# MarioPasc/MU-Diff

Hardware: AMD Instinct MI355X
Metric: 256x256 slices/sec (4-step dual-gen reverse) (higher is better)
Workload: dtype f32 (convs/attention: fp16 hi+lo split MFMA x3; 3x3 convs that fill the chip: fp16 hi.hi + e4m3 cross terms; fp32 accumulate); 1 GPU; BASELINE config 3 (BraTS-shaped test-split batches of 32; model and slice shapes of config 2): 4-step dual-generator sampling, 256x256, nf=64, ch_mult 1-2-4, 32 slices per GPU per step, batch-sharded over 1 GPU(s), weights replicated; batch=32, hipgraph=True

## Files before the change

include/mudiff_hip.h:

```cpp
#ifndef MUDIFF_HIP_H
#define MUDIFF_HIP_H

#include <stdint.h>

#ifdef __cplusplus
extern "C" {
#endif

#define MUD_OK 0
#define MUD_ERR_ARG 1
#define MUD_ERR_LAUNCH 2
#define MUD_ERR_UNSUPPORTED 3

#define MUD_ACT_NONE 0
#define MUD_ACT_SIGMOID 1
#define MUD_ACT_TANH 2
#define MUD_ACT_SILU 3
#define MUD_ACT_LRELU 4

#define MUD_PRO_NONE 0
#define MUD_PRO_AFFINE 1
#define MUD_PRO_AFFINE_SILU 2
#define MUD_PRO_LRELU 3
#define MUD_PRO_UP2_AFFINE_SILU 4

#define MUD_PREC_16X3 0
#define MUD_PREC_FP8X 1
#define MUD_PREC_16X1 2

int mud_version(void);
const char* mud_last_error(void);
const char* mud_build_flags(void);

int mud_posterior_sample(const float* x01, const float* x02, const float* xt, const float* noise,
                         const int64_t* t, const float* coef1, const float* coef2, const float* std_tab,
                         int ntab, float* out, int B, int64_t per_sample, void* stream);
int mud_q_sample(const float* x, const float* noise, const int64_t* t, int toff, const float* a_tab,
                 const float* s_tab, int ntab, float* out, int B, int64_t per_sample, void* stream);

int mud_timestep_embedding(const int64_t* t, float* out, int B, int dim, float max_positions, void* stream);
int mud_pixel_norm(const float* z, float* out, int B, int K, void* stream);
int mud_dense(const float* in, int ldi, const float* W, const float* bias, float* out, int ldo,
              int B, int K, int N, int act_in, int act_out, void* stream);

#define MUD_MLP_MAX_LAYERS 6
typedef struct mud_mlp_args {
  const float* x; int ldx; int B;
  int nlayers; int dims[MUD_MLP_MAX_LAYERS + 1];
  const float* W[MUD_MLP_MAX_LAYERS]; const float* b[MUD_MLP_MAX_LAYERS];
  int pixel_norm; int act; int act_last;
  float* out; int ldo;
  int maxdim;
} mud_mlp_args;
int mud_mlp_chain(const mud_mlp_args* a, void* stream);
int mud_mlp_chains(const mud_mlp_args* a, int n, void* stream);

int64_t mud_gn_ws_bytes(int B, int64_t HW, int C, int G);
int mud_gn_scale_shift(const float* x, int B, int64_t HW, int C, int ld, int G, float eps,
                       const float* gamma, const float* beta, int64_t g_bstride,
                       float* scale, float* shift, int ld_ss, float* mean_rstd ,
                       void* ws, void* stream);
int mud_gn_scale_shift_from_sums(const double* sums, int sums_ld, int B, int C, int G, double count, float eps,
                                 const float* gamma, const float* beta, int64_t g_bstride,
                                 float* scale, float* shift, int ld_ss, void* stream);
int mud_channel_mean(const float* x, int B, int64_t HW, int C, int ld, float* out, int ldo, void* ws, void* stream);

typedef struct mud_conv_args {
  const float* x;  int B, H, W, Cin, ldx;
  const void* w;   int64_t w_bstride;
  int ks, stride, pad;
  const float* pro_scale; const float* pro_shift; int pro_ld; int pro_mode;
  const float* bias;
  const float* bias2; int bias2_ld;
  const float* res; int ldr;
  float out_scale; int act;
  const float* emul; int ld_emul;
  const float* egate; int ld_egate;
  const float* eother; int ld_eother;
  float* out; int Cout, ldo;
  int sub2;
  double* stats; int stats_ld;
  int emul_cout;
  const double* gn_sums; int gn_sums_ld;
  int gn_G; float gn_eps; double gn_count;
  const float* gn_gamma; const float* gn_beta;
  int64_t gn_bstride;
  void* splitk_ws; int64_t splitk_ws_bytes;
  unsigned* splitk_counters; int splitk_ncounters;
  const void* skip_w; const float* skip_bias; float* skip_out; int skip_ldo;
  int prec; int w_exp;
  int res_up2; float res_k[4];
  int in_up2; float in_k[4];
} mud_conv_args;

int mud_conv2d_direct(const mud_conv_args* a, void* stream);

int64_t mud_packed_weight_bytes(int ks, int Cin, int Cout);
int mud_pack_weights(const float* src, int64_t s_tap, int64_t s_ci, int64_t s_co, int64_t src_bstride,
                     int ks, int Cin, int Cout, int nbatch, void* dst, void* stream);
int mud_pack_weights_prec(const float* src, int64_t s_tap, int64_t s_ci, int64_t s_co, int64_t src_bstride,
                          int ks, int Cin, int Cout, int nbatch, int prec, int w_exp, void* dst, void* stream);
int64_t mud_packed_weight_bytes_prec(int ks, int Cin, int Cout, int prec);
int mud_conv2d_mfma(const mud_conv_args* a, void* stream);
int mud_conv2d_mfma_prec_supported(const mud_conv_args* a, int prec);
int64_t mud_conv2d_mfma_splitk_bytes(const mud_conv_args* a);
int mud_conv2d_mfma_res_up2_supported(const mud_conv_args* a);
int mud_conv2d_mfma_in_up2_supported(const mud_conv_args* a);

typedef struct mud_census_args {
  const float* x; int B, H, W, C, ldx;
  const float* pro_scale; const float* pro_shift; int pro_ld; int pro_mode;
} mud_census_args;
typedef struct mud_census_out {
  uint64_t n, n_over, n_under, n_fp16_over, amax_bits;
} mud_census_out;
int mud_e4m3_census(const mud_census_args* a, mud_census_out* out, void* stream);

int mud_upfirdn2d(const float* in, int64_t planes, int H, int W, const float* kernel, int kh, int kw,
                  int up_x, int up_y, int down_x, int down_y, int pad_x0, int pad_x1, int pad_y0, int pad_y1,
                  float* out, void* stream);
int mud_fir_nhwc(const float* x, int B, int H, int W, int C, int ldx, const float* kernel_host, int kh, int kw,
                 int up, int down, int pad0, int pad1,
                 const float* pro_scale, const float* pro_shift, int pro_ld, int pro_mode,
                 float* out_h, int ldh, float* out_x, int ldxo, void* stream);

int mud_minibatch_stddev(const float* x, int B, int64_t hw, int C, int ld, int group, float* out, void* stream);

int mud_attention_supported(int C);
int64_t mud_attention_ws_bytes(int B, int N, int C);
int mud_attention(const float* qkv, int B, int N, int C, int ld, float scale, float* out, int ldo, void* ws, void* stream);

int mud_softmax_rows(float* s, int64_t rows, int n, int ld, void* stream);
int mud_mul(const float* a, int lda, const float* b, int ldb, float* out, int ldo, int64_t npix, int C, void* stream);
int mud_gate_mix(const float* g, int ldg, const float* att, int lda, const float* other, int ldb,
                 float* out, int ldo, int B, int64_t hw, int C, double* stats, int stats_ld, void* stream);

int mud_fourier_embedding(const float* t, const float* W, float* out, int B, int n, void* stream);
int mud_resize_bilinear(const float* in, int64_t planes, int H, int W, int Ho, int Wo, float* out, void* stream);
int mud_affine_clamp(const float* x, int64_t n, float scale, float shift, float lo, float hi, float* out, void* stream);

int64_t mud_value_range_ws_bytes(void);
int mud_value_range(const float* a, int64_t na, const float* b, int64_t nb, float* out, void* ws, void* stream);
int mud_quantize_u8(const float* x, int64_t n, float lo, float range, uint8_t* out, void* stream);
int64_t mud_slice_metrics_ws_bytes(int n, int H, int W);
int mud_slice_metrics_u8(const uint8_t* pred, const uint8_t* gt, int n, int H, int W, int64_t* sse, int64_t* sae, double* ssim_sum,
                         void* ws, int64_t ws_bytes, void* stream);

#define MUD_VM_MAX_REGIONS 8
#define MUD_VM_NQ 8
#define MUD_VM_N 0
#define MUD_VM_SSE 1
#define MUD_VM_SAE 2
#define MUD_VM_N_INT 3
#define MUD_VM_SSIM 4
#define MUD_VM_SS 5
#define MUD_VM_SS2 6
#define MUD_VM_SSE_STD 7
int64_t mud_volume_metrics_ws_bytes(int Z, int X, int Y, int nreg);
int mud_volume_metrics(const float* pred, const float* gt, const uint8_t* region, const float* std, int Z, int X, int Y, int nreg,
                       double* sums, void* ws, int64_t ws_bytes, void* stream);

int64_t mud_lpips_packed_bytes(void);
int mud_lpips_pack(const float* table, void* const* conv_w, void* const* conv_b, void* const* lin_w, void* packed, void* stream);
int64_t mud_lpips_ws_bytes(int n, int H, int W);
int mud_lpips_u8(const uint8_t* pred, const uint8_t* gt, int n, int H, int W, const void* packed, double* out, void* ws,
                 int64_t ws_bytes, void* stream);

int mud_randn_keyed(float* out, int rows, int64_t row_len, const int64_t* keys, uint64_t seed, int step, int kind, void* stream);
int mud_ensemble_stats(const float* samples, int n, int N, int64_t hw, float scale, float shift, float lo, float hi, float* mean,
                       float* std, void* stream);

#define MUD_ENSEMBLE_MAX_QUANTILES 8
#define MUD_ENSEMBLE_QUANTILES_MAX_N 64
int mud_ensemble_quantiles(const float* samples, int n, int N, int64_t hw, float scale, float shift, float lo, float hi, const double* q,
                           int K, float* out, void* stream);

#define MUD_VC_NC 5
#define MUD_VC_NS 2
#define MUD_VC_PARTS 16
#define MUD_VC_N 0
#define MUD_VC_BELOW 1
#define MUD_VC_ABOVE 2
#define MUD_VC_INSIDE 3
#define MUD_VC_NONFINITE 4
#define MUD_VC_WIDTH 0
#define MUD_VC_WIDTH_INSIDE 1
int mud_volume_interval_coverage(const float* lo, const float* hi, const float* gt, const uint8_t* region, int Z, int X, int Y, int nreg,
                                 int z0, int z1, int64_t* counts, double* sums, void* ws, int64_t ws_bytes, void* stream);

#define MUD_COUPLING_MAX_RADIUS 32
int mud_randn_keyed_coupled(float* out, int rows, int64_t row_len, const int64_t* keys, uint64_t seed, int step, int kind,
                            const double* half_taps, int radius, void* stream);

int mud_known_constrain(const float* x_new, const float* known, const uint8_t* mask, const float* noise, const int64_t* keys, uint64_t seed,
                        int step, int kind, const int64_t* t, int toff, const float* a_tab, const float* s_tab, int ntab, int clean,
                        float* out, int rows, int64_t row_len, void* stream);
int mud_known_coverage(const double* m, int SX, int SY, int SZ, int X, int Y, int Z, uint8_t* out, void* stream);

int mud_fft2_c2c(const float* in, float* out, int rows, int S, int inverse, void* stream);
int mud_fft2_r2c(const float* in, float* out, int rows, int S, int inverse, void* stream);
int mud_kspace_constrain(const float* x_new, const float* y, const uint8_t* mask, int mask_rows, const float* noise, const int64_t* keys,
                         uint64_t seed, int step, int kind, const int64_t* t, int toff, const float* a_tab, const float* s_tab, int ntab,
                         int clean, float* out, float* work, int rows, int S, void* stream);

#define MUD_SLAB_MAX_MEMBERS 16
int mud_slab_constrain(const float* x_new, const float* y, const int32_t* members, const float* weights, const float* gains, int groups, int L,
                       const float* noise, const int64_t* keys, uint64_t seed, int step, int kind, const int64_t* t, int toff,
                       const float* a_tab, const float* s_tab, int ntab, int clean, float* out, int rows, int64_t row_len, void* stream);
int mud_slab_average(const float* x, const int32_t* members, const float* weights, int groups, int L, float* avg, int rows, int64_t row_len,
                     void* stream);

int mud_slab_kspace_constrain(const float* x_new, const float* y, const uint8_t* mask, int mask_rows, const int32_t* members,
                              const float* weights, const float* gains, int groups, int L, const float* noise, const int64_t* keys,
                              uint64_t seed, int step, int kind, const int64_t* t, int toff, const float* a_tab, const float* s_tab,
                              int ntab, int clean, float* out, float* work, int rows, int S, void* stream);

#define MUD_BAND_MAX_MEMBERS 32
#define MUD_BAND_MAX_BW 8
#define MUD_BAND_MAX_M 256
#define MUD_BAND_MAX_N 512
typedef struct mud_band_tables {
  int m, n, bw, nnz;
  const int32_t* start;
  const int32_t* member;
  const float* w;
  const int32_t* tstart;
  const int32_t* tmember;
  const float* tw;
  const float* lc;
} mud_band_tables;
int mud_band_constrain(const float* x, const float* y, const mud_band_tables* tab, const float* noise, const int64_t* keys, uint64_t seed, int step,
                       int kind, const int64_t* t, int toff, const float* a_tab, const float* s_tab, int ntab, int clean, float* out, float* work,
                       int sets, int64_t row_len, void* stream);
int mud_band_measure(const float* x, const mud_band_tables* tab, float* ax, int sets, int64_t row_len, void* stream);

#define MUD_TP_NQ 8
#define MUD_TP_PARTS 16
#define MUD_TP_N_DZ 0
#define MUD_TP_S_DZ 1
#define MUD_TP_N_DZZ 2
#define MUD_TP_S_DZZ 3
#define MUD_TP_N_DX 4
#define MUD_TP_S_DX 5
#define MUD_TP_N_DY 6
#define MUD_TP_S_DY 7
int mud_volume_through_plane(const float* vol, const uint8_t* mask, int Z, int X, int Y, int z0, int z1, double* sums, void* ws,
                             int64_t ws_bytes, void* stream);

#define MUD_NIFTI_U1 2
#define MUD_NIFTI_I2 4
#define MUD_NIFTI_I4 8
#define MUD_NIFTI_F4 16
#define MUD_NIFTI_U2 512
#define MUD_VI_MAX_RANKS 4
#define MUD_VI_WINDOW 16
typedef struct mud_volume_census_record {
  uint64_t n, n_nonfinite;
  float min, max;
  int32_t count[MUD_VI_MAX_RANKS];
  int64_t first_rank[MUD_VI_MAX_RANKS];
  float window[MUD_VI_MAX_RANKS][MUD_VI_WINDOW];
} mud_volume_census_record;
int64_t mud_volume_census_ws_bytes(void);
int mud_volume_census(const void* vol, int datatype, int X, int Y, int Z, float slope, float inter, const double* q, int nq,
                      mud_volume_census_record* record, void* ws, int64_t ws_bytes, void* stream);
int mud_volume_slab_normalise(const void* vol, int datatype, int X, int Y, int Z, float slope, float inter, float lo, float den,
                              int degenerate, int s0, int s1, float* out, void* stream);
int mud_volume_slab_zscore(const void* vol, int datatype, int X, int Y, int Z, float slope, float inter, float mean, float std, int s0,
                           int s1, float* out, void* stream);
int mud_volume_assemble(const float* planes, const float* planes2, int X, int Y, int Z, int s0, int s1, float* vol, float* vol2,
                        void* stream);
int mud_volume_regrid(const void* src, int datatype, int SX, int SY, int SZ, float slope, float inter, const double* m, int mode, int X,
                      int Y, int Z, float* out, void* stream);
int mud_volume_bspline_coeffs(const void* vol, int datatype, int SX, int SY, int SZ, float slope, float inter, double* coeffs,
                              uint32_t* nonfinite, void* stream);
int mud_volume_regrid_cubic(const double* coeffs, int SX, int SY, int SZ, const void* src, int datatype, float slope, float inter,
                            const double* m, double lo, double hi, int X, int Y, int Z, float* out, void* stream);
int mud_volume_joint_hist(const void* fix, int fix_dt, int X, int Y, int Z, float fix_slope, float fix_inter, const void* mov, int mov_dt,
                          int SX, int SY, int SZ, float mov_slope, float mov_inter, const double* m, int stride, double fix_lo,
                          double fix_scale, double mov_lo, double mov_scale, int bins, uint32_t* hist, void* stream);
int mud_volume_mirror_moments(const void* vol, int datatype, int X, int Y, int Z, float slope, float inter, const double* mats, int K,
                              int stride, double lo, double scale, int bins, uint64_t* sums, void* stream);
int mud_volume_bias_log(const void* vol, int datatype, int X, int Y, int Z, float slope, float inter, int shrink, float* u, void* stream);
int mud_volume_bias_corrected(const float* u, const float* c_old, float* c_new, const double* lattices, int levels, int X, int Y, int Z,
                              int shrink, uint64_t* stats, void* stream);
int mud_volume_bias_hist(const float* c, int64_t n, double lo, double scale, int bins, uint32_t* hist, void* stream);
int mud_volume_bias_fit(const float* c, const double* table, int bins, double lo, double scale, int level, int X, int Y, int Z, int shrink,
                        int k, int64_t* sums, void* stream);
int mud_volume_bias_apply(const void* vol, int datatype, int X, int Y, int Z, float slope, float inter, const double* lattices, int levels,
                          int field, float* out, void* stream);
int mud_volume_denoise_residual(const void* vol, int datatype, int X, int Y, int Z, float slope, float inter, uint32_t* keys, void* stream);
int mud_volume_denoise_select_hist(const uint32_t* keys, int64_t n, uint32_t prefix, int pass, uint32_t* hist, void* stream);
int mud_volume_denoise_nlm(const void* vol, int datatype, int X, int Y, int Z, float slope, float inter, int search, int patch, double sigma,
                           double beta, int rician, float* out, uint32_t* zeroed, void* stream);
int mud_volume_fg_range(const void* vol, int datatype, int X, int Y, int Z, float slope, float inter, uint32_t* range, void* stream);
int mud_volume_fg_hist(const void* vol, int datatype, int X, int Y, int Z, float slope, float inter, double lo, double scale, int bins,
                       uint32_t* hist, void* stream);
int mud_volume_fg_mask(const void* vol, int datatype, int X, int Y, int Z, float slope, float inter, double lo, double scale, int bins, int k,
                       uint8_t* mask, void* stream);
int mud_volume_fg_morph(const uint8_t* in, int X, int Y, int Z, int dilate, uint8_t* out, void* stream);
int mud_volume_fg_label(const uint8_t* mask, int X, int Y, int Z, int value, int32_t* labels, void* stream);
int mud_volume_fg_census(const int32_t* labels, int X, int Y, int Z, uint32_t* census, uint64_t* summary, void* stream);
int mud_volume_fg_select(const int32_t* labels, const uint32_t* census, int64_t n, int root, int holes, uint8_t* mask, uint32_t* count,
                         void* stream);
int mud_volume_fg_apply(const void* vol, int datatype, int X, int Y, int Z, float slope, float inter, const uint8_t* mask, float* out,
                        uint32_t* removed, void* stream);
int mud_volume_edt(const uint8_t* mask, int X, int Y, int Z, int value, double sx, double sy, double sz, double* d2, void* stream);
int mud_volume_edt_select(const double* d2, int64_t n, double r2, int above, const uint8_t* within, uint8_t* out, uint32_t* count,
                          void* stream);
int mud_volume_reorient(const void* src, int elem_bytes, int SX, int SY, int SZ, int p0, int p1, int p2, int flip_mask, void* dst,
                        void* stream);
int mud_volume_lowpass(const void* vol, int datatype, int X, int Y, int Z, float slope, float inter, const double* wx, int rx,
                       const double* wy, int ry, const double* wz, int rz, float* out, float* scratch, uint32_t* nonfinite, void* stream);

#ifdef __cplusplus
}
#endif
#endif
```

mu-diff_amd/backbones/up_or_down_sampling.py:

```python
import numpy as np
import torch
import torch.nn as nn

from mudiff_hip import ops
from mudiff_hip.ops import View
from utils.op import upfirdn2d


def _setup_kernel(k):
    k = np.asarray(k, dtype=np.float32)
    if k.ndim == 1:
        k = np.outer(k, k)
    k /= np.sum(k)
    assert k.ndim == 2 and k.shape[0] == k.shape[1]
    return k


def fir_params(mode, k=None, factor=2, gain=1, conv_k=3):
    if k is None:
        k = [1] * factor
    if mode == 'up':
        kk = _setup_kernel(k) * (gain * (factor ** 2))
        p = kk.shape[0] - factor
        return kk, factor, 1, ((p + 1) // 2 + factor - 1, p // 2)
    if mode == 'naive_up':
        return np.ones((factor, factor), np.float32), factor, 1, (factor - 1, 0)
    if mode == 'naive_down':
        return np.full((factor, factor), 1.0 / (factor * factor), np.float32), 1, factor, (0, 0)
    kk = _setup_kernel(k) * gain
    if mode == 'down':
        p = kk.shape[0] - factor
        return kk, 1, factor, ((p + 1) // 2, p // 2)
    if mode == 'conv_down':
        p = (kk.shape[0] - factor) + (conv_k - 1)
        return kk, 1, 1, ((p + 1) // 2, p // 2)
    raise ValueError(mode)


_DEV_KERNELS = {}


def _device_kernel(kk, device):
    key = (kk.tobytes(), kk.shape, str(device))
    t = _DEV_KERNELS.get(key)
    if t is None:
        t = torch.tensor(kk, device=device, dtype=torch.float32)
        _DEV_KERNELS[key] = t
    return t


def upsample_2d(x, k=None, factor=2, gain=1):
    kk, up, down, pad = fir_params('up', k, factor, gain)
    return upfirdn2d(x, torch.tensor(kk, device=x.device, dtype=x.dtype), up=up, pad=pad)


def downsample_2d(x, k=None, factor=2, gain=1):
    kk, up, down, pad = fir_params('down', k, factor, gain)
    return upfirdn2d(x, torch.tensor(kk, device=x.device, dtype=x.dtype), down=down, pad=pad)


def conv_downsample_2d(x, w, k=None, factor=2, gain=1):
    kk, _, _, pad = fir_params('conv_down', k, factor, gain, conv_k=w.shape[-1])
    xf = upfirdn2d(x, torch.tensor(kk, device=x.device, dtype=x.dtype), pad=pad)
    out = ops.conv(View.from_nchw(xf), ops.direct_weight(w), w.shape[-1], w.shape[0], mfma=False, stride=factor, pad=0)
    return out.to_nchw()


def naive_upsample_2d(x, factor=2):
    kk, up, down, pad = fir_params('naive_up', factor=factor)
    return upfirdn2d(x, _device_kernel(kk, x.device), up=up, pad=pad)


def naive_downsample_2d(x, factor=2):
    kk, up, down, pad = fir_params('naive_down', factor=factor)
    return upfirdn2d(x, _device_kernel(kk, x.device), down=down, pad=pad)


def resample_view(x: View, direction, fir, fir_kernel):
    kk, up, down, pad = fir_params(direction if fir else 'naive_' + direction, fir_kernel)
    if x.C % 4 == 0:
        return ops.fir_nhwc(x, kk, up, down, pad)[0]
    assert x.ld == x.C, 'planes path needs a dense view'
    t = x.base.reshape(x.B, x.H, x.W, x.C)
    planes = t.reshape(x.B, 1, x.H, x.W) if x.C == 1 else t.permute(0, 3, 1, 2).contiguous()
    r = upfirdn2d(planes, _device_kernel(kk, x.device), up=up, down=down, pad=pad)
    return View.from_nchw(r)


def padded_strided_conv(x: View, kk, pad, weights, ks, cout, bias, res, out_scale, out, layer=None):
    if x.C % 4 == 0 and x.C >= 8 and ks == 3 and x.H % 2 == 0 and x.W % 2 == 0:
        xf, _ = ops.fir_nhwc(x, kk, 1, 1, pad)
        prec = ops.choose_prec(xf, cout, ops.PRO_NONE, sub2=True)
        return ops.conv(xf, weights(True, prec), 3, cout, mfma=True, bias=bias, res=res, out_scale=out_scale, out=out, sub2=True, prec=prec,
                        layer=layer)
    if x.C % 4 == 0:
        xf, _ = ops.fir_nhwc(x, kk, 1, 1, pad)
    else:
        assert x.ld == x.C
        t = x.base.reshape(x.B, x.H, x.W, x.C)
        planes = t.reshape(x.B, 1, x.H, x.W) if x.C == 1 else t.permute(0, 3, 1, 2).contiguous()
        xf = View.from_nchw(upfirdn2d(planes, _device_kernel(np.ascontiguousarray(kk, np.float32), x.device), pad=pad))
    return ops.conv(xf, weights(False), ks, cout, mfma=False, stride=2, pad=0, bias=bias, res=res, out_scale=out_scale, out=out)


class Conv2d(nn.Module):

    def __init__(self, in_ch, out_ch, kernel, up=False, down=False, resample_kernel=(1, 3, 3, 1), use_bias=True, kernel_init=None):
        super().__init__()
        assert not (up and down)
        assert kernel >= 1 and kernel % 2 == 1
        self.weight = nn.Parameter(torch.zeros(out_ch, in_ch, kernel, kernel))
        if kernel_init is not None:
            self.weight.data = kernel_init(self.weight.data.shape)
        if use_bias:
            self.bias = nn.Parameter(torch.zeros(out_ch))
        self.up, self.down, self.resample_kernel, self.kernel, self.use_bias = up, down, resample_kernel, kernel, use_bias
        self._prep = None

    def _weights(self, mfma=False, prec=ops.PREC_16X3):
        key = (self.weight._version, self.weight.data_ptr(), mfma, prec)
        if self._prep is None or self._prep[0] != key:
            with torch.no_grad():
                self._prep = (key, ops.pack_conv_weight(self.weight, prec=prec) if mfma else ops.direct_weight(self.weight))
        return self._prep[1]

    def run(self, x: View, res: View = None, out_scale=1.0, out: View = None):
        if self.up:
            raise NotImplementedError('Conv2d(up=True) is unreachable in the reference (upsample_conv_2d raises)')
        bias = self.bias.detach() if self.use_bias else None
        if not self.down:
            return ops.conv(x, self._weights(), self.kernel, self.weight.shape[0], mfma=False, bias=bias, res=res, out_scale=out_scale, out=out)
        kk, up, down, pad = fir_params('conv_down', self.resample_kernel, conv_k=self.kernel)
        return padded_strided_conv(x, kk, pad, self._weights, self.kernel, self.weight.shape[0], bias, res, out_scale, out,
                                   layer=self.__dict__.get('_layer_name', 'Conv2d_0'))

    def forward(self, x):
        return self.run(View.from_nchw(x)).to_nchw()
```

mu-diff_amd/csrc/conv_direct.hip:

```cpp
#include "mud_common.h"
#include <stdlib.h>

template <int VO, int VI>
__global__ __launch_bounds__(256) void k_conv_direct(mud_conv_args a, int Ho, int Wo, int co_groups) {
  extern __shared__ __attribute__((aligned(16))) char smem_raw[];
  float* st_lds = (float*)smem_raw;
  const int b = blockIdx.y;
  if (a.stats) {
    for (int i = threadIdx.x; i < 2 * a.Cout; i += 256) st_lds[i] = 0.f;
    __syncthreads();
  }
  const unsigned total = (unsigned)Ho * (unsigned)Wo * (unsigned)co_groups;
  const unsigned nthreads = gridDim.x * blockDim.x;
  const unsigned stride = (nthreads / (unsigned)co_groups) * (unsigned)co_groups;
  const unsigned first = blockIdx.x * blockDim.x + threadIdx.x;
  const int cg = (int)(first % (unsigned)co_groups);
  float ssum[VO], ssq[VO];
#pragma unroll
  for (int j = 0; j < VO; ++j) ssum[j] = ssq[j] = 0.f;
  for (uint64_t idx64 = first; first < stride && idx64 < total; idx64 += stride) {
    const unsigned p = (unsigned)idx64 / (unsigned)co_groups;
    const int oy = (int)(p / (unsigned)Wo);
    const int ox = (int)(p - (unsigned)oy * (unsigned)Wo);
    const int co = cg * VO;
    float acc[VO];
#pragma unroll
    for (int j = 0; j < VO; ++j) acc[j] = 0.f;
    const float* wb = (const float*)((const char*)a.w + (int64_t)b * a.w_bstride);
    for (int ky = 0; ky < a.ks; ++ky) {
      const int iy = oy * a.stride - a.pad + ky;
      if (iy < 0 || iy >= a.H) continue;
      for (int kx = 0; kx < a.ks; ++kx) {
        const int ix = ox * a.stride - a.pad + kx;
        if (ix < 0 || ix >= a.W) continue;
        const float* xp = a.x + (((int64_t)b * a.H + iy) * a.W + ix) * a.ldx;
        const float* wp = wb + ((int64_t)(ky * a.ks + kx) * a.Cin) * a.Cout + co;
        for (int ci = 0; ci < a.Cin; ci += VI) {
          float xv[VI];
          if (VI == 4) *(f32x4*)xv = *(const f32x4*)(xp + ci);
          else xv[0] = xp[ci];
#pragma unroll
          for (int u = 0; u < VI; ++u) {
            float v = xv[u];
            if (a.pro_mode == MUD_PRO_LRELU)
              v = v > 0.f ? v : 0.2f * v;
            else if (a.pro_mode != MUD_PRO_NONE)
              v = mud_prologue(v, a.pro_scale[(int64_t)b * a.pro_ld + ci + u], a.pro_shift[(int64_t)b * a.pro_ld + ci + u], a.pro_mode);
            const float* w = wp + (int64_t)(ci + u) * a.Cout;
            if (VO == 4) {
              const f32x4 wv = *(const f32x4*)w;
#pragma unroll
              for (int j = 0; j < 4; ++j) acc[j] = fmaf(v, wv[j], acc[j]);
            } else {
              acc[0] = fmaf(v, w[0], acc[0]);
            }
          }
        }
      }
    }
    const int64_t opix = ((int64_t)b * Ho + oy) * Wo + ox;
#pragma unroll
    for (int j = 0; j < VO; ++j) {
      float v = acc[j];
      if (a.bias) v += a.bias[co + j];
      if (a.bias2) v += a.bias2[(int64_t)b * a.bias2_ld + co + j];
      if (a.res) v += a.res[opix * a.ldr + co + j];
      v = mud_act(v * a.out_scale, a.act);
      if (a.emul && (a.emul_cout <= 0 || co + j < a.emul_cout)) v *= a.emul[opix * a.ld_emul + co + j];
      if (a.egate) {
        const float gt = a.egate[opix * a.ld_egate + co + j];
        v = gt * v + (1.0f - gt) * a.eother[opix * a.ld_eother + co + j];
      }
      acc[j] = v;
    }
    float* op = a.out + opix * a.ldo + co;
    if (VO == 4) *(f32x4*)op = *(f32x4*)acc;
    else op[0] = acc[0];
#pragma unroll
    for (int j = 0; j < VO; ++j) {
      ssum[j] += acc[j];
      ssq[j] += acc[j] * acc[j];
    }
  }
  if (a.stats) {
    if (first < stride && first < total) {
      const int co = (int)(first % co_groups) * VO;
#pragma unroll
      for (int j = 0; j < VO; ++j) {
        atomicAdd(&st_lds[(co + j) * 2], ssum[j]);
        atomicAdd(&st_lds[(co + j) * 2 + 1], ssq[j]);
      }
    }
    __syncthreads();
    for (int i = threadIdx.x; i < 2 * a.Cout; i += 256)
      atomicAdd(a.stats + ((int64_t)b * a.stats_ld + (i >> 1)) * 2 + (i & 1), (double)st_lds[i]);
  }
}

#define HEAD_PIX 8
template <int S>
__global__ __launch_bounds__(256) void k_conv_head3x3(mud_conv_args a, int co_groups, int strips_per_row, int Ho, int Wo) {
  extern __shared__ __attribute__((aligned(16))) char smem_raw[];
  float* st_lds = (float*)smem_raw;
  const int b = blockIdx.y;
  if (a.stats) {
    for (int i = threadIdx.x; i < 2 * a.Cout; i += 256) st_lds[i] = 0.f;
    __syncthreads();
  }
  const int cg = threadIdx.x % co_groups, co = cg * 4;
  const int spb = 256 / co_groups;
  const int ls = threadIdx.x / co_groups;
  f32x4 w[9];
#pragma unroll
  for (int t = 0; t < 9; ++t) w[t] = *(const f32x4*)((const float*)a.w + (int64_t)t * a.Cout + co);
  f32x4 bias = {0.f, 0.f, 0.f, 0.f};
  if (a.bias) bias = *(const f32x4*)(a.bias + co);
  if (a.bias2) bias += *(const f32x4*)(a.bias2 + (int64_t)b * a.bias2_ld + co);
  const int64_t HW = (int64_t)a.H * a.W;
  const float* xb = a.x + (int64_t)b * HW * a.ldx;
  f32x4 s4 = {0.f, 0.f, 0.f, 0.f}, q4 = {0.f, 0.f, 0.f, 0.f};
  const int64_t nstrips = (int64_t)Ho * strips_per_row;
  constexpr int WIN = S * (HEAD_PIX - 1) + 3;
  const bool active = ls < spb;
  for (int64_t st = (int64_t)blockIdx.x * spb + ls; active && st < nstrips; st += (int64_t)gridDim.x * spb) {
    const int y = (int)(st / strips_per_row), x0 = (int)(st - (int64_t)y * strips_per_row) * HEAD_PIX;
    float win[3][WIN];
#pragma unroll
    for (int dy = 0; dy < 3; ++dy) {
      const int iy = y * S + dy - a.pad;
      const bool yok = iy >= 0 && iy < a.H;
      const int64_t rowoff = (int64_t)(yok ? iy : 0) * a.W;
#pragma unroll
      for (int j = 0; j < WIN; ++j) {
        const int ix = x0 * S + j - a.pad;
        const bool ok = yok && ix >= 0 && ix < a.W;
        const float v = xb[(rowoff + (ok ? ix : 0)) * a.ldx];
        win[dy][j] = ok ? v : 0.f;
      }
    }
#pragma unroll
    for (int k = 0; k < HEAD_PIX; ++k) {
      if (x0 + k >= Wo) break;
      f32x4 acc = bias;
#pragma unroll
      for (int dy = 0; dy < 3; ++dy)
#pragma unroll
        for (int dx = 0; dx < 3; ++dx) acc += win[dy][k * S + dx] * w[dy * 3 + dx];
      const int64_t opix = ((int64_t)b * Ho + y) * Wo + x0 + k;
      if (a.res) acc += *(const f32x4*)(a.res + opix * a.ldr + co);
      acc *= a.out_scale;
      if (a.act != MUD_ACT_NONE) {
#pragma unroll
        for (int e = 0; e < 4; ++e) acc[e] = mud_act(acc[e], a.act);
      }
      *(f32x4*)(a.out + opix * a.ldo + co) = acc;
      s4 += acc;
      q4 += acc * acc;
    }
  }
  if (a.stats) {
    if (active) {
#pragma unroll
      for (int e = 0; e < 4; ++e) {
        atomicAdd(&st_lds[(co + e) * 2], s4[e]);
        atomicAdd(&st_lds[(co + e) * 2 + 1], q4[e]);
      }
    }
    __syncthreads();
    for (int i = threadIdx.x; i < 2 * a.Cout; i += 256)
      atomicAdd(a.stats + ((int64_t)b * a.stats_ld + (i >> 1)) * 2 + (i & 1), (double)st_lds[i]);
  }
}

#define TAIL_ROWS 8
#define TAIL_REC 20
template <int COUT>
__global__ __launch_bounds__(256) void k_conv_tail3x3(mud_conv_args a, int tiles_x, int tiles_y) {
  __shared__ __attribute__((aligned(16))) float tile[(TAIL_ROWS + 2) * 34 * TAIL_REC];
  const int b = blockIdx.y;
  const int ty0 = (blockIdx.x / tiles_x) * TAIL_ROWS, tx0 = (blockIdx.x % tiles_x) * 32;
  const int tid = threadIdx.x, py = tid >> 5, px = tid & 31;
  const float* xb = a.x + (int64_t)b * a.H * a.W * a.ldx;
  const float* wb = (const float*)((const char*)a.w + (int64_t)b * a.w_bstride);
  float acc[COUT];
#pragma unroll
  for (int j = 0; j < COUT; ++j) acc[j] = 0.f;
  constexpr int NPIX = (TAIL_ROWS + 2) * 34, ITEMS = NPIX * 4;
  for (int c0 = 0; c0 < a.Cin; c0 += 16) {
    for (int it = tid; it < ITEMS; it += 256) {
      const int p = it >> 2, q = it & 3;
      const int gy = ty0 + p / 34 - 1, gx = tx0 + p % 34 - 1;
      const bool ok = gy >= 0 && gy < a.H && gx >= 0 && gx < a.W;
      f32x4 v = {0.f, 0.f, 0.f, 0.f};
      if (ok) {
        v = *(const f32x4*)(xb + ((int64_t)gy * a.W + gx) * a.ldx + c0 + q * 4);
        if (a.pro_mode == MUD_PRO_LRELU) {
#pragma unroll
          for (int e = 0; e < 4; ++e) v[e] = v[e] > 0.f ? v[e] : 0.2f * v[e];
        } else if (a.pro_mode != MUD_PRO_NONE) {
          const f32x4 sc = *(const f32x4*)(a.pro_scale + (int64_t)b * a.pro_ld + c0 + q * 4);
          const f32x4 sh = *(const f32x4*)(a.pro_shift + (int64_t)b * a.pro_ld + c0 + q * 4);
#pragma unroll
          for (int e = 0; e < 4; ++e) v[e] = mud_prologue(v[e], sc[e], sh[e], a.pro_mode);
        }
      }
      *(f32x4*)(tile + p * TAIL_REC + q * 4) = v;
    }
    __syncthreads();
#pragma unroll
    for (int t = 0; t < 9; ++t) {
      const float* rec = tile + ((py + t / 3) * 34 + px + t % 3) * TAIL_REC;
      const float* wt = wb + ((int64_t)t * a.Cin + c0) * a.Cout;
#pragma unroll
      for (int q = 0; q < 4; ++q) {
        const f32x4 v = *(const f32x4*)(rec + q * 4);
#pragma unroll
        for (int e = 0; e < 4; ++e)
#pragma unroll
          for (int j = 0; j < COUT; ++j) acc[j] = fmaf(v[e], wt[(q * 4 + e) * COUT + j], acc[j]);
      }
    }
    __syncthreads();
  }
  const int gy = ty0 + py, gx = tx0 + px;
  if (gy < a.H && gx < a.W) {
    const int64_t opix = ((int64_t)b * a.H + gy) * a.W + gx;
#pragma unroll
    for (int j = 0; j < COUT; ++j) {
      float v = acc[j];
      if (a.bias) v += a.bias[j];
      if (a.res) v += a.res[opix * a.ldr + j];
      a.out[opix * a.ldo + j] = mud_act(v * a.out_scale, a.act);
    }
  }
}

extern "C" int mud_conv2d_direct(const mud_conv_args* ap, void* stream) {
  MUD_REQUIRE(ap, "mud_conv2d_direct: null args");
  const mud_conv_args a = *ap;
  MUD_REQUIRE(a.x && a.w && a.out, "mud_conv2d_direct: null pointer");
  MUD_REQUIRE(a.B >= 0 && a.H > 0 && a.W > 0 && a.Cin > 0 && a.Cout > 0 && a.ks >= 1 && a.stride >= 1 && a.pad >= 0,
              "mud_conv2d_direct: bad sizes");
  MUD_REQUIRE(a.ldx >= a.Cin && a.ldo >= a.Cout, "mud_conv2d_direct: ld smaller than C");
  MUD_REQUIRE(a.pro_mode == MUD_PRO_NONE || a.pro_mode == MUD_PRO_LRELU || (a.pro_scale && a.pro_shift && a.pro_ld >= a.Cin), "mud_conv2d_direct: prologue arrays missing");
  MUD_REQUIRE(!a.res || a.ldr >= a.Cout, "mud_conv2d_direct: bad residual view");
  MUD_REQUIRE(!a.res_up2, "mud_conv2d_direct: res_up2 (a residual up-sampled on load) is built for mud_conv2d_mfma's 3x3 kernel only");
  MUD_REQUIRE(!a.in_up2, "mud_conv2d_direct: in_up2 (an input up-sampled while it is staged) is built for mud_conv2d_mfma's 3x3 kernel only");
  const int Ho = (a.H + 2 * a.pad - a.ks) / a.stride + 1, Wo = (a.W + 2 * a.pad - a.ks) / a.stride + 1;
  MUD_REQUIRE(Ho > 0 && Wo > 0, "mud_conv2d_direct: empty output");
  if (a.B == 0) return MUD_OK;
  const bool vo4 = a.Cout % 4 == 0 && a.ldo % 4 == 0 && mud_aligned16(a.out) && mud_aligned16(a.w) && (a.w_bstride % 16 == 0);
  const bool vi4 = a.Cin % 4 == 0 && a.ldx % 4 == 0 && mud_aligned16(a.x);
  const int co_groups = vo4 ? a.Cout / 4 : a.Cout;
  if (a.Cin == 1 && a.ks == 3 && ((a.stride == 1 && a.pad == 1) || (a.stride == 2 && a.pad == 0)) && vo4 && !a.emul && !a.egate && co_groups <= 256 && a.pro_mode == MUD_PRO_NONE && a.w_bstride == 0 &&
      (!a.res || (a.ldr % 4 == 0 && mud_aligned16(a.res))) && (!a.bias || mud_aligned16(a.bias)) &&
      (!a.bias2 || (a.bias2_ld % 4 == 0 && mud_aligned16(a.bias2)))) {
    MUD_REQUIRE(a.B <= 65535 && (!a.stats || a.stats_ld >= a.Cout), "mud_conv2d_direct: bad batch / stats view");
    const int spb = 256 / co_groups, strips_per_row = (int)mud_cdiv(Wo, HEAD_PIX);
    int64_t blocks = mud_cdiv((int64_t)Ho * strips_per_row, spb);
    if (blocks > 256 * 16) blocks = 256 * 16;
    if (a.stats) {
      static const int cap = getenv("MUD_HEAD_CAP") ? atoi(getenv("MUD_HEAD_CAP")) : 0;
      int64_t per_image = 2048 / a.B > 16 ? 2048 / a.B : 16;
      const int64_t lim = cap > 0 ? cap : (a.B == 1 ? 256 : 128);
      if (per_image > lim) per_image = lim;
      if (blocks > per_image) blocks = per_image;
    }
    if (a.stride == 1)
      hipLaunchKernelGGL(k_conv_head3x3<1>, dim3((int)blocks, a.B), dim3(256), a.stats ? 2 * a.Cout * sizeof(float) : 0, (hipStream_t)stream, a, co_groups,
                         strips_per_row, Ho, Wo);
    else
      hipLaunchKernelGGL(k_conv_head3x3<2>, dim3((int)blocks, a.B), dim3(256), a.stats ? 2 * a.Cout * sizeof(float) : 0, (hipStream_t)stream, a, co_groups,
                         strips_per_row, Ho, Wo);
    MUD_CHECK_LAUNCH("mud_conv2d_direct(head)");
    return MUD_OK;
  }
  if (a.ks == 3 && a.stride == 1 && a.pad == 1 && a.Cout <= 4 && a.Cin % 16 == 0 && vi4 && !a.emul && !a.egate && !a.stats && !a.bias2 && !a.sub2 &&
      (a.pro_mode == MUD_PRO_NONE || a.pro_mode == MUD_PRO_LRELU || (a.pro_ld % 4 == 0 && mud_aligned16(a.pro_scale) && mud_aligned16(a.pro_shift)))) {
    MUD_REQUIRE(a.B <= 65535, "mud_conv2d_direct: B too large");
    const int tiles_x = (int)mud_cdiv(a.W, 32), tiles_y = (int)mud_cdiv(a.H, TAIL_ROWS);
    dim3 grid(tiles_x * tiles_y, a.B), block(256);
    hipStream_t s = (hipStream_t)stream;
    switch (a.Cout) {
      case 1: hipLaunchKernelGGL((k_conv_tail3x3<1>), grid, block, 0, s, a, tiles_x, tiles_y); break;
      case 2: hipLaunchKernelGGL((k_conv_tail3x3<2>), grid, block, 0, s, a, tiles_x, tiles_y); break;
      case 3: hipLaunchKernelGGL((k_conv_tail3x3<3>), grid, block, 0, s, a, tiles_x, tiles_y); break;
      default: hipLaunchKernelGGL((k_conv_tail3x3<4>), grid, block, 0, s, a, tiles_x, tiles_y); break;
    }
    MUD_CHECK_LAUNCH("mud_conv2d_direct(tail)");
    return MUD_OK;
  }
  const int64_t total = (int64_t)Ho * Wo * co_groups;
  int64_t blocks = mud_cdiv(total, 256 * (a.stats ? 8 : 1));
  if (blocks > 256 * 32) blocks = 256 * 32;
  while (blocks * 256 < co_groups) ++blocks;
  MUD_REQUIRE(a.B <= 65535 && total < (1ll << 31) - (1ll << 24), "mud_conv2d_direct: B or image too large");
  MUD_REQUIRE(!a.stats || (a.stats_ld >= a.Cout && a.Cout <= 8192), "mud_conv2d_direct: bad stats view");
  hipStream_t s = (hipStream_t)stream;
  dim3 grid((int)blocks, a.B), block(256);
  const size_t lds = a.stats ? 2 * a.Cout * sizeof(float) : 0;
  if (vo4 && vi4) hipLaunchKernelGGL((k_conv_direct<4, 4>), grid, block, lds, s, a, Ho, Wo, co_groups);
  else if (vo4) hipLaunchKernelGGL((k_conv_direct<4, 1>), grid, block, lds, s, a, Ho, Wo, co_groups);
  else if (vi4) hipLaunchKernelGGL((k_conv_direct<1, 4>), grid, block, lds, s, a, Ho, Wo, co_groups);
  else hipLaunchKernelGGL((k_conv_direct<1, 1>), grid, block, lds, s, a, Ho, Wo, co_groups);
  MUD_CHECK_LAUNCH("mud_conv2d_direct");
  return MUD_OK;
}
```

mu-diff_amd/csrc/conv_mfma.hip:

```cpp
#include "mud_common.h"
#include <stdlib.h>
#include <type_traits>
#include <utility>

typedef int i32x4 __attribute__((ext_vector_type(4)));
typedef int i32x8 __attribute__((ext_vector_type(8)));
typedef _Float16 f16x4 __attribute__((ext_vector_type(4)));
typedef _Float16 f16x8 __attribute__((ext_vector_type(8)));

typedef mud_h16x4 h16x4;
typedef mud_h16x8 h16x8;
__device__ __forceinline__ int cm_e4m3x4(f32x4 v, float scale) {
  v = v * scale;
#pragma unroll
  for (int e = 0; e < 4; ++e) v[e] = __builtin_amdgcn_fmed3f(v[e], -448.0f, 448.0f);
  int p = __builtin_amdgcn_cvt_pk_fp8_f32(v[0], v[1], 0, false);
  return __builtin_amdgcn_cvt_pk_fp8_f32(v[2], v[3], p, true);
}
#define CM_BN 64
#define CM_BPLANE (CM_BN * 32)
#define CM_BSTEP (2 * CM_BPLANE)
#define CM_PIX 80
#define CM_GN_MAXC 1024
#define CM_GN_BYTES (2 * CM_GN_MAXC * 4)

template <int KS, int MT, int WM, int WN, bool DUAL = false, int PREC = MUD_PREC_16X3>
struct CmGeo {
  static constexpr int NT = 64 * WM * WN;
  static constexpr int TAPS = KS * KS;
  static constexpr int CH = (KS == 3) ? 1 : 2;
  static constexpr int KCH = 16 * CH;
  static constexpr int ROWS = WM * MT;
  static constexpr int PW = 32 + KS - 1;
  static constexpr int P = (KS == 3) ? (ROWS + 2) * PW : 32 * WM * MT;
  static constexpr bool H1 = PREC == MUD_PREC_16X1;
  static constexpr int PIX = H1 ? 48 : CM_PIX;
  static constexpr int BSTEP = H1 ? CM_BPLANE : CM_BSTEP;
  static constexpr int PLANE = P * PIX;
  static constexpr int BUF = CH * PLANE;
  static constexpr int Q = 4 * CH;
  static constexpr int ITEMS = P * Q;
  static constexpr int NLOAD = (ITEMS + NT - 1) / NT;
  static constexpr int STEPS = TAPS * CH;
  static constexpr int GS = (KS == 3) ? 3 : 2;
  static constexpr int NG = STEPS / GS;
  static constexpr int GB1 = GS * BSTEP;
  static constexpr int GB = WN * GB1;
  static constexpr int N4 = GB / (1024 * WM * WN), REM = GB / 1024 - N4 * WM * WN;
  static_assert(GB % 1024 == 0 && GB1 % 1024 == 0, "whole 1 KiB pieces, none straddling two tiles");
  static constexpr int A_BYTES = 2 * BUF;
  static constexpr int B_OFF = A_BYTES;
  static constexpr int EP_BYTES = WM * WN * (32 * 36 * 4 + 64 * 2 * 4);
  static constexpr int GN_MAXC = DUAL ? 512 : CM_GN_MAXC;
  static constexpr int A2_OFF = A_BYTES + 2 * GB;
  static_assert(!DUAL || A2_OFF % 64 == 0, "the raw image's hi / lo halves are addressed by flipping bit 5 of the offset");
  static constexpr int A2_BYTES = DUAL ? ROWS * 32 * 64 : 0;
  static constexpr int B2_OFF = A2_OFF + A2_BYTES;
  static constexpr int B2_BYTES = DUAL ? WN * CM_BSTEP : 0;
  static constexpr int GN_OFF = B2_OFF + B2_BYTES;
  static constexpr int LDS_MAX = (GN_OFF + 2 * GN_MAXC * 4) > EP_BYTES ? (GN_OFF + 2 * GN_MAXC * 4) : EP_BYTES;
  static constexpr int lds_bytes(int gn_channels) {
    const int m = GN_OFF + 8 * ((gn_channels + 3) & ~3);
    return m > EP_BYTES ? m : EP_BYTES;
  }
  static_assert(LDS_MAX <= 160 * 1024, "LDS budget");
  static_assert(NT % Q == 0, "staging split");
  static constexpr int UP_ROWS = ROWS / 2 + 2, UP_COLS = 32 / 2 + 2;
  static constexpr int UP_ITEMS = UP_ROWS * UP_COLS * 4;
  static constexpr int UP_NLOAD = (UP_ITEMS + NT - 1) / NT;
  static constexpr int UP_BYTES = UP_ROWS * UP_COLS * 64;
};



template <class F, int... I>
__device__ __forceinline__ void cm_static_for_impl(F&& f, std::integer_sequence<int, I...>) { (f(std::integral_constant<int, I>{}), ...); }
template <int N, class F>
__device__ __forceinline__ void cm_static_for(F&& f) { cm_static_for_impl(f, std::make_integer_sequence<int, N>{}); }

__device__ __forceinline__ bool mud_dev_aligned16(const void* p) { return (((uintptr_t)p) & 15u) == 0; }


__device__ __forceinline__ void cm_gn_to_lds(const mud_conv_args& a, int b, int tid, int nthreads, float* sc_lds, int maxc) {
  float* sh_lds = sc_lds + maxc;
  const int cpg = a.Cin / a.gn_G;
  for (int c = tid; c < a.Cin; c += nthreads) {
    const int g0 = (c / cpg) * cpg;
    double s = 0.0, q = 0.0;
    for (int i = 0; i < cpg; ++i) {
      const double* p = a.gn_sums + ((int64_t)b * a.gn_sums_ld + g0 + i) * 2;
      s += p[0];
      q += p[1];
    }
    const double n = a.gn_count * cpg, mean = s / n;
    double var = q / n - mean * mean;
    if (var < 0.0) var = 0.0;
    const float rstd = (float)(1.0 / sqrt(var + (double)a.gn_eps)), meanf = (float)mean;
    const float ga = a.gn_gamma ? a.gn_gamma[(int64_t)b * a.gn_bstride + c] : 1.0f;
    const float be = a.gn_beta ? a.gn_beta[(int64_t)b * a.gn_bstride + c] : 0.0f;
    const float sc = ga * rstd;
    sc_lds[c] = sc;
    sh_lds[c] = be - meanf * sc;
  }
}

__device__ __forceinline__ void cm_saturating_converters() { asm volatile("s_setreg_imm32_b32 hwreg(HW_REG_MODE, 23, 1), 1"); }

template <int PRO, bool X8, bool H1 = false>
__device__ __forceinline__ void cm_stage4(const f32x4& rw, const f32x4& sc, const f32x4& sh, float keep, h16x4& hi, h16x4& lo, int& a8, int& al8) {
  f32x4 v, l;
#pragma unroll
  for (int e = 0; e < 4; ++e) {
    float x = rw[e];
    if (PRO == MUD_PRO_AFFINE || PRO == MUD_PRO_AFFINE_SILU) {
      x = __builtin_fmaf(x, sc[e], sh[e]);
      if (PRO == MUD_PRO_AFFINE_SILU) x = cm_fast_silu(x);
    } else if (PRO == MUD_PRO_LRELU) {
      x = x > 0.f ? x : 0.2f * x;
    }
    v[e] = x * keep;
  }
  hi = __builtin_convertvector(v, h16x4);
  if constexpr (H1) return;
#pragma unroll
  for (int e = 0; e < 4; ++e) l[e] = v[e] - (float)hi[e];
  if constexpr (X8) {
    typedef short s16x2 __attribute__((ext_vector_type(2)));
    constexpr float ia = 1.0f / (float)(1 << CM_X_SA), ial = 1.0f / (float)(1 << CM_X_SAL);
    const s16x2 z = {0, 0};
    const s16x2 av = __builtin_amdgcn_cvt_scalef32_pk_fp8_f32(__builtin_amdgcn_cvt_scalef32_pk_fp8_f32(z, v[0], v[1], ia, false), v[2], v[3], ia, true);
    const s16x2 lv = __builtin_amdgcn_cvt_scalef32_pk_fp8_f32(__builtin_amdgcn_cvt_scalef32_pk_fp8_f32(z, l[0], l[1], ial, false), l[2], l[3], ial, true);
    a8 = __builtin_bit_cast(int, av);
    al8 = __builtin_bit_cast(int, lv);
  } else {
    lo = __builtin_convertvector(l, h16x4);
  }
}
__device__ __forceinline__ void cm_split4s(const f32x4& rw, float keep, h16x4& hi, h16x4& lo) {
  f32x4 v, l;
#pragma unroll
  for (int e = 0; e < 4; ++e) v[e] = rw[e] * keep;
  hi = __builtin_convertvector(v, h16x4);
#pragma unroll
  for (int e = 0; e < 4; ++e) l[e] = v[e] - (float)hi[e];
  lo = __builtin_convertvector(l, h16x4);
}

struct CmFin {
  float* ws;
  unsigned* counters;
};

template <int KS, int MT, int WM, int WN, int PRO, bool DUAL = false, int PREC = MUD_PREC_16X3>
__global__ __launch_bounds__(64 * WM * WN, (MT == 1 && WM * WN == 8) ? 4 : 2) void k_conv_mfma(mud_conv_args a, int tiles_x, int tiles_per_img, int ntiles, int k16s,
                                                                unsigned nblocks, int nsplit, int64_t split_stride, CmFin fin) {
  using G = CmGeo<KS, MT, WM, WN, DUAL, PREC>;
  constexpr bool X8 = PREC == MUD_PREC_FP8X;
  constexpr bool H1 = G::H1;
  static_assert(!X8 || KS == 3, "the fp8 cross-term plan is built for the 3x3 kernel");
  static_assert(!H1 || KS == 3, "the single-pass fp16 plan is built for the 3x3 kernel");
  constexpr bool IUP = PRO == MUD_PRO_UP2_AFFINE_SILU;
  constexpr bool AFF = PRO == MUD_PRO_AFFINE || PRO == MUD_PRO_AFFINE_SILU || IUP;
  static_assert(!IUP || (KS == 3 && !DUAL && G::ROWS % 2 == 0 && G::LDS_MAX + G::UP_BYTES <= 160 * 1024), "in_up2: 3x3, no fused skip conv, even tile rows, LDS budget");
  constexpr int GN_OFF = G::GN_OFF + (IUP ? G::UP_BYTES : 0);
  constexpr int NRAW = IUP ? G::UP_NLOAD : G::NLOAD;
  using HV4 = h16x4;
  using HV8 = h16x8;
  extern __shared__ __attribute__((aligned(16))) char smem[];
  cm_saturating_converters();
  const int tid = threadIdx.x, lane = tid & 63, wave = tid >> 6, r = lane & 31, hh = lane >> 5;
  const int wm = wave % WM, wn = wave / WM;

  unsigned lid;
  {
    const unsigned orig = blockIdx.x, xcd = orig & 7u, q = nblocks >> 3, rem = nblocks & 7u;
    lid = (xcd < rem ? xcd * (q + 1) : rem * (q + 1) + (xcd - rem) * q) + (orig >> 3);
  }
  const int nt = lid % ntiles;
  const unsigned rest = lid / ntiles;
  const int tile = rest % tiles_per_img;
  const unsigned rest2 = rest / tiles_per_img;
  const int b = rest2 % (unsigned)a.B;
  const int ksi = rest2 / (unsigned)a.B;

  const int64_t HW = (int64_t)a.H * a.W;
  int ty0 = 0, tx0 = 0;
  int64_t flat0 = 0;
  if (KS == 3) {
    ty0 = (tile / tiles_x) * G::ROWS;
    tx0 = (tile % tiles_x) * 32;
  } else {
    flat0 = (int64_t)tile * G::P;
  }
  const float* xb = a.x + (int64_t)b * (IUP ? (int64_t)(a.H >> 1) * (a.W >> 1) : HW) * a.ldx;
  const int64_t tile_bytes = (int64_t)k16s * (G::TAPS * G::BSTEP);
  const char* wb = (const char*)a.w + (int64_t)b * a.w_bstride + (int64_t)nt * WN * tile_bytes;
  const float* psc = a.pro_scale + (int64_t)b * a.pro_ld;
  const float* psh = a.pro_shift + (int64_t)b * a.pro_ld;
  const int nchunks_all = (k16s + G::CH - 1) / G::CH;
  const int per_split = (nchunks_all + nsplit - 1) / nsplit;
  const int kc0 = ksi * per_split;
  const int nchunks = (kc0 + per_split < nchunks_all) ? kc0 + per_split : nchunks_all;
  a.out += (int64_t)ksi * split_stride;

  const int q = tid % G::Q;
  int goff[NRAW], loff[G::NLOAD];
  int loff2[DUAL ? G::NLOAD : 1];
  unsigned vmask = 0;
  int slo[IUP ? G::UP_NLOAD : 1], soff[IUP ? G::NLOAD : 1];
  unsigned lmask = 0, ymask = 0, xmask = 0;
  if constexpr (IUP) {
    const int Hl = a.H >> 1, Wl = a.W >> 1;
#pragma unroll
    for (int j = 0; j < G::UP_NLOAD; ++j) {
      const int item = (tid + j * G::NT) % G::UP_ITEMS;
      const int p = item >> 2, py = p / G::UP_COLS, px = p - py * G::UP_COLS;
      const int ly = (ty0 >> 1) - 1 + py, lx = (tx0 >> 1) - 1 + px;
      const bool valid = ly >= 0 && ly < Hl && lx >= 0 && lx < Wl;
      goff[j] = valid ? (ly * Wl + lx) * a.ldx : 0;
      lmask |= (valid ? 1u : 0u) << j;
      slo[j] = p * 64 + q * 16;
    }
  }
#pragma unroll
  for (int j = 0; j < G::NLOAD; ++j) {
    const int item = (tid + j * G::NT) % G::ITEMS;
    const int p = item / G::Q;
    bool valid;
    int64_t g;
    if (KS == 3) {
      const int py = p / G::PW, px = p - py * G::PW;
      const int gy = ty0 + py - 1, gx = tx0 + px - 1;
      valid = gy >= 0 && gy < a.H && gx >= 0 && gx < a.W;
      g = ((int64_t)gy * a.W + gx) * a.ldx;
      if (DUAL) {
        const bool centre = py >= 1 && py <= G::ROWS && px >= 1 && px <= 32 && tid + j * G::NT < G::ITEMS;
        const int col = px - 1, sw = (col >> 2) & 3;
        loff2[j] = centre ? ((py - 1) * 32 + col) * 64 + ((((q & 3) >> 1) ^ sw) << 4) + (q & 1) * 8 : -1;
      }
    } else {
      const int64_t fp = flat0 + p;
      valid = fp < HW;
      g = fp * a.ldx;
    }
    if constexpr (IUP) {
      const int py = p / G::PW, px = p - py * G::PW;
      const int gy = ty0 + py - 1, gx = tx0 + px - 1, ay = gy & 1, ax = gx & 1;
      soff[j] = ((((gy >> 1) + ay - (ty0 >> 1)) * G::UP_COLS + (gx >> 1) + ax - (tx0 >> 1)) * 16 + q * 4) * 4;
      ymask |= (unsigned)ay << j;
      xmask |= (unsigned)ax << j;
    } else
      goff[j] = valid ? (int)g : 0;
    vmask |= (valid ? 1u : 0u) << j;
    loff[j] = (q >> 2) * G::PLANE + p * G::PIX + (q & 3) * 8;
  }

  f32x4 raw[NRAW];
  constexpr bool CNT = KS == 3 && !DUAL;
#define CM_RAW_WAIT(N)                                                          \
  do {                                                                          \
    if constexpr (CNT) {                                                        \
      asm volatile("s_waitcnt vmcnt(%0)" ::"n"(N) : "memory");                 \
      _Pragma("unroll") for (int j_ = 0; j_ < NRAW; ++j_) asm volatile("" : "+v"(raw[j_])); \
    }                                                                           \
  } while (0)
  f32x4 psc_r = {1.f, 1.f, 1.f, 1.f}, psh_r = {0.f, 0.f, 0.f, 0.f};
  const bool gn_fold = AFF && a.gn_sums != nullptr;
  const float* const gn_sc = (const float*)(smem + GN_OFF);
  const int gn_c = (a.Cin + 3) & ~3;
  auto fetch_raw = [&](int chunk) {
    int c = chunk * G::KCH + q * 4;
    c = c < a.Cin ? c : 0;
#pragma unroll
    for (int j = 0; j < NRAW; ++j) {
      if constexpr (CNT) asm volatile("global_load_dwordx4 %0, %1, off" : "=v"(raw[j]) : "v"(xb + goff[j] + c) : "memory");
      else raw[j] = *(const f32x4*)(xb + goff[j] + c);
    }
  };
  auto fetch_ss = [&](int chunk) {
    if (AFF) {
      int c = chunk * G::KCH + q * 4;
      c = c < a.Cin ? c : 0;
      psc_r = *(const f32x4*)(gn_sc + c);
      psh_r = *(const f32x4*)(gn_sc + gn_c + c);
    }
  };
  auto fetch_a = [&](int chunk) {
    fetch_ss(chunk);
    fetch_raw(chunk);
  };
  auto store_a_slots = [&](int chunk, char* buf, int j0, int j1) {
    const bool cvalid = chunk * G::KCH + q * 4 < a.Cin;
#pragma unroll
    for (int j = 0; j < G::NLOAD; ++j) {
      if (j < j0 || j >= j1) continue;
      const float keep = (cvalid && ((vmask >> j) & 1u)) ? 1.0f : 0.0f;
      HV4 hi, lo;
      int a8 = 0, al8 = 0;
      cm_stage4<PRO, X8, H1>(raw[j], psc_r, psh_r, keep, hi, lo, a8, al8);
      *(HV4*)(buf + loff[j]) = hi;
      if constexpr (X8) {
        *(int*)(buf + loff[j] + 32 - q * 4) = a8;
        *(int*)(buf + loff[j] + 48 - q * 4) = al8;
      } else if constexpr (!H1) {
        *(HV4*)(buf + loff[j] + 32) = lo;
      }
      if (DUAL) {
        if (loff2[j] >= 0) {
          h16x4 rhi, rlo;
          cm_split4s(raw[j], cvalid ? 1.0f : 0.0f, rhi, rlo);
          char* a2 = smem + G::A2_OFF;
          *(h16x4*)(a2 + loff2[j]) = rhi;
          *(h16x4*)(a2 + (loff2[j] ^ 32)) = rlo;
        }
      }
    }
  };
  auto store_a = [&](int chunk, char* buf) { store_a_slots(chunk, buf, 0, G::NLOAD); };
  char* const scr = smem + G::GN_OFF;
  auto up_pass1 = [&](int chunk) {
    if constexpr (IUP) {
      const bool cvalid = chunk * G::KCH + q * 4 < a.Cin;
#pragma unroll
      for (int j = 0; j < G::UP_NLOAD; ++j) {
        const float keep = (cvalid && ((lmask >> j) & 1u)) ? 1.0f : 0.0f;
        f32x4 v;
#pragma unroll
        for (int e = 0; e < 4; ++e) v[e] = cm_fast_silu(__builtin_fmaf(raw[j][e], psc_r[e], psh_r[e])) * keep;
        *(f32x4*)(scr + slo[j]) = v;
      }
    }
  };
  auto up_pass2 = [&](char* buf, int j0, int j1) {
    if constexpr (IUP) {
#pragma unroll
      for (int j = 0; j < G::NLOAD; ++j) {
        if (j < j0 || j >= j1) continue;
        const bool ay = (ymask >> j) & 1u, ax = (xmask >> j) & 1u;
        const float ky0 = ay ? a.in_k[2] : a.in_k[3], ky1 = ay ? a.in_k[0] : a.in_k[1];
        const float kx0 = ax ? a.in_k[2] : a.in_k[3], kx1 = ax ? a.in_k[0] : a.in_k[1];
        const float w00 = ky0 * kx0, w01 = ky0 * kx1, w10 = ky1 * kx0, w11 = ky1 * kx1;
        const char* sp = scr + soff[j];
        const f32x4 v00 = *(const f32x4*)sp, v01 = *(const f32x4*)(sp + 64);
        const f32x4 v10 = *(const f32x4*)(sp + G::UP_COLS * 64), v11 = *(const f32x4*)(sp + G::UP_COLS * 64 + 64);
        f32x4 t;
#pragma unroll
        for (int e = 0; e < 4; ++e) {
          float u = w00 * v00[e];
          u = __builtin_fmaf(w01, v01[e], u);
          u = __builtin_fmaf(w10, v10[e], u);
          t[e] = __builtin_fmaf(w11, v11[e], u);
        }
        HV4 hi, lo;
        int a8 = 0, al8 = 0;
        cm_stage4<MUD_PRO_NONE, X8, H1>(t, psc_r, psh_r, ((vmask >> j) & 1u) ? 1.0f : 0.0f, hi, lo, a8, al8);
        *(HV4*)(buf + loff[j]) = hi;
        if constexpr (X8) {
          *(int*)(buf + loff[j] + 32 - q * 4) = a8;
          *(int*)(buf + loff[j] + 48 - q * 4) = al8;
        } else if constexpr (!H1) {
          *(HV4*)(buf + loff[j] + 32) = lo;
        }
      }
    }
  };

  const int total_groups_all = (k16s * G::TAPS + G::GS - 1) / G::GS;
  const int total_groups = (nchunks * G::NG < total_groups_all) ? nchunks * G::NG : total_groups_all;
  char* const bring = smem + G::B_OFF;
  auto dma_b = [&](int gg) {
    char* dst = bring + (gg & 1) * G::GB;
    gg = gg < total_groups ? gg : total_groups - 1;
#pragma unroll
    for (int j = 0; j < G::N4; ++j) {
      const int byte = (wave + WM * WN * j) * 1024;
      const char* src = wb + (byte / G::GB1) * tile_bytes + (int64_t)gg * G::GB1 + byte % G::GB1 + lane * 16;
      __builtin_amdgcn_global_load_lds((const __attribute__((address_space(1))) void*)src, (__attribute__((address_space(3))) void*)(dst + byte), 16, 0, 0);
    }
    if constexpr (G::REM > 0) {
      const int byte = (wave + WM * WN * G::N4) * 1024;
      if (__builtin_amdgcn_readfirstlane(wave) < G::REM) {
        const char* src = wb + (byte / G::GB1) * tile_bytes + (int64_t)gg * G::GB1 + byte % G::GB1 + lane * 16;
        __builtin_amdgcn_global_load_lds((const __attribute__((address_space(1))) void*)src, (__attribute__((address_space(3))) void*)(dst + byte), 16, 0, 0);
      }
    }
  };
  const int lane_b = r * 32 + ((hh ^ ((r >> 3) & 1)) << 4);
  auto dma_b2 = [&](int chunk) {
    if (DUAL) {
      if (wave < 4 * WN && chunk < nchunks) {
        const int t64 = wave >> 2, within = wave & 3;
        const char* src = (const char*)a.skip_w + ((int64_t)(nt * WN + t64) * k16s + chunk) * CM_BSTEP + within * 1024 + lane * 16;
        __builtin_amdgcn_global_load_lds((const __attribute__((address_space(1))) void*)src,
                                         (__attribute__((address_space(3))) void*)(smem + G::B2_OFF + wave * 1024), 16, 0, 0);
      }
    }
  };

  const int lane_a = ((KS == 3) ? (wm * MT * G::PW + r) : (wm * MT * 32 + r)) * G::PIX + hh * 16;
  const int xa_lane0 = lane_a - hh * 16 + hh * (2 * CM_PIX);
  const int xa_lane1_t0 = lane_a - hh * 16 + (hh ? 2 * CM_PIX + 64 : CM_PIX + 48);
  const int xb_lane = r * 16 + hh * (2 * CM_BSTEP);
  const int s_a = (127 - CM_X_SA) * 0x01010101, s_al = (127 - CM_X_SAL) * 0x01010101;
  const int s_w = (127 - a.w_exp) * 0x01010101, s_wl = (127 - a.w_exp - 11) * 0x01010101;

  f32x16 acc[MT][2];
  f32x16 acc2[DUAL ? MT : 1][2];
#pragma unroll
  for (int m = 0; m < MT; ++m)
#pragma unroll
    for (int n = 0; n < 2; ++n)
#pragma unroll
      for (int i = 0; i < 16; ++i) {
        acc[m][n][i] = 0.f;
        if (DUAL) acc2[m][n][i] = 0.f;
      }
  const int lane_a2 = ((wm * MT) * 32 + r) * 64 + ((hh ^ ((r >> 2) & 3)) << 4);

  if constexpr (X8) {
    if (q == 0) {
#pragma unroll
      for (int j = 0; j < G::NLOAD; ++j) {
        *(i32x4*)(smem + loff[j] + 64) = i32x4{0, 0, 0, 0};
        *(i32x4*)(smem + G::BUF + loff[j] + 64) = i32x4{0, 0, 0, 0};
      }
    }
  }
  dma_b(kc0 * G::NG);
  dma_b2(kc0);
  fetch_raw(kc0);

  const int emul_lim = a.emul_cout > 0 ? a.emul_cout : a.Cout;
  const bool vec = ((a.Cout | a.ldo | emul_lim | (a.res ? a.ldr : 0) | (a.emul ? a.ld_emul : 0) | (a.egate ? (a.ld_egate | a.ld_eother) : 0)) & 3) == 0 &&
                   mud_dev_aligned16(a.out) && (!a.res || mud_dev_aligned16(a.res)) && (!a.emul || mud_dev_aligned16(a.emul)) &&
                   (!a.egate || (mud_dev_aligned16(a.egate) && mud_dev_aligned16(a.eother)));
  const bool slab_mode = KS == 3 && nsplit > 1 && fin.counters != nullptr;
  const bool res_in_acc = !DUAL && KS == 3 && a.res != nullptr && !a.sub2 && nsplit == 1;
  constexpr bool UP2 = KS == 3 && !DUAL && PRO == MUD_PRO_AFFINE_SILU;
  bool res_up2 = false;
  if constexpr (UP2) res_up2 = res_in_acc && a.res_up2 != 0;
  if (res_up2) {
    if constexpr (UP2) {
      const int Hl = a.H >> 1, Wl = a.W >> 1;
      const float* rb = a.res + (int64_t)b * Hl * Wl * a.ldr;
      const int jq = ((tx0 + 4 * hh) >> 1) - 1;
      unsigned cmask = 0;
#pragma unroll
      for (int i = 0; i < 16; ++i) cmask |= (jq + i >= 0 && jq + i < Wl ? 1u : 0u) << i;
      const int co0 = (nt * WN + wn) * CM_BN + r;
      const float* rc = rb + (co0 < a.Cout ? co0 : 0);
      const int dn = co0 + 32 < a.Cout ? 32 : 0;
      unsigned cm[2] = {co0 < a.Cout ? cmask : 0u, co0 + 32 < a.Cout ? cmask : 0u};
      asm volatile("" : "+v"(cm[0]), "+v"(cm[1]));
#pragma unroll
      for (int m = 0; m < MT; ++m) {
        const int gy = ty0 + __builtin_amdgcn_readfirstlane(wm) * MT + m;
        const int ay = gy & 1, y0 = (gy >> 1) - 1 + ay;
        const float ky[2] = {(y0 >= 0 && y0 < Hl) ? (ay ? a.res_k[2] : a.res_k[3]) : 0.f, (y0 + 1 < Hl) ? (ay ? a.res_k[0] : a.res_k[1]) : 0.f};
        const int yo[2] = {min(max(y0, 0), Hl - 1) * Wl, min(y0 + 1, Hl - 1) * Wl};
#pragma unroll
        for (int g4 = 0; g4 < 4; ++g4) {
          float v[2][2][4];
#pragma unroll
          for (int ry = 0; ry < 2; ++ry)
#pragma unroll
            for (int cx = 0; cx < 4; ++cx) {
              const float* pp = rc + (yo[ry] + min(max(jq + 4 * g4 + cx, 0), Wl - 1)) * a.ldr;
              v[0][ry][cx] = pp[0];
              v[1][ry][cx] = pp[dn];
            }
#pragma unroll
          for (int n = 0; n < 2; ++n) {
#pragma unroll
            for (int ry = 0; ry < 2; ++ry)
#pragma unroll
              for (int cx = 0; cx < 4; ++cx) v[n][ry][cx] = (cm[n] & (1u << (4 * g4 + cx))) ? v[n][ry][cx] : 0.f;
#pragma unroll
            for (int e = 0; e < 4; ++e) {
              const int ca = (e + 1) >> 1;
              const float kx0 = (e & 1) ? a.res_k[2] : a.res_k[3], kx1 = (e & 1) ? a.res_k[0] : a.res_k[1];
              float t = (ky[0] * kx0) * v[n][0][ca];
              t = __builtin_fmaf(ky[0] * kx1, v[n][0][ca + 1], t);
              t = __builtin_fmaf(ky[1] * kx0, v[n][1][ca], t);
              t = __builtin_fmaf(ky[1] * kx1, v[n][1][ca + 1], t);
              acc[m][n][g4 * 4 + e] = t;
            }
          }
        }
      }
    }
  } else if (res_in_acc) {
#pragma unroll
    for (int n = 0; n < 2; ++n) {
      const int co = (nt * WN + wn) * CM_BN + n * 32 + r;
#pragma unroll
      for (int m = 0; m < MT; ++m) {
        const int gy = ty0 + wm * MT + m;
#pragma unroll
        for (int reg = 0; reg < 16; ++reg) {
          const int gx = tx0 + (reg & 3) + 8 * (reg >> 2) + 4 * hh;
          const bool ok = gy < a.H && gx < a.W && co < a.Cout;
          acc[m][n][reg] = ok ? a.res[(((int64_t)b * a.H + gy) * a.W + gx) * a.ldr + co] : 0.f;
        }
      }
    }
  }

  if (gn_fold) {
    cm_gn_to_lds(a, b, tid, G::NT, (float*)(smem + GN_OFF), gn_c);
    __syncthreads();
  } else if (AFF) {
    float* sc_lds = (float*)(smem + GN_OFF);
    for (int c = tid; c < a.Cin; c += G::NT) {
      sc_lds[c] = psc[c];
      sc_lds[gn_c + c] = psh[c];
    }
    __syncthreads();
  }
  fetch_ss(kc0);
  CM_RAW_WAIT(0);
  if constexpr (IUP) {
    up_pass1(kc0);
    __syncthreads();
    up_pass2(smem + (kc0 & 1) * G::BUF, 0, G::NLOAD);
  } else
    store_a(kc0, smem + (kc0 & 1) * G::BUF);
  __syncthreads();

  auto chunk_body = [&](const int kc, auto more_t) {
    constexpr bool more = decltype(more_t)::value;
    char* cur = smem + (kc & 1) * G::BUF;
    char* nxt = smem + ((kc + 1) & 1) * G::BUF;
    cm_static_for<G::NG>([&](auto g_t) {
      constexpr int g = decltype(g_t)::value;
      const int gg = kc * G::NG + g;
      dma_b(gg + 1);
      if (g == 0 && more) fetch_a(kc + 1);
      const char* bcur = bring + (gg & 1) * G::GB + wn * G::GB1;
      if (DUAL && g == 0) {
        const char* b2 = smem + G::B2_OFF + wn * CM_BSTEP;
        h16x8 bh[2], bl[2];
#pragma unroll
        for (int n = 0; n < 2; ++n) {
          bh[n] = *(const h16x8*)(b2 + n * 1024 + lane_b);
          bl[n] = *(const h16x8*)(b2 + CM_BPLANE + n * 1024 + lane_b);
        }
#pragma unroll
        for (int m = 0; m < MT; ++m) {
          const int o2 = lane_a2 + m * (32 * 64);
          const h16x8 ah = *(const h16x8*)(smem + G::A2_OFF + o2);
          const h16x8 al = *(const h16x8*)(smem + G::A2_OFF + (o2 ^ 32));
#pragma unroll
          for (int n = 0; n < 2; ++n) {
            acc2[m][n] = mud_mfma16(al, bh[n], acc2[m][n]);
            acc2[m][n] = mud_mfma16(ah, bl[n], acc2[m][n]);
            acc2[m][n] = mud_mfma16(ah, bh[n], acc2[m][n]);
          }
        }
      }
      if (DUAL && g == 1 && more) dma_b2(kc + 1);
#pragma unroll
      for (int sg = 0; sg < G::GS; ++sg) {
        const int st = g * G::GS + sg;
        const int s = (KS == 3) ? 0 : st;
        const int tap = (KS == 3) ? st : 0;
        const int dy = tap / KS, dx = tap % KS;
        if (KS == 3 || kc * G::CH + s < k16s) {
          HV8 bh[2], bl[2];
#pragma unroll
          for (int n = 0; n < 2; ++n) {
            bh[n] = *(const HV8*)(bcur + sg * G::BSTEP + n * 1024 + lane_b);
            if constexpr (!X8 && !H1) bl[n] = *(const HV8*)(bcur + sg * G::BSTEP + CM_BPLANE + n * 1024 + lane_b);
          }
#pragma unroll
          for (int m = 0; m < MT; ++m) {
            const int off = s * G::PLANE + ((KS == 3) ? ((m + dy) * G::PW + dx) : (m * 32)) * G::PIX;
            const HV8 ah = *(const HV8*)(cur + lane_a + off);
            if constexpr (X8 || H1) {
              acc[m][0] = mud_mfma16(ah, bh[0], acc[m][0]);
              acc[m][1] = mud_mfma16(ah, bh[1], acc[m][1]);
            } else {
              const HV8 al = *(const HV8*)(cur + lane_a + off + 32);
              acc[m][0] = mud_mfma16(al, bh[0], acc[m][0]);
              acc[m][1] = mud_mfma16(al, bh[1], acc[m][1]);
              acc[m][0] = mud_mfma16(ah, bl[0], acc[m][0]);
              acc[m][1] = mud_mfma16(ah, bl[1], acc[m][1]);
              acc[m][0] = mud_mfma16(ah, bh[0], acc[m][0]);
              acc[m][1] = mud_mfma16(ah, bh[1], acc[m][1]);
            }
          }
          if constexpr (X8) {
            if (sg == G::GS - 1) {
              const char* brow = bcur + xb_lane;
              const char* brow1 = bcur + CM_BSTEP + r * 16;
              const int o0 = ((g * G::GS) / KS * G::PW + (g * G::GS) % KS) * CM_PIX;
              const int d1 = hh ? 0 : 16;
              auto cross = [&](int term) {
                const int wplane = CM_BPLANE + term * 1024, aoff = 48 - 16 * term;
                const char* pa0 = cur + xa_lane0 + o0 + aoff;
                const char* pa1 = cur + xa_lane1_t0 + o0 - d1 * term;
                const int sa = term ? s_a : s_al, sb = term ? s_wl : s_w;
                i32x8 wq[2];
#pragma unroll
                for (int n = 0; n < 2; ++n) {
                  const i32x4 q0 = *(const i32x4*)(brow + wplane + n * 512);
                  const i32x4 q1 = *(const i32x4*)(brow1 + wplane + n * 512);
                  wq[n] = i32x8{q0[0], q0[1], q0[2], q0[3], q1[0], q1[1], q1[2], q1[3]};
                }
#pragma unroll
                for (int m = 0; m < MT; ++m) {
                  const i32x4 p0 = *(const i32x4*)(pa0 + m * G::PW * CM_PIX);
                  const i32x4 p1 = *(const i32x4*)(pa1 + m * G::PW * CM_PIX);
                  const i32x8 aq = i32x8{p0[0], p0[1], p0[2], p0[3], p1[0], p1[1], p1[2], p1[3]};
#pragma unroll
                  for (int n = 0; n < 2; ++n) acc[m][n] = __builtin_amdgcn_mfma_scale_f32_32x32x64_f8f6f4(aq, wq[n], acc[m][n], 0, 0, 0, sa, 0, sb);
                }
              };
              if constexpr (DUAL || MT == 1) {
#pragma clang loop unroll(disable)
                for (int term = 0; term < 2; ++term) cross(term);
              } else {
                cross(0);
                cross(1);
              }
            }
          }
        }
        if (more && G::NG > 1 && st >= G::GS) {
          static_assert(G::N4 * WM * WN + G::REM == G::GB / 1024 && G::REM < WM * WN, "DMA pieces per wave and group");
          if (st == G::GS) {
            if constexpr (G::REM > 0) {
              if (__builtin_amdgcn_readfirstlane(wave) < G::REM) CM_RAW_WAIT(G::N4 + 1);
              else CM_RAW_WAIT(G::N4);
            } else CM_RAW_WAIT(G::N4);
          }
          constexpr int SPAN = G::STEPS - G::GS;
          auto jb = [](int i) {
            if (PRO != MUD_PRO_NONE) return (i * G::NLOAD) / SPAN;
            return i >= SPAN ? G::NLOAD : ((i > 0 ? i - 1 : 0) * G::NLOAD + G::NLOAD - 1) / SPAN;
          };
          const int j0 = jb(st - G::GS), j1 = jb(st - G::GS + 1);
          if constexpr (IUP) {
            static_assert(G::NG == 3 && G::GS == 3, "in_up2: the scratch in group 1, the staging in group 2");
            if (st == G::GS) up_pass1(kc + 1);
            if (st >= 2 * G::GS) up_pass2(nxt, ((st - 2 * G::GS) * G::NLOAD) / G::GS, ((st - 2 * G::GS + 1) * G::NLOAD) / G::GS);
          } else
            store_a_slots(kc + 1, nxt, j0, j1);
        }
      }
      if (G::NG == 1 && more) store_a(kc + 1, nxt);
      if constexpr (g == 0 && more && CNT) {
        asm volatile("s_waitcnt vmcnt(%0) lgkmcnt(0)\n\ts_barrier" ::"n"(NRAW) : "memory");
      } else
        __syncthreads();
    });
  };
  for (int kc = kc0; kc + 1 < nchunks; ++kc) chunk_body(kc, std::true_type{});
  if (kc0 < nchunks) chunk_body(nchunks - 1, std::false_type{});

  if constexpr (KS == 3) {
    if (slab_mode) {
      constexpr int NT = 64 * WM * WN;
      const unsigned nslots = nblocks / (unsigned)nsplit;
      const unsigned slot = ((unsigned)b * (unsigned)tiles_per_img + (unsigned)tile) * (unsigned)ntiles + (unsigned)nt;
      constexpr int ACC_WORDS = 32 * MT;
      const int64_t tile_words = (int64_t)NT * ACC_WORDS * (DUAL ? 2 : 1);
      float* mine = fin.ws + ((int64_t)ksi * nslots + slot) * tile_words + tid;
#pragma unroll
      for (int m = 0; m < MT; ++m)
#pragma unroll
        for (int n = 0; n < 2; ++n)
#pragma unroll
          for (int reg = 0; reg < 16; ++reg)
            __hip_atomic_store(mine + ((m * 2 + n) * 16 + reg) * NT, acc[m][n][reg], __ATOMIC_RELAXED, __HIP_MEMORY_SCOPE_AGENT);
      if (DUAL) {
#pragma unroll
        for (int m = 0; m < MT; ++m)
#pragma unroll
          for (int n = 0; n < 2; ++n)
#pragma unroll
            for (int reg = 0; reg < 16; ++reg)
              __hip_atomic_store(mine + (ACC_WORDS + (m * 2 + n) * 16 + reg) * NT, acc2[m][n][reg], __ATOMIC_RELAXED, __HIP_MEMORY_SCOPE_AGENT);
      }
      __builtin_amdgcn_fence(__ATOMIC_RELEASE, "workgroup");
      asm volatile("s_waitcnt vmcnt(0)" ::: "memory");
      __syncthreads();
      int* flag = (int*)smem;
      if (tid == 0) {
        unsigned* cnt = fin.counters + slot;
        const int last = __hip_atomic_fetch_add(cnt, 1u, __ATOMIC_RELAXED, __HIP_MEMORY_SCOPE_AGENT) == (unsigned)nsplit - 1u;
        if (last) __hip_atomic_store(cnt, 0u, __ATOMIC_RELAXED, __HIP_MEMORY_SCOPE_AGENT);
        *flag = last;
      }
      __syncthreads();
      if (!*flag) return;
      __syncthreads();
      const float* slab0 = fin.ws + (int64_t)slot * tile_words + tid;
      for (int k = 0; k < nsplit; ++k) {
        const float* src = slab0 + (int64_t)k * nslots * tile_words;
#pragma unroll
        for (int m = 0; m < MT; ++m)
#pragma unroll
          for (int n = 0; n < 2; ++n)
#pragma unroll
            for (int reg = 0; reg < 16; ++reg) {
              const float pv = __hip_atomic_load(src + ((m * 2 + n) * 16 + reg) * NT, __ATOMIC_RELAXED, __HIP_MEMORY_SCOPE_AGENT);
              acc[m][n][reg] = k == 0 ? pv : acc[m][n][reg] + pv;
            }
        if (DUAL) {
#pragma unroll
          for (int m = 0; m < MT; ++m)
#pragma unroll
            for (int n = 0; n < 2; ++n)
#pragma unroll
              for (int reg = 0; reg < 16; ++reg) {
                const float pv = __hip_atomic_load(src + (ACC_WORDS + (m * 2 + n) * 16 + reg) * NT, __ATOMIC_RELAXED, __HIP_MEMORY_SCOPE_AGENT);
                acc2[m][n][reg] = k == 0 ? pv : acc2[m][n][reg] + pv;
              }
        }
      }
    }
  }

  constexpr int EP_LD = 36;
  float* ep = (float*)smem + wave * (32 * EP_LD);
  float* st_lds = (float*)smem + WM * WN * (32 * EP_LD);
#pragma unroll
  for (int n = 0; n < 2; ++n) {
    const int co = (nt * WN + wn) * CM_BN + n * 32 + r;
    const bool cok = co < a.Cout;
    float badd = (a.bias && cok) ? a.bias[co] : 0.f;
    if (a.bias2 && cok) badd += a.bias2[(int64_t)b * a.bias2_ld + co];
    if (vec) {
      const int col = (lane & 7) * 4, co4 = (nt * WN + wn) * CM_BN + n * 32 + col;
      f32x4 s4 = {0.f, 0.f, 0.f, 0.f}, q4 = {0.f, 0.f, 0.f, 0.f};
#pragma unroll
      for (int m = 0; m < MT; ++m) {
#pragma unroll
        for (int reg = 0; reg < 16; ++reg) ep[((reg & 3) + 8 * (reg >> 2) + 4 * hh) * EP_LD + r] = acc[m][n][reg] + badd;
#pragma unroll
        for (int pass = 0; pass < 4; ++pass) {
          const int prow = pass * 8 + (lane >> 3);
          int64_t opix;
          bool valid;
          if (KS == 3) {
            const int gy = ty0 + wm * MT + m, gx = tx0 + prow;
            valid = gy < a.H && gx < a.W;
            opix = ((int64_t)b * a.H + gy) * a.W + gx;
            if (a.sub2) {
              valid = valid && (gy & 1) && (gx & 1);
              opix = ((int64_t)b * (a.H >> 1) + (gy >> 1)) * (a.W >> 1) + (gx >> 1);
            }
          } else {
            const int64_t fp = flat0 + (wm * MT + m) * 32 + prow;
            valid = fp < HW;
            opix = (int64_t)b * HW + fp;
          }
          f32x4 v = *(const f32x4*)(ep + prow * EP_LD + col);
          if (valid && co4 < a.Cout) {
            if (a.res && !res_in_acc) v += *(const f32x4*)(a.res + opix * a.ldr + co4);
            v *= a.out_scale;
            if (a.act != MUD_ACT_NONE) {
#pragma unroll
              for (int e = 0; e < 4; ++e) v[e] = mud_act_fast(v[e], a.act);
            }
            if (a.emul && co4 < emul_lim) v *= *(const f32x4*)(a.emul + opix * a.ld_emul + co4);
            if (a.egate) {
              const f32x4 gt = *(const f32x4*)(a.egate + opix * a.ld_egate + co4);
              v = gt * v + (1.0f - gt) * *(const f32x4*)(a.eother + opix * a.ld_eother + co4);
            }
            *(f32x4*)(a.out + opix * a.ldo + co4) = v;
            s4 += v;
            q4 += v * v;
          }
        }
      }
      if (a.stats) {
#pragma unroll
        for (int e = 0; e < 4; ++e) {
          float ss = s4[e], qq = q4[e];
#pragma unroll
          for (int o = 8; o < 64; o <<= 1) { ss += __shfl_xor(ss, o, 64); qq += __shfl_xor(qq, o, 64); }
          if (lane < 8) {
            st_lds[(wave * 64 + n * 32 + col + e) * 2] = ss;
            st_lds[(wave * 64 + n * 32 + col + e) * 2 + 1] = qq;
          }
        }
      }
    } else {
      float ssum = 0.f, ssq = 0.f;
#pragma unroll
      for (int m = 0; m < MT; ++m) {
#pragma unroll
        for (int reg = 0; reg < 16; ++reg) {
          const int prow = (reg & 3) + 8 * (reg >> 2) + 4 * hh;
          int64_t opix;
          bool valid;
          if (KS == 3) {
            const int gy = ty0 + wm * MT + m, gx = tx0 + prow;
            valid = gy < a.H && gx < a.W;
            opix = ((int64_t)b * a.H + gy) * a.W + gx;
            if (a.sub2) {
              valid = valid && (gy & 1) && (gx & 1);
              opix = ((int64_t)b * (a.H >> 1) + (gy >> 1)) * (a.W >> 1) + (gx >> 1);
            }
          } else {
            const int64_t fp = flat0 + (wm * MT + m) * 32 + prow;
            valid = fp < HW;
            opix = (int64_t)b * HW + fp;
          }
          if (valid && cok) {
            float v = acc[m][n][reg] + badd;
            if (a.res && !res_in_acc) v += a.res[opix * a.ldr + co];
            v = mud_act_fast(v * a.out_scale, a.act);
            if (a.emul && co < emul_lim) v *= a.emul[opix * a.ld_emul + co];
            if (a.egate) {
              const float gt = a.egate[opix * a.ld_egate + co];
              v = gt * v + (1.0f - gt) * a.eother[opix * a.ld_eother + co];
            }
            a.out[opix * a.ldo + co] = v;
            ssum += v;
            ssq += v * v;
          }
        }
      }
      if (a.stats) {
        ssum += __shfl_xor(ssum, 32, 64);
        ssq += __shfl_xor(ssq, 32, 64);
        if (hh == 0) {
          st_lds[(wave * 64 + n * 32 + r) * 2] = ssum;
          st_lds[(wave * 64 + n * 32 + r) * 2 + 1] = ssq;
        }
      }
    }
  }
  if (DUAL) {
#pragma unroll
    for (int n = 0; n < 2; ++n) {
      const int co = (nt * WN + wn) * CM_BN + n * 32 + r;
      const float badd = (a.skip_bias && co < a.Cout) ? a.skip_bias[co] : 0.f;
      const int col = (lane & 7) * 4, co4 = (nt * WN + wn) * CM_BN + n * 32 + col;
#pragma unroll
      for (int m = 0; m < MT; ++m) {
#pragma unroll
        for (int reg = 0; reg < 16; ++reg) ep[((reg & 3) + 8 * (reg >> 2) + 4 * hh) * EP_LD + r] = acc2[m][n][reg] + badd;
#pragma unroll
        for (int pass = 0; pass < 4; ++pass) {
          const int prow = pass * 8 + (lane >> 3);
          const int gy = ty0 + wm * MT + m, gx = tx0 + prow;
          const f32x4 v = *(const f32x4*)(ep + prow * EP_LD + col);
          if (gy < a.H && gx < a.W && co4 < a.Cout) *(f32x4*)(a.skip_out + (((int64_t)b * a.H + gy) * a.W + gx) * a.skip_ldo + co4) = v;
        }
      }
    }
  }
  if (a.stats) {
    __syncthreads();
    if (tid < 128 * WN) {
      const int tn = tid >> 7, ch = (tid & 127) >> 1, k = tid & 1, co = (nt * WN + tn) * CM_BN + ch;
      if (co < a.Cout) {
        float t = 0.f;
#pragma unroll
        for (int w = 0; w < WM; ++w) t += st_lds[((tn * WM + w) * 64 + ch) * 2 + k];
        atomicAdd(a.stats + ((int64_t)b * a.stats_ld + co) * 2 + k, (double)t);
      }
    }
  }
}

template <int KS, int MT>
struct CmGeoRegB {
  static constexpr int TAPS = KS * KS;
  static constexpr int CH = (KS == 3) ? 1 : 2;
  static constexpr int KCH = 16 * CH;
  static constexpr int ROWS = 4 * MT;
  static constexpr int PW = 32 + KS - 1;
  static constexpr int P = (KS == 3) ? (ROWS + 2) * PW : 128 * MT;
  static constexpr int PLANE = P * CM_PIX;
  static constexpr int BUF = CH * PLANE;
  static constexpr int GN_OFF = 2 * BUF;
  static constexpr int GN_MAXC = CM_GN_MAXC;
  static constexpr int LDS_MAX = GN_OFF + CM_GN_BYTES;
  static constexpr int lds_bytes(int gn_channels) { return GN_OFF + 8 * ((gn_channels + 3) & ~3); }
  static constexpr int Q = 4 * CH;
  static constexpr int ITEMS = P * Q;
  static constexpr int NLOAD = (ITEMS + 255) / 256;
  static constexpr int STEPS = TAPS * CH;
  static constexpr int RING = (KS == 3) ? 3 : 2;
};
template <int KS, int MT, int PRO>
__global__ __launch_bounds__(256, (MT == 4 ? 1 : 2)) void k_conv_mfma_regb(mud_conv_args a, int tiles_x, int tiles_per_img, int ntiles, int k16s,
                                                       unsigned nblocks) {
  using G = CmGeoRegB<KS, MT>;
  extern __shared__ __attribute__((aligned(16))) char smem[];
  cm_saturating_converters();
  const int tid = threadIdx.x, lane = tid & 63, wave = tid >> 6, r = lane & 31, hh = lane >> 5;

  unsigned lid;
  {
    const unsigned orig = blockIdx.x, xcd = orig & 7u, q = nblocks >> 3, rem = nblocks & 7u;
    lid = (xcd < rem ? xcd * (q + 1) : rem * (q + 1) + (xcd - rem) * q) + (orig >> 3);
  }
  const int nt = lid % ntiles;
  const unsigned rest = lid / ntiles;
  const int tile = rest % tiles_per_img;
  const int b = rest / tiles_per_img;

  const int64_t HW = (int64_t)a.H * a.W;
  int ty0 = 0, tx0 = 0;
  int64_t flat0 = 0;
  if (KS == 3) {
    ty0 = (tile / tiles_x) * G::ROWS;
    tx0 = (tile % tiles_x) * 32;
  } else {
    flat0 = (int64_t)tile * G::P;
  }
  const float* xb = a.x + (int64_t)b * HW * a.ldx;
  const char* wb = (const char*)a.w + (int64_t)b * a.w_bstride + (int64_t)nt * k16s * (G::TAPS * CM_BSTEP) + r * 32 + ((hh ^ ((r >> 3) & 1)) << 4);
  const float* psc = a.pro_scale + (int64_t)b * a.pro_ld;
  const float* psh = a.pro_shift + (int64_t)b * a.pro_ld;
  const int nchunks = (k16s + G::CH - 1) / G::CH;

  const int q = tid % G::Q;
  int goff[G::NLOAD], loff[G::NLOAD];
  unsigned vmask = 0;
#pragma unroll
  for (int j = 0; j < G::NLOAD; ++j) {
    const int item = (tid + j * 256) % G::ITEMS;
    const int p = item / G::Q;
    bool valid;
    int64_t g;
    if (KS == 3) {
      const int py = p / G::PW, px = p - py * G::PW;
      const int gy = ty0 + py - 1, gx = tx0 + px - 1;
      valid = gy >= 0 && gy < a.H && gx >= 0 && gx < a.W;
      g = ((int64_t)gy * a.W + gx) * a.ldx;
    } else {
      const int64_t fp = flat0 + p;
      valid = fp < HW;
      g = fp * a.ldx;
    }
    goff[j] = valid ? (int)g : 0;
    vmask |= (valid ? 1u : 0u) << j;
    loff[j] = (q >> 2) * G::PLANE + p * CM_PIX + (q & 3) * 8;
  }

  f32x4 raw[G::NLOAD];
  f32x4 psc_r = {1.f, 1.f, 1.f, 1.f}, psh_r = {0.f, 0.f, 0.f, 0.f};
  const bool gn_fold = (PRO == MUD_PRO_AFFINE || PRO == MUD_PRO_AFFINE_SILU) && a.gn_sums != nullptr;
  const float* const gn_sc = (const float*)(smem + G::GN_OFF);
  const int gn_c = (a.Cin + 3) & ~3;
  auto fetch_raw = [&](int chunk) {
    int c = chunk * G::KCH + q * 4;
    c = c < a.Cin ? c : 0;
#pragma unroll
    for (int j = 0; j < G::NLOAD; ++j) raw[j] = *(const f32x4*)(xb + goff[j] + c);
  };
  auto fetch_ss = [&](int chunk) {
    if (PRO == MUD_PRO_AFFINE || PRO == MUD_PRO_AFFINE_SILU) {
      int c = chunk * G::KCH + q * 4;
      c = c < a.Cin ? c : 0;
// ... 118 lines not shown
            const int gy = ty0 + wave * MT + m, gx = tx0 + prow;
            valid = gy < a.H && gx < a.W;
            opix = ((int64_t)b * a.H + gy) * a.W + gx;
            if (a.sub2) {
              valid = valid && (gy & 1) && (gx & 1);
              opix = ((int64_t)b * (a.H >> 1) + (gy >> 1)) * (a.W >> 1) + (gx >> 1);
            }
          } else {
            const int64_t fp = flat0 + (wave * MT + m) * 32 + prow;
            valid = fp < HW;
            opix = (int64_t)b * HW + fp;
          }
          f32x4 v = *(const f32x4*)(ep + prow * EP_LD + col);
          if (valid && co4 < a.Cout) {
            if (a.res) v += *(const f32x4*)(a.res + opix * a.ldr + co4);
            v *= a.out_scale;
            if (a.act != MUD_ACT_NONE) {
#pragma unroll
              for (int e = 0; e < 4; ++e) v[e] = mud_act_fast(v[e], a.act);
            }
            if (a.emul && co4 < emul_lim) v *= *(const f32x4*)(a.emul + opix * a.ld_emul + co4);
            if (a.egate) {
              const f32x4 gt = *(const f32x4*)(a.egate + opix * a.ld_egate + co4);
              v = gt * v + (1.0f - gt) * *(const f32x4*)(a.eother + opix * a.ld_eother + co4);
            }
            *(f32x4*)(a.out + opix * a.ldo + co4) = v;
            s4 += v;
            q4 += v * v;
          }
        }
      }
      if (a.stats) {
#pragma unroll
        for (int e = 0; e < 4; ++e) {
          float ss = s4[e], qq = q4[e];
#pragma unroll
          for (int o = 8; o < 64; o <<= 1) { ss += __shfl_xor(ss, o, 64); qq += __shfl_xor(qq, o, 64); }
          if (lane < 8) {
            st_lds[(wave * 64 + n * 32 + col + e) * 2] = ss;
            st_lds[(wave * 64 + n * 32 + col + e) * 2 + 1] = qq;
          }
        }
      }
    } else {
      float ssum = 0.f, ssq = 0.f;
#pragma unroll
      for (int m = 0; m < MT; ++m) {
#pragma unroll
        for (int reg = 0; reg < 16; ++reg) {
          const int prow = (reg & 3) + 8 * (reg >> 2) + 4 * hh;
          int64_t opix;
          bool valid;
          if (KS == 3) {
            const int gy = ty0 + wave * MT + m, gx = tx0 + prow;
            valid = gy < a.H && gx < a.W;
            opix = ((int64_t)b * a.H + gy) * a.W + gx;
            if (a.sub2) {
              valid = valid && (gy & 1) && (gx & 1);
              opix = ((int64_t)b * (a.H >> 1) + (gy >> 1)) * (a.W >> 1) + (gx >> 1);
            }
          } else {
            const int64_t fp = flat0 + (wave * MT + m) * 32 + prow;
            valid = fp < HW;
            opix = (int64_t)b * HW + fp;
          }
          if (valid && cok) {
            float v = acc[m][n][reg] + badd;
            if (a.res) v += a.res[opix * a.ldr + co];
            v = mud_act_fast(v * a.out_scale, a.act);
            if (a.emul && co < emul_lim) v *= a.emul[opix * a.ld_emul + co];
            if (a.egate) {
              const float gt = a.egate[opix * a.ld_egate + co];
              v = gt * v + (1.0f - gt) * a.eother[opix * a.ld_eother + co];
            }
            a.out[opix * a.ldo + co] = v;
            ssum += v;
            ssq += v * v;
          }
        }
      }
      if (a.stats) {
        ssum += __shfl_xor(ssum, 32, 64);
        ssq += __shfl_xor(ssq, 32, 64);
        if (hh == 0) {
          st_lds[(wave * 64 + n * 32 + r) * 2] = ssum;
          st_lds[(wave * 64 + n * 32 + r) * 2 + 1] = ssq;
        }
      }
    }
  }
  if (a.stats) {
    __syncthreads();
    if (tid < 128) {
      const int ch = tid >> 1, k = tid & 1, co = nt * CM_BN + ch;
      if (co < a.Cout) {
        const float t = (st_lds[(0 * 64 + ch) * 2 + k] + st_lds[(1 * 64 + ch) * 2 + k]) +
                        (st_lds[(2 * 64 + ch) * 2 + k] + st_lds[(3 * 64 + ch) * 2 + k]);
        atomicAdd(a.stats + ((int64_t)b * a.stats_ld + co) * 2 + k, (double)t);
      }
    }
  }
}

__global__ __launch_bounds__(256) void k_pack_weights(const float* __restrict__ src, int64_t s_tap, int64_t s_ci, int64_t s_co,
                                                      int64_t src_bstride, int taps, int Cin, int Cout, int k16s,
                                                      int64_t units, char* __restrict__ dst, int64_t dst_bstride, int prec, int w_exp) {
  const int b = blockIdx.y;
  for (int64_t u = (int64_t)blockIdx.x * blockDim.x + threadIdx.x; u < units; u += (int64_t)gridDim.x * blockDim.x) {
    const int h2 = (int)(u & 1), co_l = (int)((u >> 1) & 63);
    int64_t rest = u >> 7;
    const int tap = (int)(rest % taps);
    rest /= taps;
    const int kc = (int)(rest % k16s);
    const int nt = (int)(rest / k16s);
    const int co = nt * CM_BN + co_l, ci0 = kc * 16 + h2 * 8;
    f32x4 v0 = {0.f, 0.f, 0.f, 0.f}, v1 = {0.f, 0.f, 0.f, 0.f};
#pragma unroll
    for (int j = 0; j < 8; ++j) {
      float v = 0.f;
      if (co < Cout && ci0 + j < Cin) v = src[(int64_t)b * src_bstride + tap * s_tap + (int64_t)(ci0 + j) * s_ci + (int64_t)co * s_co];
      if (j < 4) v0[j] = v;
      else v1[j - 4] = v;
    }
    const int64_t bstep = prec == MUD_PREC_16X1 ? CM_BPLANE : CM_BSTEP;
    char* step = dst + (int64_t)b * dst_bstride + (((int64_t)nt * k16s + kc) * taps + tap) * bstep;
    char* base = step + co_l * 32 + ((h2 ^ ((co_l >> 3) & 1)) << 4);
    if (prec == MUD_PREC_16X1) {
      h16x4 h0, h1, l0, l1;
      mud_split4(v0, h0, l0);
      mud_split4(v1, h1, l1);
      *(h16x4*)base = h0;
      *(h16x4*)(base + 8) = h1;
    } else if (prec == MUD_PREC_FP8X) {
      h16x4 h0, h1, l0, l1;
      mud_split4(v0, h0, l0);
      mud_split4(v1, h1, l1);
      *(h16x4*)base = h0;
      *(h16x4*)(base + 8) = h1;
      const f32x4 lf0 = v0 - __builtin_convertvector(h0, f32x4), lf1 = v1 - __builtin_convertvector(h1, f32x4);
      const float sw = exp2f((float)w_exp), swl = exp2f((float)(w_exp + 11));
      char* row8 = step + CM_BPLANE + (co_l >> 5) * 512 + (co_l & 31) * 16 + h2 * 8;
      *(int*)(row8) = cm_e4m3x4(v0, sw);
      *(int*)(row8 + 4) = cm_e4m3x4(v1, sw);
      *(int*)(row8 + 1024) = cm_e4m3x4(lf0, swl);
      *(int*)(row8 + 1024 + 4) = cm_e4m3x4(lf1, swl);
    } else {
      h16x4 h0, h1, l0, l1;
      mud_split4(v0, h0, l0);
      mud_split4(v1, h1, l1);
      *(h16x4*)base = h0;
      *(h16x4*)(base + 8) = h1;
      *(h16x4*)(base + CM_BPLANE) = l0;
      *(h16x4*)(base + CM_BPLANE + 8) = l1;
    }
  }
}

extern "C" int64_t mud_packed_weight_bytes(int ks, int Cin, int Cout) {
  if ((ks != 1 && ks != 3) || Cin <= 0 || Cout <= 0) return -1;
  return mud_cdiv(Cout, CM_BN) * mud_cdiv(Cin, 16) * (int64_t)ks * ks * CM_BSTEP + 2 * CM_BSTEP;
}

extern "C" int64_t mud_packed_weight_bytes_prec(int ks, int Cin, int Cout, int prec) {
  if (prec == MUD_PREC_16X3 || (prec == MUD_PREC_FP8X && ks == 3)) return mud_packed_weight_bytes(ks, Cin, Cout);
  if (prec != MUD_PREC_16X1 || ks != 3 || Cin <= 0 || Cout <= 0) return -1;
  return mud_cdiv(Cout, CM_BN) * mud_cdiv(Cin, 16) * (int64_t)9 * CM_BPLANE + 2 * CM_BPLANE;
}

extern "C" int mud_pack_weights_prec(const float* src, int64_t s_tap, int64_t s_ci, int64_t s_co, int64_t src_bstride, int ks,
                                     int Cin, int Cout, int nbatch, int prec, int w_exp, void* dst, void* stream) {
  MUD_REQUIRE(src && dst, "mud_pack_weights: null pointer");
  MUD_REQUIRE((ks == 1 || ks == 3) && Cin > 0 && Cout > 0 && nbatch >= 1 && nbatch <= 65535, "mud_pack_weights: bad sizes");
  MUD_REQUIRE(mud_aligned16(dst), "mud_pack_weights: dst must be 16-byte aligned");
  MUD_REQUIRE(prec == MUD_PREC_16X3 || (prec == MUD_PREC_FP8X && ks == 3 && w_exp >= -100 && w_exp <= 100) || (prec == MUD_PREC_16X1 && ks == 3),
              "mud_pack_weights: prec must be MUD_PREC_16X3, MUD_PREC_FP8X with ks == 3 and |w_exp| <= 100, or MUD_PREC_16X1 with ks == 3 "
              "(got prec=%d ks=%d w_exp=%d)", prec, ks, w_exp);
  const int k16s = (int)mud_cdiv(Cin, 16), ntiles = (int)mud_cdiv(Cout, CM_BN), taps = ks * ks;
  const int64_t units = (int64_t)ntiles * k16s * taps * 128;
  int64_t blocks = mud_cdiv(units, 256);
  if (blocks > 256 * 16) blocks = 256 * 16;
  hipLaunchKernelGGL(k_pack_weights, dim3((int)blocks, nbatch), dim3(256), 0, (hipStream_t)stream, src, s_tap, s_ci, s_co,
                     src_bstride, taps, Cin, Cout, k16s, units, (char*)dst, mud_packed_weight_bytes_prec(ks, Cin, Cout, prec), prec, w_exp);
  MUD_CHECK_LAUNCH("mud_pack_weights");
  return MUD_OK;
}

extern "C" int mud_pack_weights(const float* src, int64_t s_tap, int64_t s_ci, int64_t s_co, int64_t src_bstride, int ks,
                                int Cin, int Cout, int nbatch, void* dst, void* stream) {
  return mud_pack_weights_prec(src, s_tap, s_ci, s_co, src_bstride, ks, Cin, Cout, nbatch, MUD_PREC_16X3, 0, dst, stream);
}

__global__ __launch_bounds__(256) void k_splitk_epilogue(mud_conv_args a, const float* __restrict__ part, int nsplit, int64_t split_stride,
                                                         int ldp, int64_t npix, int pix_per_block) {
  __shared__ float red[256 * 8];
  const int quads = a.Cout >> 2;
  const int rows = 256 / quads;
  const int tq = threadIdx.x % quads, tr = threadIdx.x / quads;
  const int64_t p0 = (int64_t)blockIdx.x * pix_per_block;
  const int64_t HW = (int64_t)a.H * a.W;
  const int b = (int)(p0 / HW);
  const int co = tq * 4;
  f32x4 badd = {0.f, 0.f, 0.f, 0.f};
  if (tr < rows) {
    if (a.bias) badd = *(const f32x4*)(a.bias + co);
    if (a.bias2) badd += *(const f32x4*)(a.bias2 + (int64_t)b * a.bias2_ld + co);
  }
  f32x4 s4 = {0.f, 0.f, 0.f, 0.f}, q4 = {0.f, 0.f, 0.f, 0.f};
  if (tr < rows) {
    for (int64_t p = p0 + tr; p < p0 + pix_per_block && p < npix; p += rows) {
      f32x4 v = *(const f32x4*)(part + p * ldp + co);
      for (int k = 1; k < nsplit; ++k) v += *(const f32x4*)(part + k * split_stride + p * ldp + co);
      v += badd;
      if (a.res) v += *(const f32x4*)(a.res + p * a.ldr + co);
      v *= a.out_scale;
      if (a.act != MUD_ACT_NONE) {
#pragma unroll
        for (int e = 0; e < 4; ++e) v[e] = mud_act_fast(v[e], a.act);
      }
      *(f32x4*)(a.out + p * a.ldo + co) = v;
      s4 += v;
      q4 += v * v;
    }
  }
  if (a.stats) {
#pragma unroll
    for (int e = 0; e < 4; ++e) {
      red[threadIdx.x * 8 + e] = s4[e];
      red[threadIdx.x * 8 + 4 + e] = q4[e];
    }
    __syncthreads();
    for (int i = threadIdx.x; i < quads * 8; i += 256) {
      const int qd = i >> 3, e = i & 7;
      float t = 0.f;
      for (int r = 0; r < rows; ++r) t += red[(r * quads + qd) * 8 + e];
      atomicAdd(a.stats + ((int64_t)b * a.stats_ld + qd * 4 + (e & 3)) * 2 + (e >> 2), (double)t);
    }
  }
}

static bool cm_split_eligible(const mud_conv_args& a) {
  return a.ks == 3 && !a.sub2 && !a.emul && !a.egate && a.Cout % 4 == 0 && a.Cout <= 1024 && a.ldo % 4 == 0 && (!a.res || a.ldr % 4 == 0) &&
         mud_aligned16(a.out) && (!a.res || mud_aligned16(a.res)) && (!a.bias || mud_aligned16(a.bias)) &&
         (!a.bias2 || (mud_aligned16(a.bias2) && a.bias2_ld % 4 == 0));
}

static int64_t cm_slab_bytes(int ns, int64_t blocks, int tile_words) { return (int64_t)ns * blocks * tile_words * 4; }

static int cm_splits(int64_t blocks, int nchunks) {
  static const int force = getenv("MUD_CONV_SPLITK") ? atoi(getenv("MUD_CONV_SPLITK")) : -1;
  static const int kMaxBlocks = getenv("MUD_SPLITK_MAXBLOCKS") ? atoi(getenv("MUD_SPLITK_MAXBLOCKS")) : 192;
  static const int kTarget = getenv("MUD_SPLITK_TARGET") ? atoi(getenv("MUD_SPLITK_TARGET")) : 512;
  static const int kMinChunks = getenv("MUD_SPLITK_MINCHUNKS") ? atoi(getenv("MUD_SPLITK_MINCHUNKS")) : 16;
  static const int kMinPer = getenv("MUD_SPLITK_MINPER") ? atoi(getenv("MUD_SPLITK_MINPER")) : 4;
  int ns = 1;
  if (force >= 0) ns = force < 1 ? 1 : force;
  else if (blocks <= kMaxBlocks && nchunks >= kMinChunks) {
    ns = (int)((kTarget + blocks - 1) / blocks);
    if (ns > 4) ns = 4;
  }
  if (ns > nchunks / kMinPer) ns = nchunks / kMinPer;
  if (ns < 1) ns = 1;
  while (ns > 1 && (nchunks + ns - 1) / ns * (ns - 1) >= nchunks) --ns;
  return ns;
}

template <int KS, int MT, int WM, int WN, int PRO, bool DUAL = false, int PREC = MUD_PREC_16X3>
static int cm_launch_pro(const mud_conv_args& a, hipStream_t s) {
  using G = typename std::conditional<KS == 3, CmGeo<KS, MT, WM, WN, DUAL, PREC>, CmGeoRegB<KS, MT>>::type;
  const void* kfn;
  if constexpr (KS == 3) kfn = (const void*)k_conv_mfma<KS, MT, WM, WN, PRO, DUAL, PREC>;
  else kfn = (const void*)k_conv_mfma_regb<KS, MT, PRO>;
  static mud_attr_once attr_once;
  int up_bytes = 0;
  if constexpr (PRO == MUD_PRO_UP2_AFFINE_SILU) up_bytes = G::UP_BYTES;
  if (attr_once.need()) {
    hipError_t e = hipFuncSetAttribute(kfn, hipFuncAttributeMaxDynamicSharedMemorySize, G::LDS_MAX + up_bytes);
    if (e != hipSuccess) {
      mud_set_error("mud_conv2d_mfma: cannot reserve %d B of LDS: %s", G::LDS_MAX + up_bytes, hipGetErrorString(e));
      return MUD_ERR_LAUNCH;
    }
    attr_once.ok();
  }
  const int k16s = (int)mud_cdiv(a.Cin, 16), ntiles = (int)mud_cdiv(a.Cout, CM_BN * WN);
  const int lds = G::lds_bytes((PRO == MUD_PRO_AFFINE || PRO == MUD_PRO_AFFINE_SILU || PRO == MUD_PRO_UP2_AFFINE_SILU) ? a.Cin : 0) + up_bytes;
  int tiles_x = 1;
  int64_t tiles;
  if (KS == 3) {
    tiles_x = (int)mud_cdiv(a.W, 32);
    tiles = (int64_t)tiles_x * mud_cdiv(a.H, WM * MT);
  } else {
    tiles = mud_cdiv((int64_t)a.H * a.W, G::P);
  }
  int64_t nblocks = tiles * ntiles * a.B;
  MUD_REQUIRE(nblocks <= 0x7fffffff, "mud_conv2d_mfma: grid too large");
  if constexpr (KS == 3) {
    const int64_t npix = (int64_t)a.B * a.H * a.W;
    int ns = 1;
    static const bool two_launches = getenv("MUD_CONV_SPLITK_2LAUNCH") != nullptr;
    const bool in_launch = !two_launches && a.splitk_counters && nblocks <= a.splitk_ncounters;
    if ((!DUAL || in_launch) && a.splitk_ws && mud_aligned16(a.splitk_ws) && cm_split_eligible(a)) ns = cm_splits(nblocks, k16s);
    if (ns > 1 && a.splitk_ws_bytes < cm_slab_bytes(ns, nblocks, 64 * WM * WN * 32 * MT * (DUAL ? 2 : 1))) ns = 1;
    MUD_REQUIRE(ns == 1 || !a.res_up2, "mud_conv2d_mfma: res_up2 is not built for a launch split over K (ask mud_conv2d_mfma_res_up2_supported first)");
    MUD_REQUIRE(ns == 1 || !a.in_up2, "mud_conv2d_mfma: in_up2 is not built for a launch split over K (ask mud_conv2d_mfma_in_up2_supported first)");
    if (ns > 1) {
      mud_conv_args p = a;
      p.out = (float*)a.splitk_ws;
      p.ldo = a.Cout;
      p.bias = p.bias2 = p.res = nullptr;
      p.out_scale = 1.0f;
      p.act = MUD_ACT_NONE;
      p.stats = nullptr;
      const int64_t stride = npix * a.Cout;
      if (in_launch) {
        hipLaunchKernelGGL((k_conv_mfma<KS, MT, WM, WN, PRO, DUAL, PREC>), dim3((unsigned)(nblocks * ns)), dim3(64 * WM * WN), lds, s, a, tiles_x,
                           (int)tiles, ntiles, k16s, (unsigned)(nblocks * ns), ns, (int64_t)0, CmFin{(float*)a.splitk_ws, a.splitk_counters});
        MUD_CHECK_LAUNCH("mud_conv2d_mfma(split-K, reduced in the launch)");
        return MUD_OK;
      }
      hipLaunchKernelGGL((k_conv_mfma<KS, MT, WM, WN, PRO, DUAL, PREC>), dim3((unsigned)(nblocks * ns)), dim3(64 * WM * WN), lds, s, p, tiles_x,
                         (int)tiles, ntiles, k16s, (unsigned)(nblocks * ns), ns, stride, CmFin{nullptr, nullptr});
      MUD_CHECK_LAUNCH("mud_conv2d_mfma(split-K)");
      const int64_t HW = (int64_t)a.H * a.W;
      int ppb = 32;
      while (ppb > 1 && HW % ppb) ppb >>= 1;
      hipLaunchKernelGGL(k_splitk_epilogue, dim3((unsigned)mud_cdiv(npix, ppb)), dim3(256), 0, s, a, (const float*)a.splitk_ws, ns, stride, a.Cout,
                         npix, ppb);
      MUD_CHECK_LAUNCH("mud_conv2d_mfma(split-K epilogue)");
      return MUD_OK;
    }
    hipLaunchKernelGGL((k_conv_mfma<KS, MT, WM, WN, PRO, DUAL, PREC>), dim3((unsigned)nblocks), dim3(64 * WM * WN), lds, s, a, tiles_x, (int)tiles,
                       ntiles, k16s, (unsigned)nblocks, 1, (int64_t)0, CmFin{nullptr, nullptr});
  } else
    hipLaunchKernelGGL((k_conv_mfma_regb<KS, MT, PRO>), dim3((unsigned)nblocks), dim3(256), lds, s, a, tiles_x, (int)tiles, ntiles, k16s,
                       (unsigned)nblocks);
  MUD_CHECK_LAUNCH("mud_conv2d_mfma");
  return MUD_OK;
}

template <int KS, int MT, int WM = 4, int WN = 1, int PREC = MUD_PREC_16X3>
static int cm_launch(const mud_conv_args& a, hipStream_t s) {
  switch (a.pro_mode) {
    case MUD_PRO_NONE: return cm_launch_pro<KS, MT, WM, WN, MUD_PRO_NONE, false, PREC>(a, s);
    case MUD_PRO_AFFINE: return cm_launch_pro<KS, MT, WM, WN, MUD_PRO_AFFINE, false, PREC>(a, s);
    case MUD_PRO_LRELU: return cm_launch_pro<KS, MT, WM, WN, MUD_PRO_LRELU, false, PREC>(a, s);
    default: return cm_launch_pro<KS, MT, WM, WN, MUD_PRO_AFFINE_SILU, false, PREC>(a, s);
  }
}

#ifdef MUD_EXPERIMENT_WS
#include "experiments/conv_ws.inc"
#endif

enum { CMV_8X2, CMV_16X1, CMV_MT2, CMV_MT1, CMV_8X1R };
static int cm_variant3(const mud_conv_args& a, int64_t* blocks) {
  const int64_t ntiles = mud_cdiv(a.Cout, CM_BN);
  int64_t nb;
  int v;
  const int64_t blocks8 = mud_cdiv(a.W, 32) * mud_cdiv(a.H, 8) * (ntiles / 2) * a.B;
  const int64_t blocks16 = mud_cdiv(a.W, 32) * mud_cdiv(a.H, 16) * ntiles * a.B;
  const int64_t blocks2 = mud_cdiv(a.W, 32) * mud_cdiv(a.H, 8) * ntiles * a.B;
  static const bool no16 = getenv("MUD_CONV_NO16") != nullptr;
  static const bool no8x1r = getenv("MUD_CONV_NO8X1R") != nullptr;
  if (!no8x1r && !a.skip_w && ntiles == 1 && a.Cin <= 64 && a.H >= 8 && blocks2 >= 512) v = CMV_8X1R, nb = blocks2;
  else if (ntiles % 2 == 0 && a.H >= 8 && blocks8 >= 256) v = CMV_8X2, nb = blocks8;
  else if (!no16 && a.H >= 16 && blocks16 >= 256) v = CMV_16X1, nb = blocks16;
  else if (blocks2 >= 512 && a.H >= 8) v = CMV_MT2, nb = blocks2;
  else v = CMV_MT1, nb = mud_cdiv(a.W, 32) * mud_cdiv(a.H, 4) * ntiles * a.B;
  if (blocks) *blocks = nb;
  return v;
}

extern "C" int64_t mud_conv2d_mfma_splitk_bytes(const mud_conv_args* ap) {
  if (!ap || ap->ks != 3 || ap->B <= 0 || ap->H <= 0 || ap->W <= 0 || ap->Cin <= 0 || ap->Cout <= 0 || !cm_split_eligible(*ap)) return 0;
  int64_t blocks = 0;
  int v = cm_variant3(*ap, &blocks);
  if (ap->skip_w) {
    if (!ap->splitk_counters) return 0;
    if (v != CMV_8X2 && v != CMV_16X1) {
      v = CMV_MT1;
      blocks = mud_cdiv(ap->W, 32) * mud_cdiv(ap->H, 4) * mud_cdiv(ap->Cout, CM_BN) * ap->B;
    }
  }
  const int ns = cm_splits(blocks, (int)mud_cdiv(ap->Cin, 16));
  const int tile_words = ((v == CMV_8X2 || v == CMV_16X1) ? 512 * 64 : v == CMV_MT2 ? 256 * 64 : v == CMV_8X1R ? 512 * 32 : 256 * 32) * (ap->skip_w ? 2 : 1);
  return ns > 1 ? cm_slab_bytes(ns, blocks, tile_words) : 0;
}

extern "C" int mud_conv2d_mfma_res_up2_supported(const mud_conv_args* ap) {
  if (!ap || ap->ks != 3 || ap->stride != 1 || ap->pad != 1 || ap->sub2 || ap->skip_w || ap->pro_mode != MUD_PRO_AFFINE_SILU) return 0;
  if (ap->B <= 0 || ap->H <= 0 || ap->W <= 0 || ap->Cin <= 0 || ap->Cout <= 0 || (ap->H & 1) || (ap->W & 1)) return 0;
  int64_t blocks = 0;
  cm_variant3(*ap, &blocks);
  return cm_splits(blocks, (int)mud_cdiv(ap->Cin, 16)) == 1;
}

static bool cm_in_up2_built(int variant, int prec) {
  if (variant == CMV_8X2) return prec == MUD_PREC_16X3 || prec == MUD_PREC_FP8X || prec == MUD_PREC_16X1;
  return variant == CMV_MT1 && (prec == MUD_PREC_16X3 || prec == MUD_PREC_16X1);
}
extern "C" int mud_conv2d_mfma_in_up2_supported(const mud_conv_args* ap) {
  if (!ap || ap->ks != 3 || ap->stride != 1 || ap->pad != 1 || ap->sub2 || ap->skip_w || ap->res_up2 || ap->pro_mode != MUD_PRO_AFFINE_SILU) return 0;
  if (ap->B <= 0 || ap->H <= 0 || ap->W <= 0 || ap->Cin <= 0 || ap->Cout <= 0 || (ap->H & 1) || (ap->W & 1)) return 0;
  static const bool forced_tile = getenv("MUD_CONV_MT") != nullptr;
  if (forced_tile) return 0;
  int64_t blocks = 0;
  const int v = cm_variant3(*ap, &blocks);
  return cm_in_up2_built(v, ap->prec) && cm_splits(blocks, (int)mud_cdiv(ap->Cin, 16)) == 1;
}

static bool cm_fp8x_built(const mud_conv_args& a) {
  if (a.ks != 3 || a.sub2 || (a.pro_mode != MUD_PRO_NONE && a.pro_mode != MUD_PRO_AFFINE_SILU)) return false;
  if (a.skip_w && a.pro_mode != MUD_PRO_AFFINE_SILU) return false;
  const int v = cm_variant3(a, nullptr);
  return v == CMV_8X2 || v == CMV_16X1 || v == CMV_8X1R;
}
extern "C" int mud_conv2d_mfma_prec_supported(const mud_conv_args* ap, int prec) {
  if (!ap || ap->B <= 0 || ap->H <= 0 || ap->W <= 0 || ap->Cin <= 0 || ap->Cout <= 0) return 0;
  if (prec == MUD_PREC_16X3) return ap->ks == 1 || ap->ks == 3;
  if (prec == MUD_PREC_16X1)
    return ap->ks == 3 && ap->pro_mode >= MUD_PRO_NONE && ap->pro_mode <= MUD_PRO_LRELU && (!ap->skip_w || ap->pro_mode == MUD_PRO_AFFINE_SILU);
  mud_conv_args a = *ap;
  a.prec = prec;
  return prec == MUD_PREC_FP8X && cm_fp8x_built(a);
}

extern "C" int mud_conv2d_mfma(const mud_conv_args* ap, void* stream) {
  MUD_REQUIRE(ap, "mud_conv2d_mfma: null args");
  mud_conv_args a = *ap;
  MUD_REQUIRE(a.x && a.w && a.out, "mud_conv2d_mfma: null pointer");
  MUD_REQUIRE((a.ks == 1 || a.ks == 3) && a.stride == 1 && a.pad == a.ks / 2, "mud_conv2d_mfma: only ks in {1,3}, stride 1, pad ks/2 (got ks=%d stride=%d pad=%d)", a.ks, a.stride, a.pad);
  MUD_REQUIRE(a.B >= 0 && a.H > 0 && a.W > 0 && a.Cin > 0 && a.Cout > 0, "mud_conv2d_mfma: bad sizes");
  MUD_REQUIRE(a.Cin % 4 == 0 && a.ldx % 4 == 0 && a.ldx >= a.Cin && mud_aligned16(a.x), "mud_conv2d_mfma: needs Cin%%4==0 (Cin=%d), ldx%%4==0 (ldx=%d), 16-byte aligned x", a.Cin, a.ldx);
  MUD_REQUIRE((int64_t)a.H * a.W * a.ldx < 0x7fffffffLL, "mud_conv2d_mfma: one image must stay below 2^31 elements");
  MUD_REQUIRE(mud_aligned16(a.w) && a.w_bstride % 16 == 0, "mud_conv2d_mfma: packed weights must be 16-byte aligned");
  MUD_REQUIRE(a.ldo >= a.Cout && (!a.res || a.ldr >= a.Cout), "mud_conv2d_mfma: bad output/residual view");
  MUD_REQUIRE(!a.stats || a.stats_ld >= a.Cout, "mud_conv2d_mfma: bad stats view");
  MUD_REQUIRE(!a.sub2 || (a.ks == 3 && (a.H & 1) && (a.W & 1)), "mud_conv2d_mfma: sub2 needs ks == 3 and odd H, W");
  MUD_REQUIRE(a.emul_cout >= 0 && a.emul_cout <= a.Cout, "mud_conv2d_mfma: emul_cout out of range");
  MUD_REQUIRE((!a.emul || a.ld_emul >= (a.emul_cout > 0 ? a.emul_cout : a.Cout)) && (!a.egate || (a.eother && a.ld_egate >= a.Cout && a.ld_eother >= a.Cout)), "mud_conv2d_mfma: bad emul / egate / eother view");
  MUD_REQUIRE(a.pro_mode >= MUD_PRO_NONE && a.pro_mode <= MUD_PRO_LRELU, "mud_conv2d_mfma: unknown prologue mode %d", a.pro_mode);
  if ((a.pro_mode == MUD_PRO_AFFINE || a.pro_mode == MUD_PRO_AFFINE_SILU) && a.gn_sums) {
    MUD_REQUIRE(a.Cin <= CM_GN_MAXC && a.gn_G > 0 && a.Cin % a.gn_G == 0 && a.gn_sums_ld >= a.Cin && a.gn_count > 0,
                "mud_conv2d_mfma: folded GroupNorm needs Cin <= %d, Cin %% gn_G == 0, gn_sums_ld >= Cin, gn_count > 0 (Cin=%d gn_G=%d)", CM_GN_MAXC, a.Cin, a.gn_G);
    MUD_REQUIRE((a.gn_gamma == nullptr) == (a.gn_beta == nullptr) && a.gn_bstride >= 0, "mud_conv2d_mfma: folded GroupNorm: gamma and beta come together");
    a.pro_scale = a.pro_shift = a.x;
    a.pro_ld = 0;
  } else if (a.pro_mode == MUD_PRO_AFFINE || a.pro_mode == MUD_PRO_AFFINE_SILU) {
    a.gn_sums = nullptr;
    MUD_REQUIRE(a.pro_scale && a.pro_shift && a.pro_ld >= a.Cin && a.pro_ld % 4 == 0 && mud_aligned16(a.pro_scale) && mud_aligned16(a.pro_shift),
                "mud_conv2d_mfma: prologue arrays missing or misaligned");
    MUD_REQUIRE(a.Cin <= CM_GN_MAXC, "mud_conv2d_mfma: a launch with prologue arrays takes Cin <= %d (the kernels keep them in LDS; Cin=%d)", CM_GN_MAXC, a.Cin);
  } else {
    a.pro_scale = a.pro_shift = a.x;
    a.pro_ld = 0;
    a.gn_sums = nullptr;
  }
  if (a.skip_w) {
    MUD_REQUIRE(a.ks == 3 && a.pro_mode == MUD_PRO_AFFINE_SILU && !a.res && !a.sub2 && !a.emul && !a.egate,
                "mud_conv2d_mfma: the fused skip conv needs ks == 3, the AFFINE_SILU prologue and a plain epilogue");
    MUD_REQUIRE(a.skip_out && a.Cin <= 512 && a.Cout % 4 == 0 && a.skip_ldo >= a.Cout && a.skip_ldo % 4 == 0 && a.ldo % 4 == 0 &&
                mud_aligned16(a.skip_w) && mud_aligned16(a.skip_out) && mud_aligned16(a.out),
                "mud_conv2d_mfma: fused skip conv needs Cin <= 512, Cout %% 4 == 0 and aligned float4 output rows (Cin=%d Cout=%d)", a.Cin, a.Cout);
  }
  if (a.res_up2) {
    MUD_REQUIRE(a.ks == 3 && a.res && !a.sub2 && !a.skip_w && (a.H & 1) == 0 && (a.W & 1) == 0 && a.pro_mode == MUD_PRO_AFFINE_SILU,
                "mud_conv2d_mfma: res_up2 needs ks == 3, the AFFINE_SILU prologue, a residual, no sub2 / fused skip conv and even H, W (ks=%d H=%d W=%d sub2=%d pro_mode=%d)",
                a.ks, a.H, a.W, a.sub2, a.pro_mode);
    MUD_REQUIRE((int64_t)(a.H / 2) * (a.W / 2) * a.ldr < 0x7fffffffLL, "mud_conv2d_mfma: res_up2: one low-resolution image must stay below 2^31 elements");
  }
  MUD_REQUIRE(a.prec == MUD_PREC_16X3 || a.prec == MUD_PREC_FP8X || a.prec == MUD_PREC_16X1, "mud_conv2d_mfma: unknown arithmetic plan prec=%d", a.prec);
  if (a.in_up2) {
    MUD_REQUIRE(a.ks == 3 && !a.sub2 && !a.skip_w && !a.res_up2 && (a.H & 1) == 0 && (a.W & 1) == 0 && a.pro_mode == MUD_PRO_AFFINE_SILU,
                "mud_conv2d_mfma: in_up2 needs ks == 3, the AFFINE_SILU prologue, no sub2 / fused skip conv / res_up2 and even H, W (ks=%d H=%d W=%d sub2=%d pro_mode=%d)",
                a.ks, a.H, a.W, a.sub2, a.pro_mode);
    MUD_REQUIRE(cm_in_up2_built(cm_variant3(a, nullptr), a.prec),
                "mud_conv2d_mfma: in_up2 is not built for the tile / arithmetic plan of this launch (prec=%d; ask mud_conv2d_mfma_in_up2_supported first)", a.prec);
  }
  MUD_REQUIRE(a.prec != MUD_PREC_16X1 || a.ks == 3, "mud_conv2d_mfma: MUD_PREC_16X1 is built for ks == 3 only (got ks=%d)", a.ks);
  MUD_REQUIRE(a.prec != MUD_PREC_FP8X || (cm_fp8x_built(a) && a.w_exp >= -100 && a.w_exp <= 100),
              "mud_conv2d_mfma: MUD_PREC_FP8X is not built for this launch (ask mud_conv2d_mfma_prec_supported first; the weights were packed for it and cannot be read by another plan)");
  if (a.B == 0) return MUD_OK;
  hipStream_t s = (hipStream_t)stream;
  if (a.in_up2) {
    constexpr int PU = MUD_PRO_UP2_AFFINE_SILU;
    if (cm_variant3(a, nullptr) == CMV_8X2)
      return a.prec == MUD_PREC_FP8X   ? cm_launch_pro<3, 2, 4, 2, PU, false, MUD_PREC_FP8X>(a, s)
             : a.prec == MUD_PREC_16X1 ? cm_launch_pro<3, 2, 4, 2, PU, false, MUD_PREC_16X1>(a, s)
                                       : cm_launch_pro<3, 2, 4, 2, PU>(a, s);
    return a.prec == MUD_PREC_16X1 ? cm_launch_pro<3, 1, 4, 1, PU, false, MUD_PREC_16X1>(a, s) : cm_launch_pro<3, 1, 4, 1, PU>(a, s);
  }
#ifdef MUD_EXPERIMENT_WS
  if (cm_ws_wanted(a)) return cm_ws_dispatch(a, s);
#endif
  if (a.prec == MUD_PREC_FP8X) {
    const int v8 = cm_variant3(a, nullptr);
    if (v8 == CMV_8X1R) return a.pro_mode == MUD_PRO_NONE ? cm_launch_pro<3, 1, 8, 1, MUD_PRO_NONE, false, MUD_PREC_FP8X>(a, s) : cm_launch_pro<3, 1, 8, 1, MUD_PRO_AFFINE_SILU, false, MUD_PREC_FP8X>(a, s);
    const bool x2 = v8 == CMV_8X2;
    if (a.skip_w) return x2 ? cm_launch_pro<3, 2, 4, 2, MUD_PRO_AFFINE_SILU, true, MUD_PREC_FP8X>(a, s) : cm_launch_pro<3, 2, 8, 1, MUD_PRO_AFFINE_SILU, true, MUD_PREC_FP8X>(a, s);
    if (a.pro_mode == MUD_PRO_NONE) return x2 ? cm_launch_pro<3, 2, 4, 2, MUD_PRO_NONE, false, MUD_PREC_FP8X>(a, s) : cm_launch_pro<3, 2, 8, 1, MUD_PRO_NONE, false, MUD_PREC_FP8X>(a, s);
    return x2 ? cm_launch_pro<3, 2, 4, 2, MUD_PRO_AFFINE_SILU, false, MUD_PREC_FP8X>(a, s) : cm_launch_pro<3, 2, 8, 1, MUD_PRO_AFFINE_SILU, false, MUD_PREC_FP8X>(a, s);
  }
  if (a.prec == MUD_PREC_16X1) {
    constexpr int P1 = MUD_PREC_16X1;
    if (a.skip_w) {
      switch (cm_variant3(a, nullptr)) {
        case CMV_8X2: return cm_launch_pro<3, 2, 4, 2, MUD_PRO_AFFINE_SILU, true, P1>(a, s);
        case CMV_16X1: return cm_launch_pro<3, 2, 8, 1, MUD_PRO_AFFINE_SILU, true, P1>(a, s);
        default: return cm_launch_pro<3, 1, 4, 1, MUD_PRO_AFFINE_SILU, true, P1>(a, s);
      }
    }
    switch (cm_variant3(a, nullptr)) {
      case CMV_8X2: return cm_launch<3, 2, 4, 2, P1>(a, s);
      case CMV_16X1: return cm_launch<3, 2, 8, 1, P1>(a, s);
      case CMV_MT2: return cm_launch<3, 2, 4, 1, P1>(a, s);
      case CMV_8X1R: return cm_launch<3, 1, 8, 1, P1>(a, s);
      default: return cm_launch<3, 1, 4, 1, P1>(a, s);
    }
  }
  const int64_t ntiles = mud_cdiv(a.Cout, CM_BN);
  static const int force_mt = getenv("MUD_CONV_MT") ? atoi(getenv("MUD_CONV_MT")) : 0;
  if (force_mt && !a.skip_w) {
    if (a.ks == 3) return (force_mt == 8 && ntiles % 2 == 0) ? cm_launch<3, 2, 4, 2>(a, s) : force_mt == 16 ? cm_launch<3, 2, 8, 1>(a, s) : force_mt == 1 ? cm_launch<3, 1>(a, s) : cm_launch<3, 2>(a, s);
    return cm_launch<1, 1>(a, s);
  }
  if (a.ks == 3 && a.skip_w) {
    switch (cm_variant3(a, nullptr)) {
      case CMV_8X2: return cm_launch_pro<3, 2, 4, 2, MUD_PRO_AFFINE_SILU, true>(a, s);
      case CMV_16X1: return cm_launch_pro<3, 2, 8, 1, MUD_PRO_AFFINE_SILU, true>(a, s);
      default: return cm_launch_pro<3, 1, 4, 1, MUD_PRO_AFFINE_SILU, true>(a, s);
    }
  }
  if (a.ks == 3) {
    switch (cm_variant3(a, nullptr)) {
      case CMV_8X2: return cm_launch<3, 2, 4, 2>(a, s);
      case CMV_16X1: return cm_launch<3, 2, 8, 1>(a, s);
      case CMV_MT2: return cm_launch<3, 2>(a, s);
      case CMV_8X1R: return cm_launch<3, 1, 8, 1>(a, s);
      default: return cm_launch<3, 1>(a, s);
    }
  }
  return cm_launch<1, 1>(a, s);
}
```

mu-diff_amd/mudiff_hip/__init__.py:

```python
from __future__ import annotations

import ctypes as C
import os

import torch

_HERE = os.path.dirname(os.path.abspath(__file__))
_SHIPPED = os.path.join(_HERE, 'libmudiff_hip.so')
_LIB_PATH = os.environ.get('MUDIFF_HIP_LIB', _SHIPPED)
_lib = None
PREC_16X3, PREC_FP8X, PREC_16X1 = 0, 1, 2

ACT_NONE, ACT_SIGMOID, ACT_TANH, ACT_SILU, ACT_LRELU = 0, 1, 2, 3, 4
PRO_NONE, PRO_AFFINE, PRO_AFFINE_SILU, PRO_LRELU = 0, 1, 2, 3


class MudiffHipError(RuntimeError):
    pass


class ConvArgs(C.Structure):
    _fields_ = [
        ('x', C.c_void_p), ('B', C.c_int), ('H', C.c_int), ('W', C.c_int), ('Cin', C.c_int), ('ldx', C.c_int),
        ('w', C.c_void_p), ('w_bstride', C.c_int64),
        ('ks', C.c_int), ('stride', C.c_int), ('pad', C.c_int),
        ('pro_scale', C.c_void_p), ('pro_shift', C.c_void_p), ('pro_ld', C.c_int), ('pro_mode', C.c_int),
        ('bias', C.c_void_p),
        ('bias2', C.c_void_p), ('bias2_ld', C.c_int),
        ('res', C.c_void_p), ('ldr', C.c_int),
        ('out_scale', C.c_float), ('act', C.c_int),
        ('emul', C.c_void_p), ('ld_emul', C.c_int), ('egate', C.c_void_p), ('ld_egate', C.c_int), ('eother', C.c_void_p), ('ld_eother', C.c_int),
        ('out', C.c_void_p), ('Cout', C.c_int), ('ldo', C.c_int),
        ('sub2', C.c_int),
        ('stats', C.c_void_p), ('stats_ld', C.c_int),
        ('emul_cout', C.c_int),
        ('gn_sums', C.c_void_p), ('gn_sums_ld', C.c_int), ('gn_G', C.c_int), ('gn_eps', C.c_float), ('gn_count', C.c_double),
        ('gn_gamma', C.c_void_p), ('gn_beta', C.c_void_p), ('gn_bstride', C.c_int64),
        ('splitk_ws', C.c_void_p), ('splitk_ws_bytes', C.c_int64),
        ('splitk_counters', C.c_void_p), ('splitk_ncounters', C.c_int),
        ('skip_w', C.c_void_p), ('skip_bias', C.c_void_p), ('skip_out', C.c_void_p), ('skip_ldo', C.c_int),
        ('prec', C.c_int), ('w_exp', C.c_int),
        ('res_up2', C.c_int), ('res_k', C.c_float * 4),
        ('in_up2', C.c_int), ('in_k', C.c_float * 4),
    ]


MLP_MAX_LAYERS = 6


class MlpArgs(C.Structure):
    _fields_ = [
        ('x', C.c_void_p), ('ldx', C.c_int), ('B', C.c_int),
        ('nlayers', C.c_int), ('dims', C.c_int * (MLP_MAX_LAYERS + 1)),
        ('W', C.c_void_p * MLP_MAX_LAYERS), ('b', C.c_void_p * MLP_MAX_LAYERS),
        ('pixel_norm', C.c_int), ('act', C.c_int), ('act_last', C.c_int),
        ('out', C.c_void_p), ('ldo', C.c_int), ('maxdim', C.c_int),
    ]


class CensusArgs(C.Structure):
    _fields_ = [
        ('x', C.c_void_p), ('B', C.c_int), ('H', C.c_int), ('W', C.c_int), ('C', C.c_int), ('ldx', C.c_int),
        ('pro_scale', C.c_void_p), ('pro_shift', C.c_void_p), ('pro_ld', C.c_int), ('pro_mode', C.c_int),
    ]


class CensusOut(C.Structure):
    _fields_ = [('n', C.c_uint64), ('n_over', C.c_uint64), ('n_under', C.c_uint64), ('n_fp16_over', C.c_uint64), ('amax_bits', C.c_uint64)]


VI_MAX_RANKS, VI_WINDOW = 4, 16
NIFTI_U1, NIFTI_I2, NIFTI_I4, NIFTI_F4, NIFTI_U2 = 2, 4, 8, 16, 512


class VolumeCensusRecord(C.Structure):
    _fields_ = [('n', C.c_uint64), ('n_nonfinite', C.c_uint64), ('min', C.c_float), ('max', C.c_float),
                ('count', C.c_int32 * VI_MAX_RANKS), ('first_rank', C.c_int64 * VI_MAX_RANKS),
                ('window', (C.c_float * VI_WINDOW) * VI_MAX_RANKS)]


class BandTables(C.Structure):
    _fields_ = [('m', C.c_int), ('n', C.c_int), ('bw', C.c_int), ('nnz', C.c_int),
                ('start', C.c_void_p), ('member', C.c_void_p), ('w', C.c_void_p),
                ('tstart', C.c_void_p), ('tmember', C.c_void_p), ('tw', C.c_void_p), ('lc', C.c_void_p)]


_P, _I, _L, _F, _D = C.c_void_p, C.c_int, C.c_int64, C.c_float, C.c_double
_SIGNATURES = {
    'mud_version': (C.c_int, []),
    'mud_last_error': (C.c_char_p, []),
    'mud_build_flags': (C.c_char_p, []),
    'mud_posterior_sample': (_I, [_P, _P, _P, _P, _P, _P, _P, _P, _I, _P, _I, _L, _P]),
    'mud_q_sample': (_I, [_P, _P, _P, _I, _P, _P, _I, _P, _I, _L, _P]),
    'mud_timestep_embedding': (_I, [_P, _P, _I, _I, _F, _P]),
    'mud_pixel_norm': (_I, [_P, _P, _I, _I, _P]),
    'mud_dense': (_I, [_P, _I, _P, _P, _P, _I, _I, _I, _I, _I, _I, _P]),
    'mud_mlp_chain': (_I, [C.POINTER(MlpArgs), _P]),
    'mud_mlp_chains': (_I, [C.POINTER(MlpArgs), _I, _P]),
    'mud_gn_ws_bytes': (_L, [_I, _L, _I, _I]),
    'mud_gn_scale_shift': (_I, [_P, _I, _L, _I, _I, _I, _F, _P, _P, _L, _P, _P, _I, _P, _P, _P]),
    'mud_gn_scale_shift_from_sums': (_I, [_P, _I, _I, _I, _I, C.c_double, _F, _P, _P, _L, _P, _P, _I, _P]),
    'mud_channel_mean': (_I, [_P, _I, _L, _I, _I, _P, _I, _P, _P]),
    'mud_conv2d_direct': (_I, [C.POINTER(ConvArgs), _P]),
    'mud_packed_weight_bytes': (_L, [_I, _I, _I]),
    'mud_pack_weights': (_I, [_P, _L, _L, _L, _L, _I, _I, _I, _I, _P, _P]),
    'mud_pack_weights_prec': (_I, [_P, _L, _L, _L, _L, _I, _I, _I, _I, _I, _I, _P, _P]),
    'mud_packed_weight_bytes_prec': (_L, [_I, _I, _I, _I]),
    'mud_conv2d_mfma': (_I, [C.POINTER(ConvArgs), _P]),
    'mud_conv2d_mfma_prec_supported': (_I, [C.POINTER(ConvArgs), _I]),
    'mud_conv2d_mfma_splitk_bytes': (_L, [C.POINTER(ConvArgs)]),
    'mud_conv2d_mfma_res_up2_supported': (_I, [C.POINTER(ConvArgs)]),
    'mud_conv2d_mfma_in_up2_supported': (_I, [C.POINTER(ConvArgs)]),
    'mud_upfirdn2d': (_I, [_P, _L, _I, _I, _P, _I, _I, _I, _I, _I, _I, _I, _I, _I, _I, _P, _P]),
    'mud_fir_nhwc': (_I, [_P, _I, _I, _I, _I, _I, C.POINTER(C.c_float), _I, _I, _I, _I, _I, _I, _P, _P, _I, _I, _P, _I, _P, _I, _P]),
    'mud_minibatch_stddev': (_I, [_P, _I, _L, _I, _I, _I, _P, _P]),
    'mud_attention_supported': (_I, [_I]),
    'mud_attention_ws_bytes': (_L, [_I, _I, _I]),
    'mud_attention': (_I, [_P, _I, _I, _I, _I, _F, _P, _I, _P, _P]),
    'mud_softmax_rows': (_I, [_P, _L, _I, _I, _P]),
    'mud_mul': (_I, [_P, _I, _P, _I, _P, _I, _L, _I, _P]),
    'mud_gate_mix': (_I, [_P, _I, _P, _I, _P, _I, _P, _I, _I, _L, _I, _P, _I, _P]),
    'mud_fourier_embedding': (_I, [_P, _P, _P, _I, _I, _P]),
    'mud_resize_bilinear': (_I, [_P, _L, _I, _I, _I, _I, _P, _P]),
    'mud_affine_clamp': (_I, [_P, _L, _F, _F, _F, _F, _P, _P]),
    'mud_e4m3_census': (_I, [C.POINTER(CensusArgs), _P, _P]),
    'mud_value_range_ws_bytes': (_L, []),
    'mud_value_range': (_I, [_P, _L, _P, _L, _P, _P, _P]),
    'mud_quantize_u8': (_I, [_P, _L, _F, _F, _P, _P]),
    'mud_slice_metrics_ws_bytes': (_L, [_I, _I, _I]),
    'mud_slice_metrics_u8': (_I, [_P, _P, _I, _I, _I, _P, _P, _P, _P, _L, _P]),
    'mud_volume_metrics_ws_bytes': (_L, [_I, _I, _I, _I]),
    'mud_volume_metrics': (_I, [_P, _P, _P, _P, _I, _I, _I, _I, _P, _P, _L, _P]),
    'mud_lpips_packed_bytes': (_L, []),
    'mud_lpips_pack': (_I, [_P, _P, _P, _P, _P, _P]),
    'mud_lpips_ws_bytes': (_L, [_I, _I, _I]),
    'mud_lpips_u8': (_I, [_P, _P, _I, _I, _I, _P, _P, _P, _L, _P]),
    'mud_randn_keyed': (_I, [_P, _I, _L, _P, C.c_uint64, _I, _I, _P]),
    'mud_ensemble_stats': (_I, [_P, _I, _I, _L, _F, _F, _F, _F, _P, _P, _P]),
    'mud_ensemble_quantiles': (_I, [_P, _I, _I, _L, _F, _F, _F, _F, C.POINTER(C.c_double), _I, _P, _P]),
    'mud_volume_interval_coverage': (_I, [_P, _P, _P, _P, _I, _I, _I, _I, _I, _I, _P, _P, _P, _L, _P]),
    'mud_randn_keyed_coupled': (_I, [_P, _I, _L, _P, C.c_uint64, _I, _I, C.POINTER(C.c_double), _I, _P]),
    'mud_known_constrain': (_I, [_P, _P, _P, _P, _P, C.c_uint64, _I, _I, _P, _I, _P, _P, _I, _I, _P, _I, _L, _P]),
    'mud_known_coverage': (_I, [C.POINTER(C.c_double), _I, _I, _I, _I, _I, _I, _P, _P]),
    'mud_fft2_c2c': (_I, [_P, _P, _I, _I, _I, _P]),
    'mud_fft2_r2c': (_I, [_P, _P, _I, _I, _I, _P]),
    'mud_kspace_constrain': (_I, [_P, _P, _P, _I, _P, _P, C.c_uint64, _I, _I, _P, _I, _P, _P, _I, _I, _P, _P, _I, _I, _P]),
    'mud_slab_constrain': (_I, [_P, _P, _P, _P, _P, _I, _I, _P, _P, C.c_uint64, _I, _I, _P, _I, _P, _P, _I, _I, _P, _I, _L, _P]),
    'mud_slab_average': (_I, [_P, _P, _P, _I, _I, _P, _I, _L, _P]),
    'mud_slab_kspace_constrain': (_I, [_P, _P, _P, _I, _P, _P, _P, _I, _I, _P, _P, C.c_uint64, _I, _I, _P, _I, _P, _P, _I, _I, _P, _P, _I, _I,
                                        _P]),
    'mud_band_constrain': (_I, [_P, _P, C.POINTER(BandTables), _P, _P, C.c_uint64, _I, _I, _P, _I, _P, _P, _I, _I, _P, _P, _I, _L, _P]),
    'mud_band_measure': (_I, [_P, C.POINTER(BandTables), _P, _I, _L, _P]),
    'mud_volume_through_plane': (_I, [_P, _P, _I, _I, _I, _I, _I, _P, _P, _L, _P]),
    'mud_volume_census_ws_bytes': (_L, []),
    'mud_volume_census': (_I, [_P, _I, _I, _I, _I, _F, _F, C.POINTER(C.c_double), _I, _P, _P, _L, _P]),
    'mud_volume_slab_normalise': (_I, [_P, _I, _I, _I, _I, _F, _F, _F, _F, _I, _I, _I, _P, _P]),
    'mud_volume_slab_zscore': (_I, [_P, _I, _I, _I, _I, _F, _F, _F, _F, _I, _I, _P, _P]),
    'mud_volume_assemble': (_I, [_P, _P, _I, _I, _I, _I, _I, _P, _P, _P]),
    'mud_volume_regrid': (_I, [_P, _I, _I, _I, _I, _F, _F, C.POINTER(C.c_double), _I, _I, _I, _I, _P, _P]),
    'mud_volume_bspline_coeffs': (_I, [_P, _I, _I, _I, _I, _F, _F, _P, _P, _P]),
    'mud_volume_regrid_cubic': (_I, [_P, _I, _I, _I, _P, _I, _F, _F, C.POINTER(C.c_double), _D, _D, _I, _I, _I, _P, _P]),
    'mud_volume_joint_hist': (_I, [_P, _I, _I, _I, _I, _F, _F, _P, _I, _I, _I, _I, _F, _F, C.POINTER(C.c_double), _I, _D, _D, _D, _D, _I, _P, _P]),
    'mud_volume_mirror_moments': (_I, [_P, _I, _I, _I, _I, _F, _F, _P, _I, _I, _D, _D, _I, _P, _P]),
    'mud_volume_bias_log': (_I, [_P, _I, _I, _I, _I, _F, _F, _I, _P, _P]),
    'mud_volume_bias_corrected': (_I, [_P, _P, _P, _P, _I, _I, _I, _I, _I, _P, _P]),
    'mud_volume_bias_hist': (_I, [_P, _L, _D, _D, _I, _P, _P]),
    'mud_volume_bias_fit': (_I, [_P, _P, _I, _D, _D, _I, _I, _I, _I, _I, _I, _P, _P]),
    'mud_volume_bias_apply': (_I, [_P, _I, _I, _I, _I, _F, _F, _P, _I, _I, _P, _P]),
    'mud_volume_denoise_residual': (_I, [_P, _I, _I, _I, _I, _F, _F, _P, _P]),
    'mud_volume_denoise_select_hist': (_I, [_P, _L, C.c_uint32, _I, _P, _P]),
    'mud_volume_denoise_nlm': (_I, [_P, _I, _I, _I, _I, _F, _F, _I, _I, _D, _D, _I, _P, _P, _P]),
    'mud_volume_fg_range': (_I, [_P, _I, _I, _I, _I, _F, _F, _P, _P]),
    'mud_volume_fg_hist': (_I, [_P, _I, _I, _I, _I, _F, _F, _D, _D, _I, _P, _P]),
    'mud_volume_fg_mask': (_I, [_P, _I, _I, _I, _I, _F, _F, _D, _D, _I, _I, _P, _P]),
    'mud_volume_fg_morph': (_I, [_P, _I, _I, _I, _I, _P, _P]),
    'mud_volume_fg_label': (_I, [_P, _I, _I, _I, _I, _P, _P]),
    'mud_volume_fg_census': (_I, [_P, _I, _I, _I, _P, _P, _P]),
    'mud_volume_fg_select': (_I, [_P, _P, _L, _I, _I, _P, _P, _P]),
    'mud_volume_fg_apply': (_I, [_P, _I, _I, _I, _I, _F, _F, _P, _P, _P, _P]),
    'mud_volume_edt': (_I, [_P, _I, _I, _I, _I, _D, _D, _D, _P, _P]),
    'mud_volume_edt_select': (_I, [_P, _L, _D, _I, _P, _P, _P, _P]),
    'mud_volume_reorient': (_I, [_P, _I, _I, _I, _I, _I, _I, _I, _I, _P, _P]),
    'mud_volume_lowpass': (_I, [_P, _I, _I, _I, _I, _F, _F, C.POINTER(C.c_double), _I, C.POINTER(C.c_double), _I, C.POINTER(C.c_double), _I, _P, _P, _P, _P]),
}
EXPORTED_SYMBOLS = tuple(_SIGNATURES)


def lib_path():
    return _LIB_PATH


def load():
    global _lib
    if _lib is None:
        allow = os.environ.get('MUDIFF_ALLOW_VARIANT', '0') == '1'
        if os.path.realpath(_LIB_PATH) != os.path.realpath(_SHIPPED) and not allow:
            raise MudiffHipError(f'MUDIFF_HIP_LIB={_LIB_PATH} is not the shipped library ({_SHIPPED}); '
                                 'set MUDIFF_ALLOW_VARIANT=1 to run an experiment build')
        if not os.path.isfile(_LIB_PATH):
            raise MudiffHipError(
                f'{_LIB_PATH} not found: build it with `make -C mu-diff_amd/csrc` (or __graft_entry__.build()). '
                'There is no CPU / PyTorch fallback for the MU-Diff sampling path.')
        lib = C.CDLL(_LIB_PATH)
        for name, (res, args) in _SIGNATURES.items():
            fn = getattr(lib, name)
            fn.restype, fn.argtypes = res, args
        flags = lib.mud_build_flags().decode()
        if flags and not allow:
            raise MudiffHipError(f'{_LIB_PATH} is an experiment build ({flags}); set MUDIFF_ALLOW_VARIANT=1 to run it')
        _lib = lib
    return _lib


def check(code, what=''):
    if code != 0:
        raise MudiffHipError(f'{what or "libmudiff_hip"} failed ({code}): {load().mud_last_error().decode()}')


def stream_ptr(device=None):
    return C.c_void_p(torch.cuda.current_stream(device).cuda_stream)


def require_gpu(*tensors):
    dev = None
    for t in tensors:
        if t is None:
            continue
        if not t.is_cuda:
            raise MudiffHipError('the MU-Diff HIP path needs tensors on an MI355X (got a CPU tensor); there is no CPU fallback')
        if dev is None:
            dev = t.device
        elif t.device != dev:
            raise MudiffHipError(f'operands of one launch live on different GPUs ({dev} and {t.device})')


def ptr(t):
    return None if t is None else C.c_void_p(t.data_ptr())
```

mu-diff_amd/mudiff_hip/ops.py:

```python
from __future__ import annotations

import collections
import ctypes as C
import math
import os

import numpy as np
import torch

from . import (ACT_LRELU, ACT_NONE, ACT_SIGMOID, ACT_SILU, ACT_TANH, PREC_16X1, PREC_16X3, PREC_FP8X, PRO_AFFINE, PRO_AFFINE_SILU, PRO_LRELU,
               PRO_NONE, ConvArgs, MudiffHipError, check, load, ptr, require_gpu)


DETERMINISTIC = os.environ.get('MUD_DETERMINISTIC', '0') == '1'


class StatsArena:

    def __init__(self, device, chunk_doubles=1 << 18):
        self.device, self.chunk = device, chunk_doubles
        self.buf, self.used = None, 0

    def take(self, B, C):
        if DETERMINISTIC:
            return None
        n = B * C * 2
        if self.buf is None or self.used + n > self.buf.numel():
            self.buf = torch.zeros(max(self.chunk, n), device=self.device, dtype=torch.float64)
            self.used = 0
        t = self.buf[self.used:self.used + n].view(B, C, 2)
        self.used += n
        return t


class View:
    __slots__ = ('base', 'B', 'H', 'W', 'C', 'ld', 'c0', 'stats')

    def __init__(self, base, B, H, W, C, ld=None, c0=0, stats=None):
        self.base, self.B, self.H, self.W, self.C = base, B, H, W, C
        self.ld = C if ld is None else ld
        self.c0 = c0
        self.stats = stats

    @staticmethod
    def empty(B, H, W, C, device, arena=None):
        v = View(torch.empty(B, H, W, C, device=device, dtype=torch.float32), B, H, W, C)
        if arena is not None:
            v.stats = arena.take(B, C)
        return v

    @property
    def stats_ptr(self):
        return None if self.stats is None else C.c_void_p(self.stats.data_ptr() + 16 * self.c0)

    @staticmethod
    def from_nchw(x):
        require_gpu(x)
        B, Cc, H, W = x.shape
        x = x.float()
        t = x.reshape(B, H, W, 1) if Cc == 1 else x.permute(0, 2, 3, 1)
        return View(t.contiguous(), B, H, W, Cc)

    def to_nchw(self):
        t = self.tensor()
        if self.C == 1:
            return t.reshape(self.B, 1, self.H, self.W)
        return t.permute(0, 3, 1, 2).contiguous()

    def tensor(self):
        return self.base.reshape(self.B, self.H, self.W, self.ld)[..., self.c0:self.c0 + self.C]

    def up2_shape(self):
        return View(self.base, self.B, 2 * self.H, 2 * self.W, self.C, self.ld, self.c0)

    def slice(self, c0, C_):
        assert 0 <= c0 and c0 + C_ <= self.C
        return View(self.base, self.B, self.H, self.W, C_, self.ld, self.c0 + c0, self.stats)

    @property
    def ptr(self):
        return C.c_void_p(self.base.data_ptr() + 4 * self.c0)

    @property
    def npix(self):
        return self.B * self.H * self.W

    @property
    def device(self):
        return self.base.device


class _Profile:

    def __init__(self):
        self.on = False
        self.records = []

    def enable(self):
        self.on, self.records = True, []

    def disable(self):
        self.on = False

    def summary(self):
        torch.cuda.synchronize()
        out = {}
        for name, e0, e1, flops, nbytes in self.records:
            d = out.setdefault(name, dict(n=0, ms=0.0, flops=0.0, bytes=0.0))
            d['n'] += 1
            d['ms'] += e0.elapsed_time(e1)
            d['flops'] += flops
            d['bytes'] += nbytes
        return out


PROFILE = _Profile()


STREAM = object()


def _launch(name, dev, fn, *args, flops=0.0, nbytes=0.0):
    idx = torch.cuda.current_device() if dev.index is None else dev.index
    if idx != torch.cuda.current_device():
        with torch.cuda.device(idx):
            return _launch(name, dev, fn, *args, flops=flops, nbytes=nbytes)
    args = tuple(C.c_void_p(torch.cuda.current_stream().cuda_stream) if a_ is STREAM else a_ for a_ in args)
    if PROFILE.on:
        e0, e1 = torch.cuda.Event(enable_timing=True), torch.cuda.Event(enable_timing=True)
        e0.record()
        code = fn(*args)
        e1.record()
        PROFILE.records.append((name, e0, e1, flops, nbytes))
    else:
        code = fn(*args)
    check(code, name)


def _f32(t):
    assert t.dtype == torch.float32 and t.is_contiguous(), (t.dtype, t.is_contiguous())
    return t


def posterior_sample(x01, x02, xt, noise, t, coef1, coef2, std_tab, out=None):
    require_gpu(x01, xt, noise, t, coef1)
    B = xt.shape[0]
    per = xt[0].numel() if B else 0
    x01, xt, noise = _f32(x01.contiguous()), _f32(xt.contiguous()), _f32(noise.contiguous())
    if x02 is not None:
        x02 = _f32(x02.contiguous())
        assert x02.shape == xt.shape
    assert x01.shape == xt.shape == noise.shape and t.dtype == torch.int64 and t.numel() == B
    out = torch.empty_like(xt) if out is None else out
    _launch('posterior_sample', xt.device, load().mud_posterior_sample, ptr(x01), ptr(x02), ptr(xt), ptr(noise), ptr(t.contiguous()), ptr(coef1), ptr(coef2),
                                      ptr(std_tab), coef1.numel(), ptr(out), B, per, STREAM)
    return out


def q_sample(x, noise, t, toff, a_tab, s_tab):
    require_gpu(x, noise, t, a_tab, s_tab)
    x, noise = _f32(x.contiguous()), _f32(noise.contiguous())
    B = x.shape[0]
    out = torch.empty_like(x)
    _launch('q_sample', x.device, load().mud_q_sample, ptr(x), ptr(noise), ptr(t.contiguous()), toff, ptr(a_tab), ptr(s_tab), a_tab.numel(), ptr(out), B,
                              x[0].numel() if B else 0, STREAM)
    return out


def timestep_embedding(t, dim, max_positions=10000.0):
    require_gpu(t)
    assert t.dim() == 1 and t.dtype == torch.int64
    out = torch.empty(t.shape[0], dim, device=t.device, dtype=torch.float32)
    _launch('timestep_embedding', t.device, load().mud_timestep_embedding, ptr(t.contiguous()), ptr(out), t.shape[0], dim, float(max_positions), STREAM)
    return out


def fourier_embedding(t, W):
    require_gpu(t, W)
    tf, Wf = _f32(t.float().contiguous()), _f32(W.detach().float().contiguous())
    out = torch.empty(tf.shape[0], 2 * Wf.shape[0], device=t.device, dtype=torch.float32)
    _launch('fourier_embedding', t.device, load().mud_fourier_embedding, ptr(tf), ptr(Wf), ptr(out), tf.shape[0], Wf.shape[0], STREAM)
    return out


def pixel_norm(z):
    require_gpu(z)
    z = _f32(z.contiguous())
    out = torch.empty_like(z)
    _launch('pixel_norm', z.device, load().mud_pixel_norm, ptr(z), ptr(out), z.shape[0], z.shape[1], STREAM)
    return out


def dense(x, W, bias, act_in=ACT_NONE, act_out=ACT_NONE):
    require_gpu(x, W)
    assert x.dim() == 2 and x.stride(1) == 1 and W.is_contiguous() and x.shape[1] == W.shape[1]
    B, K = x.shape
    N = W.shape[0]
    out = torch.empty(B, N, device=x.device, dtype=torch.float32)
    _launch('dense', x.device, load().mud_dense, ptr(x), x.stride(0) if B > 1 else K, ptr(W), ptr(bias), ptr(out), N, B, K, N, act_in, act_out,
                           STREAM)
    return out


def _mlp_args(a, x, layers, pixel_norm, act, act_last):
    from . import MLP_MAX_LAYERS
    require_gpu(x, *[w for w, _ in layers])
    assert x.dim() == 2 and x.stride(1) == 1 and 1 <= len(layers) <= MLP_MAX_LAYERS
    xin = x if x.dtype == torch.float32 else x.float()
    a.x, a.ldx, a.B, a.nlayers = ptr(xin), (xin.stride(0) if xin.shape[0] > 1 else xin.shape[1]), xin.shape[0], len(layers)
    a.dims[0] = xin.shape[1]
    keep = [xin]
    for l, (w, b) in enumerate(layers):
        w = _f32(w.detach().contiguous())
        assert w.shape[1] == a.dims[l], (tuple(w.shape), a.dims[l])
        a.dims[l + 1] = w.shape[0]
        a.W[l] = w.data_ptr()
        if b is not None:
            b = _f32(b.detach().contiguous())
            a.b[l] = b.data_ptr()
        keep += [w, b]
    a.pixel_norm, a.act, a.act_last = int(pixel_norm), act, int(act_last)
    out = torch.empty(xin.shape[0], a.dims[len(layers)], device=x.device, dtype=torch.float32)
    a.out, a.ldo = ptr(out), out.shape[1]
    return out, keep


def mlp_chain(x, layers, *, pixel_norm=False, act=ACT_SILU, act_last=False):
    return mlp_chains([dict(x=x, layers=layers, pixel_norm=pixel_norm, act=act, act_last=act_last)])[0]


def mlp_chains(chains):
    from . import MlpArgs
    assert 1 <= len(chains) <= 4
    arr = (MlpArgs * len(chains))()
    outs, keep = [], []
    for a, c in zip(arr, chains):
        o, k = _mlp_args(a, c['x'], c['layers'], c.get('pixel_norm', False), c.get('act', ACT_SILU), c.get('act_last', False))
        outs.append(o)
        keep.append(k)
    require_gpu(*[c['x'] for c in chains])
    _launch('mlp_chain', chains[0]['x'].device, load().mud_mlp_chains, arr, len(chains), STREAM)
    return outs


_WS = {}


def _workspace(device, nbytes):
    ws = _WS.get(device)
    if ws is None or ws.numel() < nbytes:
        ws = torch.empty(max(nbytes, 1 << 20), device=device, dtype=torch.uint8)
        _WS[device] = ws
    return ws


def gn_scale_shift(x: View, G, gamma=None, beta=None, eps=1e-6):
    lib = load()
    HW = x.H * x.W
    ss = torch.empty(2, x.B, x.C, device=x.device, dtype=torch.float32)
    bstride = 0
    if gamma is not None:
        assert gamma.stride(-1) == 1 and beta.stride(-1) == 1 and gamma.shape[-1] == x.C
        if gamma.dim() == 2:
            assert gamma.shape[0] == x.B and gamma.stride(0) == beta.stride(0)
            bstride = gamma.stride(0)
    if x.stats is not None:
        _launch('gn_from_sums', x.device, lib.mud_gn_scale_shift_from_sums, x.stats_ptr, x.stats.shape[1], x.B, x.C, G, float(HW), eps, ptr(gamma),
                ptr(beta), bstride, ptr(ss[0]), ptr(ss[1]), x.C, STREAM)
        return ss[0], ss[1]
    ws = _workspace(x.device, lib.mud_gn_ws_bytes(x.B, HW, x.C, G))
    _launch('gn_scale_shift', x.device, lib.mud_gn_scale_shift, x.ptr, x.B, HW, x.C, x.ld, G, eps, ptr(gamma), ptr(beta), bstride, ptr(ss[0]),
            ptr(ss[1]), x.C, None, ptr(ws), STREAM, nbytes=4.0 * x.npix * x.C)
    return ss[0], ss[1]


class LazyGN:
    __slots__ = ('x', 'G', 'gamma', 'beta', 'bstride', 'eps', '_ss')

    def __init__(self, x: View, G, gamma, beta, bstride, eps):
        self.x, self.G, self.gamma, self.beta, self.bstride, self.eps, self._ss = x, G, gamma, beta, bstride, eps, None

    def tensors(self):
        if self._ss is None:
            x = self.x
            ss = torch.empty(2, x.B, x.C, device=x.device, dtype=torch.float32)
            _launch('gn_from_sums', x.device, load().mud_gn_scale_shift_from_sums, x.stats_ptr, x.stats.shape[1], x.B, x.C, self.G,
                    float(x.H * x.W), self.eps, ptr(self.gamma), ptr(self.beta), self.bstride, ptr(ss[0]), ptr(ss[1]), x.C, STREAM)
            self._ss = (ss[0], ss[1])
        return self._ss

    def __iter__(self):
        return iter(self.tensors())


def gn_lazy(x: View, G, gamma=None, beta=None, eps=1e-6):
    if x.stats is None or not FOLD_GN:
        return gn_scale_shift(x, G, gamma, beta, eps)
    bstride = 0
    if gamma is not None:
        assert gamma.stride(-1) == 1 and beta.stride(-1) == 1 and gamma.shape[-1] == x.C
        if gamma.dim() == 2:
            assert gamma.shape[0] == x.B and gamma.stride(0) == beta.stride(0)
            bstride = gamma.stride(0)
    return LazyGN(x, G, gamma, beta, bstride, eps)


FOLD_GN = os.environ.get('MUD_FOLD_GN', '1') != '0'


FUSE_SKIP = os.environ.get('MUD_FUSE_SKIP', '1') != '0'


_SPLITK_COUNTERS = {}
_SPLITK_OWNED = []


def new_splitk_counters(device):
    return torch.zeros(4096, device=device, dtype=torch.int32)


class own_splitk_counters:

    def __init__(self, buf):
        self.buf = buf

    def __enter__(self):
        _SPLITK_OWNED.append(self.buf)
        return self.buf

    def __exit__(self, *exc):
        _SPLITK_OWNED.pop()
        return False


def splitk_counters(device):
    if _SPLITK_OWNED and _SPLITK_OWNED[-1].device == torch.device(device):
        return _SPLITK_OWNED[-1]
    key = (device.index if device.index is not None else torch.cuda.current_device(), torch.cuda.current_stream(device).cuda_stream)
    buf = _SPLITK_COUNTERS.get(key)
    if buf is None:
        buf = _SPLITK_COUNTERS[key] = new_splitk_counters(device)
    return buf


def conv3x3_would_split_k(x: View, cout):
    a = ConvArgs()
    a.x, a.B, a.H, a.W, a.Cin, a.ldx, a.ks, a.stride, a.pad = x.ptr, x.B, x.H, x.W, x.C, x.ld, 3, 1, 1
    a.out, a.Cout, a.ldo = x.ptr, cout, (cout + 3) & ~3
    return load().mud_conv2d_mfma_splitk_bytes(C.byref(a)) > 0


FUSE_SKIP_SPLIT = os.environ.get('MUD_FUSE_SKIP_SPLIT', '1') != '0'


def fused_skip_ok(x: View, cout, pro_mode):
    return (FUSE_SKIP and pro_mode == PRO_AFFINE_SILU and x.C % 4 == 0 and 8 <= x.C <= 512 and cout % 4 == 0
            and (FUSE_SKIP_SPLIT or not conv3x3_would_split_k(x, cout)))


RES_UP2 = os.environ.get('MUD_RES_UP2', '1') != '0'


def up2_taps(kernel2d, up, down, pad):
    k = np.asarray(kernel2d, dtype=np.float32)
    if k.shape != (4, 4) or (up, down, tuple(pad)) != (2, 1, (2, 1)) or not float(k.sum()) > 0.0:
        return None
    t = (k.sum(axis=1) / np.sqrt(k.sum())).astype(np.float32)
    return tuple(float(v) for v in t) if np.array_equal(np.outer(t, t).astype(np.float32), k) else None


def res_up2_ok(B, H, W, cin, cout):
    if not RES_UP2 or cin % 4 or cout % 4:
        return False
    a = ConvArgs()
    a.B, a.H, a.W, a.Cin, a.ldx, a.ks, a.stride, a.pad, a.Cout, a.ldo, a.pro_mode = B, H, W, cin, cin, 3, 1, 1, cout, cout, PRO_AFFINE_SILU
    return bool(load().mud_conv2d_mfma_res_up2_supported(C.byref(a)))


IN_UP2 = os.environ.get('MUD_IN_UP2', '1') != '0'


def in_up2_ok(B, H, W, cin, cout, prec=PREC_16X3):
    if not IN_UP2 or cin % 4 or cout % 4:
        return False
    a = ConvArgs()
    a.B, a.H, a.W, a.Cin, a.ldx, a.ks, a.stride, a.pad, a.Cout, a.ldo, a.pro_mode, a.prec = B, H, W, cin, cin, 3, 1, 1, cout, cout, PRO_AFFINE_SILU, prec
    return bool(load().mud_conv2d_mfma_in_up2_supported(C.byref(a)))


def resolve_pro(pro):
    if pro is not None and isinstance(pro[0], LazyGN):
        sc, sh = pro[0].tensors()
        return (sc, sh, pro[2])
    return pro


def channel_mean(x: View):
    lib = load()
    HW = x.H * x.W
    ws = _workspace(x.device, lib.mud_gn_ws_bytes(x.B, HW, x.C, x.C))
    out = torch.empty(x.B, x.C, device=x.device, dtype=torch.float32)
    _launch('channel_mean', x.device, lib.mud_channel_mean, x.ptr, x.B, HW, x.C, x.ld, ptr(out), x.C, ptr(ws), STREAM, nbytes=4.0 * x.npix * x.C)
    return out


def pack_weights(src, s_tap, s_ci, s_co, ks, Cin, Cout, nbatch=1, src_bstride=0, src_offset=0, prec=PREC_16X3, w_exp=0):
    lib = load()
    require_gpu(src)
    nbytes = lib.mud_packed_weight_bytes_prec(ks, Cin, Cout, prec)
    if nbytes < 0:
        raise MudiffHipError(f'pack_weights: plan {prec} has no packed form for ks={ks}')
    dst = torch.empty(nbatch, nbytes, device=src.device, dtype=torch.uint8)
    _launch('pack_weights', src.device, lib.mud_pack_weights_prec, C.c_void_p(src.data_ptr() + 4 * src_offset), s_tap, s_ci, s_co, src_bstride, ks, Cin, Cout,
            nbatch, prec, w_exp, ptr(dst), STREAM)
    return dst


def fp8x_weight_exponent(w):
    m = float(w.detach().abs().max())
    if not (m > 0.0) or not math.isfinite(m):
        return 0
    return max(-100, min(100, int(math.floor(math.log2(448.0 / m)))))


def pack_conv_weight(w_oihw, prec=PREC_16X3, w_exp=0):
    O, I, k, _ = w_oihw.shape
    w = _f32(w_oihw.detach().contiguous())
    return pack_weights(w, 1, k * k, I * k * k, k, I, O, prec=prec, w_exp=w_exp)


def pack_matrix_in_out(W_in_out):
    I, O = W_in_out.shape
    return pack_weights(_f32(W_in_out.detach().contiguous()), 0, O, 1, 1, I, O)


def direct_weight(w_oihw):
    return w_oihw.detach().permute(2, 3, 1, 0).contiguous()


PREC_PLAN = os.environ.get('MUD_PREC_PLAN', 'auto')


def fp8x_pays(B, H, W, cin, cout):
    return True


PREC_PLANS = ('off', 'auto', 'all', 'fp16')


class prec_plan:

    def __init__(self, name):
        if name not in PREC_PLANS:
            raise ValueError(f'prec_plan: unknown plan {name!r} (one of {PREC_PLANS})')
        self.name, self._saved = name, None

    def __enter__(self):
        global PREC_PLAN
        self._saved, PREC_PLAN = PREC_PLAN, self.name
        return self

    def __exit__(self, *exc):
        global PREC_PLAN
        PREC_PLAN = self._saved
        return False


def conv_prec_supported(x: View, cout, pro_mode, prec, skip=False, sub2=False):
    a = ConvArgs()
    a.x, a.B, a.H, a.W, a.Cin, a.ldx, a.ks, a.stride, a.pad = x.ptr, x.B, x.H, x.W, x.C, x.ld, 3, 1, 1
    a.out, a.Cout, a.ldo, a.pro_mode, a.sub2 = x.ptr, cout, (cout + 3) & ~3, pro_mode, int(sub2)
    if skip:
        a.skip_w = x.ptr
    return bool(load().mud_conv2d_mfma_prec_supported(C.byref(a), prec))


def choose_prec(x: View, cout, pro_mode, *, skip=False, sub2=False, w_bstride=0):
    if PREC_PLAN == 'off' or w_bstride or x.C % 4:
        return PREC_16X3
    if PREC_PLAN == 'fp16':
        return PREC_16X1 if conv_prec_supported(x, cout, pro_mode, PREC_16X1, skip=skip, sub2=sub2) else PREC_16X3
    if PREC_PLAN != 'all' and not fp8x_pays(x.B, x.H, x.W, x.C, cout):
        return PREC_16X3
    return PREC_FP8X if conv_prec_supported(x, cout, pro_mode, PREC_FP8X, skip=skip, sub2=sub2) else PREC_16X3


Launch = collections.namedtuple('Launch', 'layer ks mfma prec shape sub2 skip pro')


RECORD = None


def conv(x: View, w, ks, Cout, *, mfma, stride=1, pad=None, pro=None, bias=None, bias2=None, res: View = None,
         out_scale=1.0, act=ACT_NONE, out: View = None, w_bstride=0, arena=None, sub2=False, emul: View = None, gate=None, emul_cout=0,
         skip=None, prec=PREC_16X3, w_exp=0, layer=None, res_up2=None, split_k=True, in_up2=None):
    if in_up2 is not None:
        assert mfma and ks == 3 and stride == 1 and not sub2 and skip is None and res_up2 is None and len(in_up2) == 4
        assert pro is not None and pro[2] == PRO_AFFINE_SILU
        x_lo, x = x, x.up2_shape()
    if RECORD is not None:
        if torch.cuda.is_current_stream_capturing():
            raise RuntimeError('precision.launch_record() is eager only: the launch is being captured into a graph')
        RECORD.append(Launch(layer, ks, bool(mfma), prec, (x.B, x.H, x.W, x.C, Cout), bool(sub2), skip is not None,
                             PRO_NONE if pro is None else pro[2]))
    lib = load()
    pad = ks // 2 if pad is None else pad
    Ho = (x.H + 2 * pad - ks) // stride + 1
    Wo = (x.W + 2 * pad - ks) // stride + 1
    if sub2:
        assert mfma and ks == 3 and stride == 1 and x.H % 2 == 1 and x.W % 2 == 1
        Ho, Wo = x.H // 2, x.W // 2
    if out is None:
        out = View.empty(x.B, Ho, Wo, Cout, x.device, arena)
    assert (out.B, out.H, out.W, out.C) == (x.B, Ho, Wo, Cout), ((out.B, out.H, out.W, out.C), (x.B, Ho, Wo, Cout))
    a = ConvArgs()
    a.x, a.B, a.H, a.W, a.Cin, a.ldx = x.ptr, x.B, x.H, x.W, x.C, x.ld
    a.w, a.w_bstride = ptr(w), w_bstride
    a.ks, a.stride, a.pad = ks, stride, pad
    keep = None
    if pro is not None and isinstance(pro[0], LazyGN) and not (mfma and x.C <= 1024 and pro[0].x.stats is not None):
        pro = resolve_pro(pro)
    if pro is not None and pro[2] == PRO_LRELU:
        a.pro_mode = PRO_LRELU
    elif pro is not None and isinstance(pro[0], LazyGN):
        gn = keep = pro[0]
        assert gn.x.C == x.C and gn.x.B == x.B
        a.pro_mode = pro[2]
        a.gn_sums, a.gn_sums_ld, a.gn_G, a.gn_eps, a.gn_count = gn.x.stats_ptr, gn.x.stats.shape[1], gn.G, gn.eps, float(gn.x.H * gn.x.W)
        a.gn_gamma, a.gn_beta, a.gn_bstride = ptr(gn.gamma), ptr(gn.beta), gn.bstride
    elif pro is not None:
        sc, sh, mode = pro
        assert sc.shape == (x.B, x.C) and sc.stride(1) == 1 and sh.stride() == sc.stride()
        a.pro_scale, a.pro_shift, a.pro_ld, a.pro_mode = ptr(sc), ptr(sh), sc.stride(0), mode
    else:
        a.pro_mode = PRO_NONE
    if bias is not None:
        assert bias.numel() == Cout and bias.is_contiguous()
        a.bias = ptr(bias)
    if bias2 is not None:
        assert bias2.shape == (x.B, Cout) and bias2.stride(1) == 1
        a.bias2, a.bias2_ld = ptr(bias2), bias2.stride(0)
    if res is not None:
        if res_up2 is not None:
            assert mfma and Ho % 2 == 0 and Wo % 2 == 0 and (res.B, res.H, res.W, res.C) == (x.B, Ho // 2, Wo // 2, Cout) and len(res_up2) == 4
            a.res_up2, a.res_k = 1, (C.c_float * 4)(*res_up2)
        else:
            assert (res.B, res.H, res.W, res.C) == (x.B, Ho, Wo, Cout)
        a.res, a.ldr = res.ptr, res.ld
    if in_up2 is not None:
        a.in_up2, a.in_k = 1, (C.c_float * 4)(*in_up2)
    a.out_scale, a.act = out_scale, act
    a.sub2 = 1 if sub2 else 0
    if emul is not None:
        assert (emul.B, emul.H, emul.W, emul.C) == (x.B, Ho, Wo, emul_cout or Cout)
        a.emul, a.ld_emul, a.emul_cout = emul.ptr, emul.ld, emul_cout
    if gate is not None:
        gv, ov = gate
        assert (gv.B, gv.H, gv.W, gv.C) == (x.B, Ho, Wo, Cout) == (ov.B, ov.H, ov.W, ov.C)
        a.egate, a.ld_egate, a.eother, a.ld_eother = gv.ptr, gv.ld, ov.ptr, ov.ld
    a.out, a.Cout, a.ldo = out.ptr, Cout, out.ld
    a.prec, a.w_exp = prec, w_exp
    if out.stats is not None:
        a.stats, a.stats_ld = out.stats_ptr, out.stats.shape[1]
    skip_flops = 0.0
    if skip is not None:
        sw, sb, so = skip
        assert mfma and ks == 3 and res is None and (so.B, so.H, so.W, so.C) == (x.B, Ho, Wo, Cout)
        a.skip_w, a.skip_bias, a.skip_out, a.skip_ldo = ptr(sw), ptr(sb), so.ptr, so.ld
        skip_flops = 2.0 * x.B * Ho * Wo * Cout * x.C
    if mfma and ks == 3 and split_k and res_up2 is None and in_up2 is None:
        cnt = splitk_counters(x.device)
        a.splitk_counters, a.splitk_ncounters = ptr(cnt), cnt.numel()
        nws = lib.mud_conv2d_mfma_splitk_bytes(C.byref(a))
        if nws > 0:
            keep = (keep, torch.empty(nws, device=x.device, dtype=torch.uint8))
            a.splitk_ws, a.splitk_ws_bytes = ptr(keep[1]), nws
    fn = lib.mud_conv2d_mfma if mfma else lib.mud_conv2d_direct
    name = (f'conv_mfma_k{ks}' if mfma else f'conv_direct_k{ks}') + {PREC_FP8X: '_fp8x', PREC_16X1: '_fp16'}.get(prec, '')
    flops = 2.0 * x.B * Ho * Wo * Cout * x.C * ks * ks + skip_flops
    nbytes = 4.0 * ((x_lo if in_up2 is not None else x).npix * x.C + out.npix * Cout * ((2 if res is not None else 1) + (1 if skip is not None else 0))) + (w.numel() * w.element_size() if w_bstride == 0 else x.B * w_bstride)
    _launch(name, x.device, fn, C.byref(a), STREAM, flops=flops, nbytes=nbytes)
    return out


CENSUS_FIELDS = ('n', 'n_over', 'n_under', 'n_fp16_over', 'amax_bits')


def new_census_slot(device):
    return torch.zeros(len(CENSUS_FIELDS), device=device, dtype=torch.int64)


def e4m3_census(x: View, pro, out):
    from . import CensusArgs
    require_gpu(x.base, out)
    assert out.dtype == torch.int64 and out.numel() == len(CENSUS_FIELDS) and out.is_contiguous()
    a = CensusArgs()
    a.x, a.B, a.H, a.W, a.C, a.ldx = x.ptr, x.B, x.H, x.W, x.C, x.ld
    if pro is None:
        a.pro_mode = PRO_NONE
    else:
        sc, sh, mode = resolve_pro(pro)
        a.pro_mode = mode
        if mode != PRO_NONE:
            assert sc.shape == (x.B, x.C) and sc.stride(1) == 1 and sh.stride() == sc.stride(), (tuple(sc.shape), sc.stride(), sh.stride())
            a.pro_scale, a.pro_shift, a.pro_ld = ptr(sc), ptr(sh), sc.stride(0)
    _launch('e4m3_census', x.device, load().mud_e4m3_census, C.byref(a), ptr(out), STREAM, nbytes=4.0 * x.npix * x.C)
    return out


def upfirdn2d_planes(x, kernel, up, down, pad):
    require_gpu(x, kernel)
    N, Cc, H, W = x.shape
    xin = _f32(x.float().contiguous())
    k = _f32(kernel.float().contiguous())
    kh, kw = k.shape
    (ux, uy), (dx, dy), (px0, px1, py0, py1) = up, down, pad
    Ho = (H * uy + py0 + py1 - kh) // dy + 1
    Wo = (W * ux + px0 + px1 - kw) // dx + 1
    out = torch.empty(N, Cc, Ho, Wo, device=x.device, dtype=torch.float32)
    _launch('upfirdn2d', x.device, load().mud_upfirdn2d, ptr(xin), N * Cc, H, W, ptr(k), kh, kw, ux, uy, dx, dy, px0, px1, py0, py1, ptr(out), STREAM)
    return out.to(x.dtype)


def fir_nhwc(x: View, kernel2d, up, down, pad, pro=None, want_h=True, want_x=False):
    import numpy as np
    k = np.ascontiguousarray(kernel2d, dtype=np.float32)
    kh, kw = k.shape
    Ho = (x.H * up + pad[0] + pad[1] - kh) // down + 1
    Wo = (x.W * up + pad[0] + pad[1] - kw) // down + 1
    oh = View.empty(x.B, Ho, Wo, x.C, x.device) if want_h else None
    ox = View.empty(x.B, Ho, Wo, x.C, x.device) if want_x else None
    sc = sh = None
    ld = mode = 0
    if pro is not None:
        sc, sh, mode = resolve_pro(pro)
        ld = sc.stride(0)
    _launch('fir_nhwc', x.device, load().mud_fir_nhwc, x.ptr, x.B, x.H, x.W, x.C, x.ld, k.ctypes.data_as(C.POINTER(C.c_float)), kh, kw, up, down,
            pad[0], pad[1], ptr(sc), ptr(sh), ld, mode, oh.ptr if oh else None, oh.ld if oh else 0, ox.ptr if ox else None,
            ox.ld if ox else 0, STREAM, nbytes=4.0 * x.C * (x.npix + x.B * Ho * Wo * (int(want_h) + int(want_x))))
    return oh, ox


def minibatch_stddev(x: View, group):
    out = torch.empty(x.B, device=x.device, dtype=torch.float32)
    _launch('minibatch_stddev', x.device, load().mud_minibatch_stddev, x.ptr, x.B, x.H * x.W, x.C, x.ld, group, ptr(out), STREAM)
    return out


def attention_supported(C_):
    return bool(load().mud_attention_supported(C_))


def attention(qkv: View, C_, scale):
    assert qkv.C == 3 * C_
    n = qkv.H * qkv.W
    out = View.empty(qkv.B, qkv.H, qkv.W, C_, qkv.device)
    nws = load().mud_attention_ws_bytes(qkv.B, n, C_)
    ws = torch.empty(nws // 4, device=qkv.device, dtype=torch.float32) if nws else None
    _launch('attention', qkv.device, load().mud_attention, qkv.ptr, qkv.B, n, C_, qkv.ld, float(scale), out.ptr, out.ld, ptr(ws) if nws else None,
            STREAM, flops=4.0 * qkv.B * n * n * C_)
    return out


def softmax_rows_(s, n):
    rows = s.numel() // n
    _launch('softmax_rows', s.device, load().mud_softmax_rows, ptr(s), rows, n, n, STREAM)
    return s


def mul(a: View, b: View, out: View = None):
    out = View.empty(a.B, a.H, a.W, a.C, a.device) if out is None else out
    _launch('mul', a.device, load().mud_mul, a.ptr, a.ld, b.ptr, b.ld, out.ptr, out.ld, a.npix, a.C, STREAM)
    return out


def gate_mix(g: View, att: View, other: View, out: View):
    _launch('gate_mix', g.device, load().mud_gate_mix, g.ptr, g.ld, att.ptr, att.ld, other.ptr, other.ld, out.ptr, out.ld, g.B, g.H * g.W, g.C,
            out.stats_ptr, out.stats.shape[1] if out.stats is not None else 0, STREAM)
    return out


def resize_bilinear(x, size):
    require_gpu(x)
    H, W = x.shape[-2:]
    Ho, Wo = int(size[0]), int(size[1])
    xin = _f32(x.float().contiguous())
    out = torch.empty(*x.shape[:-2], Ho, Wo, device=x.device, dtype=torch.float32)
    _launch('resize_bilinear', x.device, load().mud_resize_bilinear, ptr(xin), xin.numel() // (H * W), H, W, Ho, Wo, ptr(out), STREAM)
    return out


def affine_clamp(x, scale, shift, lo, hi):
    require_gpu(x)
    xin = _f32(x.float().contiguous())
    out = torch.empty_like(xin)
    _launch('affine_clamp', x.device, load().mud_affine_clamp, ptr(xin), xin.numel(), float(scale), float(shift), float(lo), float(hi), ptr(out), STREAM)
    return out


def value_range(a, b=None):
    require_gpu(a, b)
    ain = _f32(a.contiguous())
    bin_ = None if b is None else _f32(b.contiguous())
    out = torch.empty(2, device=a.device, dtype=torch.float32)
    ws = torch.empty(load().mud_value_range_ws_bytes(), device=a.device, dtype=torch.uint8)
    _launch('value_range', a.device, load().mud_value_range, ptr(ain), ain.numel(), ptr(bin_), 0 if bin_ is None else bin_.numel(),
            ptr(out), ptr(ws), STREAM)
    return out


def quantize_u8(x, gmin, gmax):
    require_gpu(x)
    gmin, gmax = float(gmin), float(gmax)
    if not gmax > gmin:
        raise ValueError(f'quantize_u8: empty range [{gmin}, {gmax}] (use the (0, 1) fallback of the driver)')
    xin = _f32(x.contiguous())
    out = torch.empty(xin.shape, device=x.device, dtype=torch.uint8)
    _launch('quantize_u8', x.device, load().mud_quantize_u8, ptr(xin), xin.numel(), float(np.float32(gmin)), float(np.float32(gmax - gmin)),
            ptr(out), STREAM)
    return out


def slice_metrics_u8(pred, gt):
    require_gpu(pred, gt)
    if pred.dtype != torch.uint8 or gt.dtype != torch.uint8 or pred.dim() != 3 or pred.shape != gt.shape:
        raise MudiffHipError(f'slice_metrics_u8: need two uint8 [n, H, W] tensors of one shape (got {pred.dtype} {tuple(pred.shape)}, '
                             f'{gt.dtype} {tuple(gt.shape)})')
    n, H, W = pred.shape
    if H < 7 or W < 7:
        raise MudiffHipError(f'slice_metrics_u8: slices must be at least 7x7 (the SSIM window), got {H}x{W}')
    pin, gin = pred.contiguous(), gt.contiguous()
    sse = torch.empty(n, device=pred.device, dtype=torch.int64)
    sae = torch.empty(n, device=pred.device, dtype=torch.int64)
    ssim_sum = torch.empty(n, device=pred.device, dtype=torch.float64)
    if n == 0:
        return sse, sae, ssim_sum
    nbytes = load().mud_slice_metrics_ws_bytes(n, H, W)
    ws = torch.empty(nbytes, device=pred.device, dtype=torch.uint8)
    _launch('slice_metrics_u8', pred.device, load().mud_slice_metrics_u8, ptr(pin), ptr(gin), n, H, W, ptr(sse), ptr(sae), ptr(ssim_sum),
            ptr(ws), nbytes, STREAM)
    return sse, sae, ssim_sum


VM_N, VM_SSE, VM_SAE, VM_N_INT, VM_SSIM, VM_SS, VM_SS2, VM_SSE_STD = range(8)
VM_NQ, VM_MAX_REGIONS = 8, 8


def volume_metrics(pred, gt, region, std=None, nreg=VM_MAX_REGIONS):
    require_gpu(pred, gt, region, std)
    ts = [pred, gt] + ([] if std is None else [std])
    if any(t.dtype != torch.float32 for t in ts) or region.dtype != torch.uint8:
        raise MudiffHipError(f'volume_metrics: need fp32 pred / gt{" / std" if std is not None else ""} and a uint8 region '
                             f'(got {", ".join(str(t.dtype) for t in ts)}, {region.dtype})')
    if pred.dim() != 3 or any(t.shape != pred.shape for t in ts + [region]):
        raise MudiffHipError(f'volume_metrics: need [Z, X, Y] tensors of one shape (got {", ".join(str(tuple(t.shape)) for t in ts + [region])})')
    Z, X, Y = pred.shape
    if Z < 7 or X < 7 or Y < 7:
        raise MudiffHipError(f'volume_metrics: volumes must be at least 7x7x7 (the SSIM window), got {Z}x{X}x{Y}')
    if not 1 <= int(nreg) <= VM_MAX_REGIONS:
        raise MudiffHipError(f'volume_metrics: nreg must be in [1, {VM_MAX_REGIONS}] (got {nreg})')
    nreg = int(nreg)
    pin, gin, rin = pred.contiguous(), gt.contiguous(), region.contiguous()
    sin = None if std is None else std.contiguous()
    sums = torch.empty(Z, nreg, VM_NQ, device=pred.device, dtype=torch.float64)
    nbytes = load().mud_volume_metrics_ws_bytes(Z, X, Y, nreg)
    ws = torch.empty(nbytes, device=pred.device, dtype=torch.uint8)
    _launch('volume_metrics', pred.device, load().mud_volume_metrics, ptr(pin), ptr(gin), ptr(rin), ptr(sin), Z, X, Y, nreg, ptr(sums),
            ptr(ws), nbytes, STREAM, nbytes=float(pin.numel()) * (9 + (0 if sin is None else 4)))
    return sums


LPIPS_WS_CAP = 512 << 20


def lpips_pack(table, conv_w, conv_b, lin_w):
    require_gpu(table, *conv_w, *conv_b, *lin_w)
    table = _f32(table.contiguous())
    conv_w, conv_b, lin_w = ([_f32(t.contiguous()) for t in ts] for ts in (conv_w, conv_b, lin_w))
    packed = torch.empty(load().mud_lpips_packed_bytes(), device=table.device, dtype=torch.uint8)
    arr = lambda ts: (C.c_void_p * 5)(*[ptr(t) for t in ts])
    _launch('lpips_pack', table.device, load().mud_lpips_pack, ptr(table), arr(conv_w), arr(conv_b), arr(lin_w), ptr(packed), STREAM)
    return packed


def lpips_u8(pred_u8, gt_u8, net, max_ws_bytes=LPIPS_WS_CAP):
    require_gpu(pred_u8, gt_u8)
    if pred_u8.dtype != torch.uint8 or gt_u8.dtype != torch.uint8 or pred_u8.dim() != 3 or pred_u8.shape != gt_u8.shape:
        raise MudiffHipError(f'lpips_u8: need two uint8 [n, H, W] tensors of one shape (got {pred_u8.dtype} {tuple(pred_u8.shape)}, '
                             f'{gt_u8.dtype} {tuple(gt_u8.shape)})')
    n, H, W = pred_u8.shape
    if H < 31 or W < 31:
        raise MudiffHipError(f'lpips_u8: slices must be at least 31x31 (AlexNet\'s two pools), got {H}x{W}')
    packed = getattr(net, 'packed', None)
    if packed is None or packed.device != pred_u8.device:
        raise MudiffHipError(f'lpips_u8: the LPIPS weights are not packed on {pred_u8.device} (call net.to(device) first)')
    out = torch.empty(n, 5, device=pred_u8.device, dtype=torch.float64)
    if n == 0:
        return out
    lib = load()
    chunk = max(1, min(n, int(max_ws_bytes) // max(lib.mud_lpips_ws_bytes(1, H, W), 1)))
    nbytes = lib.mud_lpips_ws_bytes(chunk, H, W)
    ws = torch.empty(nbytes, device=pred_u8.device, dtype=torch.uint8)
    pin, gin = pred_u8.contiguous(), gt_u8.contiguous()
    for c0 in range(0, n, chunk):
        m = min(chunk, n - c0)
        _launch('lpips_u8', pred_u8.device, lib.mud_lpips_u8, ptr(pin[c0:c0 + m]), ptr(gin[c0:c0 + m]), m, H, W, ptr(packed),
                ptr(out[c0:c0 + m]), ptr(ws), nbytes, STREAM, flops=3.47e9 * m * (H * W / 65536.0))
    return out


def to_range_0_1(x):
    return affine_clamp(x, 0.5, 0.5, 0.0, 1.0)


INV_SQRT2 = 1.0 / math.sqrt(2.0)


KIND_X_INIT, KIND_Z, KIND_NOISE = 0, 1, 2
_MAX_SAMPLE = 1 << 31


def check_keys(keys):
    k = torch.as_tensor(keys).detach().to('cpu', torch.int64)
    if k.dim() != 2 or k.shape[1] != 2:
        raise MudiffHipError(f'randn_keyed: keys must be [rows, 2] = (slice, sample), got {tuple(k.shape)}')
    if k.numel() and int(k[:, 0].min()) < 0:
        raise MudiffHipError('randn_keyed: slice indices must be >= 0')
    if k.numel() and (int(k[:, 1].min()) < 0 or int(k[:, 1].max()) >= _MAX_SAMPLE):
        raise MudiffHipError('randn_keyed: sample indices must lie in [0, 2^31)')
    return k.contiguous()


def _seed64(seed):
    seed = int(seed)
    if not 0 <= seed < 1 << 64:
        raise MudiffHipError(f'randn_keyed: seed must lie in [0, 2^64), got {seed}')
    return seed


def randn_keyed_into(out, keys_dev, seed, step, kind):
    rows = keys_dev.shape[0]
    _launch('randn_keyed', out.device, load().mud_randn_keyed, ptr(out), rows, out.numel() // max(rows, 1), ptr(keys_dev), C.c_uint64(seed),
            int(step), int(kind), STREAM)
    return out


def randn_keyed(rows_keys, row_len, seed, step, kind, out=None):
    k = check_keys(rows_keys)
    seed = _seed64(seed)
    rows, row_len = k.shape[0], int(row_len)
    if out is None:
        dev = rows_keys.device if isinstance(rows_keys, torch.Tensor) and rows_keys.is_cuda else torch.device('cuda', torch.cuda.current_device())
        out = torch.empty(rows, row_len, device=dev, dtype=torch.float32)
    require_gpu(out)
    if out.dtype != torch.float32 or not out.is_contiguous() or out.numel() != rows * row_len:
        raise MudiffHipError(f'randn_keyed: out must be a contiguous fp32 tensor of {rows} x {row_len} elements, got {out.dtype} '
                             f'{tuple(out.shape)}')
    _launch('randn_keyed', out.device, load().mud_randn_keyed, ptr(out), rows, row_len, ptr(k.to(out.device)), C.c_uint64(seed), int(step),
            int(kind), STREAM)
    return out


COUPLING_MAX_RADIUS = 32


def coupling_taps_arg(half_taps, radius):
    from .slice_coupling import check_coupling
    try:
        half, R = check_coupling((half_taps, radius))
    except ValueError as e:
        raise MudiffHipError(f'randn_keyed_coupled: {e}') from None
    return (C.c_double * (R + 1))(*half.tolist()), R


def randn_keyed_coupled_into(out, keys_dev, seed, step, kind, taps, radius):
    rows = keys_dev.shape[0]
    _launch('randn_keyed_coupled', out.device, load().mud_randn_keyed_coupled, ptr(out), rows, out.numel() // max(rows, 1), ptr(keys_dev),
            C.c_uint64(seed), int(step), int(kind), taps, int(radius), STREAM)
    return out


def randn_keyed_coupled(rows_keys, row_len, seed, step, kind, half_taps, radius, out=None):
# ... 775 lines not shown
```

Before: 111.4 slices/s.

## Fold FIR blur into strided downsample conv via space-to-depth 3x3 MFMA

Down-sampling convs that first blur with a separable 4x4 FIR and then run a stride-2 3x3 conv are replaced by one stride-1 3x3 conv over a space-to-depth view of the input. The FIR taps are folded into 6x6 weights that are rearranged to 4*Cin channels, and the gather is done while the kernel stages its input. This removes the separate fir_nhwc pass and its intermediate tensor. In exchange the folded conv has four times the input channels, and a power-of-two weight pre-scale (w_exp) is added to protect fp16 precision.

```diff
diff --git a/include/mudiff_hip.h b/include/mudiff_hip.h
--- a/include/mudiff_hip.h
+++ b/include/mudiff_hip.h
@@ -23,6 +23,7 @@
 #define MUD_PRO_AFFINE_SILU 2
 #define MUD_PRO_LRELU 3
 #define MUD_PRO_UP2_AFFINE_SILU 4
+#define MUD_PRO_S2D 5
 
 #define MUD_PREC_16X3 0
 #define MUD_PREC_FP8X 1
@@ -91,6 +92,7 @@
   int prec; int w_exp;
   int res_up2; float res_k[4];
   int in_up2; float in_k[4];
+  int in_s2d;
 } mud_conv_args;
 
 int mud_conv2d_direct(const mud_conv_args* a, void* stream);
@@ -106,6 +108,7 @@
 int64_t mud_conv2d_mfma_splitk_bytes(const mud_conv_args* a);
 int mud_conv2d_mfma_res_up2_supported(const mud_conv_args* a);
 int mud_conv2d_mfma_in_up2_supported(const mud_conv_args* a);
+int mud_conv2d_mfma_in_s2d_supported(const mud_conv_args* a);
 
 typedef struct mud_census_args {
   const float* x; int B, H, W, C, ldx;
diff --git a/mu-diff_amd/backbones/up_or_down_sampling.py b/mu-diff_amd/backbones/up_or_down_sampling.py
--- a/mu-diff_amd/backbones/up_or_down_sampling.py
+++ b/mu-diff_amd/backbones/up_or_down_sampling.py
@@ -87,8 +87,41 @@
     return View.from_nchw(r)
 
 
-def padded_strided_conv(x: View, kk, pad, weights, ks, cout, bias, res, out_scale, out, layer=None):
+def fold_fir_conv_weight(w, k1d, dtype=torch.float32):
+    Cout, Cin = w.shape[:2]
+    kf = torch.as_tensor(np.asarray(k1d, dtype=np.float64)[::-1].copy(), device=w.device)
+    w64 = w.detach().double()
+    w6 = torch.zeros(Cout, Cin, 6, 6, dtype=torch.float64, device=w.device)
+    for a in range(3):
+        for b in range(3):
+            w6[:, :, a:a + 4, b:b + 4] += w64[:, :, a, b, None, None] * (kf[:, None] * kf[None, :])
+    folded = w6.reshape(Cout, Cin, 3, 2, 3, 2).permute(0, 3, 5, 1, 2, 4).reshape(Cout, 4 * Cin, 3, 3)
+    return folded.to(dtype).contiguous()
+
+
+def fold_weight_exponent(w):
+    m = float(w.detach().abs().max())
+    if not (m > 0.0) or not np.isfinite(m):
+        return 0
+    return max(-60, min(60, 8 - int(np.ceil(np.log2(m)))))
+
+
+def separable_taps(kk, pad):
+    k = np.asarray(kk, dtype=np.float64)
+    if k.shape != (4, 4) or tuple(pad) != (2, 2) or not k.sum() > 0.0:
+        return None
+    t = k.sum(axis=1) / np.sqrt(k.sum())
+    return t if np.allclose(np.outer(t, t), k, rtol=1e-7, atol=0.0) else None
+
+
+def padded_strided_conv(x: View, kk, pad, weights, ks, cout, bias, res, out_scale, out, layer=None, folded=None):
     if x.C % 4 == 0 and x.C >= 8 and ks == 3 and x.H % 2 == 0 and x.W % 2 == 0:
+        if folded is not None and ops.PYR_S2D:
+            prec = ops.PREC_16X1 if ops.PREC_PLAN == 'fp16' else ops.PREC_16X3
+            if ops.in_s2d_ok(x.B, x.H, x.W, x.C, cout, prec):
+                wf, w_exp = folded(prec)
+                return ops.conv(x, wf, 3, cout, mfma=True, bias=bias, res=res, out_scale=out_scale, out=out, in_s2d=True, prec=prec, w_exp=w_exp,
+                                layer=layer, flops=2.0 * x.B * (x.H // 2) * (x.W // 2) * cout * x.C * 9)
         xf, _ = ops.fir_nhwc(x, kk, 1, 1, pad)
         prec = ops.choose_prec(xf, cout, ops.PRO_NONE, sub2=True)
         return ops.conv(xf, weights(True, prec), 3, cout, mfma=True, bias=bias, res=res, out_scale=out_scale, out=out, sub2=True, prec=prec,
@@ -116,6 +149,11 @@
             self.bias = nn.Parameter(torch.zeros(out_ch))
         self.up, self.down, self.resample_kernel, self.kernel, self.use_bias = up, down, resample_kernel, kernel, use_bias
         self._prep = None
+        self._fold = None
+        self._fold_taps = None
+        if down and kernel == 3:
+            kk, _, _, pad = fir_params('conv_down', resample_kernel, conv_k=kernel)
+            self._fold_taps = separable_taps(kk, pad)
 
     def _weights(self, mfma=False, prec=ops.PREC_16X3):
         key = (self.weight._version, self.weight.data_ptr(), mfma, prec)
@@ -124,6 +162,17 @@
                 self._prep = (key, ops.pack_conv_weight(self.weight, prec=prec) if mfma else ops.direct_weight(self.weight))
         return self._prep[1]
 
+    def _folded_weights(self, prec):
+        key = (self.weight._version, self.weight.data_ptr(), prec)
+        if self._fold is None or self._fold[0] != key:
+            if torch.cuda.is_available() and torch.cuda.is_current_stream_capturing():
+                raise RuntimeError('Conv2d: the folded down-sampling operand must be packed before graph capture (run the layer once eagerly)')
+            with torch.no_grad():
+                w64 = fold_fir_conv_weight(self.weight, self._fold_taps, dtype=torch.float64)
+                w_exp = fold_weight_exponent(w64)
+                self._fold = (key, (ops.pack_conv_weight((w64 * 2.0 ** w_exp).float(), prec=prec), w_exp))
+        return self._fold[1]
+
     def run(self, x: View, res: View = None, out_scale=1.0, out: View = None):
         if self.up:
             raise NotImplementedError('Conv2d(up=True) is unreachable in the reference (upsample_conv_2d raises)')
@@ -131,8 +180,9 @@
         if not self.down:
             return ops.conv(x, self._weights(), self.kernel, self.weight.shape[0], mfma=False, bias=bias, res=res, out_scale=out_scale, out=out)
         kk, up, down, pad = fir_params('conv_down', self.resample_kernel, conv_k=self.kernel)
+        folded = self._folded_weights if self._fold_taps is not None else None
         return padded_strided_conv(x, kk, pad, self._weights, self.kernel, self.weight.shape[0], bias, res, out_scale, out,
-                                   layer=self.__dict__.get('_layer_name', 'Conv2d_0'))
+                                   layer=self.__dict__.get('_layer_name', 'Conv2d_0'), folded=folded)
 
     def forward(self, x):
         return self.run(View.from_nchw(x)).to_nchw()
diff --git a/mu-diff_amd/csrc/conv_direct.hip b/mu-diff_amd/csrc/conv_direct.hip
--- a/mu-diff_amd/csrc/conv_direct.hip
+++ b/mu-diff_amd/csrc/conv_direct.hip
@@ -241,6 +241,7 @@
   MUD_REQUIRE(a.x && a.w && a.out, "mud_conv2d_direct: null pointer");
   MUD_REQUIRE(a.B >= 0 && a.H > 0 && a.W > 0 && a.Cin > 0 && a.Cout > 0 && a.ks >= 1 && a.stride >= 1 && a.pad >= 0,
               "mud_conv2d_direct: bad sizes");
+  MUD_REQUIRE(!a.in_s2d, "mud_conv2d_direct: in_s2d (the space-to-depth view gathered while it is staged) is built for mud_conv2d_mfma's 3x3 kernel only");
   MUD_REQUIRE(a.ldx >= a.Cin && a.ldo >= a.Cout, "mud_conv2d_direct: ld smaller than C");
   MUD_REQUIRE(a.pro_mode == MUD_PRO_NONE || a.pro_mode == MUD_PRO_LRELU || (a.pro_scale && a.pro_shift && a.pro_ld >= a.Cin), "mud_conv2d_direct: prologue arrays missing");
   MUD_REQUIRE(!a.res || a.ldr >= a.Cout, "mud_conv2d_direct: bad residual view");
diff --git a/mu-diff_amd/csrc/conv_mfma.hip b/mu-diff_amd/csrc/conv_mfma.hip
--- a/mu-diff_amd/csrc/conv_mfma.hip
+++ b/mu-diff_amd/csrc/conv_mfma.hip
@@ -164,6 +164,9 @@
   static_assert(!IUP || (KS == 3 && !DUAL && G::ROWS % 2 == 0 && G::LDS_MAX + G::UP_BYTES <= 160 * 1024), "in_up2: 3x3, no fused skip conv, even tile rows, LDS budget");
   constexpr int GN_OFF = G::GN_OFF + (IUP ? G::UP_BYTES : 0);
   constexpr int NRAW = IUP ? G::UP_NLOAD : G::NLOAD;
+  constexpr bool S2D = PRO == MUD_PRO_S2D;
+  constexpr int PROX = S2D ? MUD_PRO_NONE : PRO;
+  static_assert(!S2D || (KS == 3 && !DUAL), "in_s2d: 3x3, no fused skip conv");
   using HV4 = h16x4;
   using HV8 = h16x8;
   extern __shared__ __attribute__((aligned(16))) char smem[];
@@ -192,7 +195,7 @@
   } else {
     flat0 = (int64_t)tile * G::P;
   }
-  const float* xb = a.x + (int64_t)b * (IUP ? (int64_t)(a.H >> 1) * (a.W >> 1) : HW) * a.ldx;
+  const float* xb = a.x + (int64_t)b * (IUP ? (int64_t)(a.H >> 1) * (a.W >> 1) : S2D ? 4 * HW : HW) * a.ldx;
   const int64_t tile_bytes = (int64_t)k16s * (G::TAPS * G::BSTEP);
   const char* wb = (const char*)a.w + (int64_t)b * a.w_bstride + (int64_t)nt * WN * tile_bytes;
   const float* psc = a.pro_scale + (int64_t)b * a.pro_ld;
@@ -232,7 +235,8 @@
       const int py = p / G::PW, px = p - py * G::PW;
       const int gy = ty0 + py - 1, gx = tx0 + px - 1;
       valid = gy >= 0 && gy < a.H && gx >= 0 && gx < a.W;
-      g = ((int64_t)gy * a.W + gx) * a.ldx;
+      if constexpr (S2D) g = ((int64_t)(2 * gy) * (2 * a.W) + 2 * gx) * a.ldx;
+      else g = ((int64_t)gy * a.W + gx) * a.ldx;
       if (DUAL) {
         const bool centre = py >= 1 && py <= G::ROWS && px >= 1 && px <= 32 && tid + j * G::NT < G::ITEMS;
         const int col = px - 1, sw = (col >> 2) & 3;
@@ -271,6 +275,11 @@
   auto fetch_raw = [&](int chunk) {
     int c = chunk * G::KCH + q * 4;
     c = c < a.Cin ? c : 0;
+    if constexpr (S2D) {
+      const int cpp = a.Cin >> 6, kc_ = chunk < k16s ? chunk : k16s - 1;
+      const int par = (kc_ >= cpp ? 1 : 0) + (kc_ >= 2 * cpp ? 1 : 0) + (kc_ >= 3 * cpp ? 1 : 0);
+      c = ((par >> 1) * 2 * a.W + (par & 1)) * a.ldx + (kc_ - par * cpp) * 16 + q * 4;
+    }
 #pragma unroll
     for (int j = 0; j < NRAW; ++j) {
       if constexpr (CNT) asm volatile("global_load_dwordx4 %0, %1, off" : "=v"(raw[j]) : "v"(xb + goff[j] + c) : "memory");
@@ -297,7 +306,7 @@
       const float keep = (cvalid && ((vmask >> j) & 1u)) ? 1.0f : 0.0f;
       HV4 hi, lo;
       int a8 = 0, al8 = 0;
-      cm_stage4<PRO, X8, H1>(raw[j], psc_r, psh_r, keep, hi, lo, a8, al8);
+      cm_stage4<PROX, X8, H1>(raw[j], psc_r, psh_r, keep, hi, lo, a8, al8);
       *(HV4*)(buf + loff[j]) = hi;
       if constexpr (X8) {
         *(int*)(buf + loff[j] + 32 - q * 4) = a8;
@@ -501,6 +510,7 @@
           const int gx = tx0 + (reg & 3) + 8 * (reg >> 2) + 4 * hh;
           const bool ok = gy < a.H && gx < a.W && co < a.Cout;
           acc[m][n][reg] = ok ? a.res[(((int64_t)b * a.H + gy) * a.W + gx) * a.ldr + co] : 0.f;
+          if constexpr (S2D) acc[m][n][reg] *= __builtin_ldexpf(1.0f, a.w_exp);
         }
       }
     }
@@ -636,7 +646,7 @@
           }
           constexpr int SPAN = G::STEPS - G::GS;
           auto jb = [](int i) {
-            if (PRO != MUD_PRO_NONE) return (i * G::NLOAD) / SPAN;
+            if (PROX != MUD_PRO_NONE) return (i * G::NLOAD) / SPAN;
             return i >= SPAN ? G::NLOAD : ((i > 0 ? i - 1 : 0) * G::NLOAD + G::NLOAD - 1) / SPAN;
           };
           const int j0 = jb(st - G::GS), j1 = jb(st - G::GS + 1);
@@ -657,6 +667,15 @@
   };
   for (int kc = kc0; kc + 1 < nchunks; ++kc) chunk_body(kc, std::true_type{});
   if (kc0 < nchunks) chunk_body(nchunks - 1, std::false_type{});
+  if constexpr (S2D) {
+    const float unscale = __builtin_ldexpf(1.0f, -a.w_exp);
+#pragma unroll
+    for (int m = 0; m < MT; ++m)
+#pragma unroll
+      for (int n = 0; n < 2; ++n)
+#pragma unroll
+        for (int i = 0; i < 16; ++i) acc[m][n][i] *= unscale;
+  }
 
   if constexpr (KS == 3) {
     if (slab_mode) {
@@ -1381,6 +1400,7 @@
     if (ns > 1 && a.splitk_ws_bytes < cm_slab_bytes(ns, nblocks, 64 * WM * WN * 32 * MT * (DUAL ? 2 : 1))) ns = 1;
     MUD_REQUIRE(ns == 1 || !a.res_up2, "mud_conv2d_mfma: res_up2 is not built for a launch split over K (ask mud_conv2d_mfma_res_up2_supported first)");
     MUD_REQUIRE(ns == 1 || !a.in_up2, "mud_conv2d_mfma: in_up2 is not built for a launch split over K (ask mud_conv2d_mfma_in_up2_supported first)");
+    MUD_REQUIRE(ns == 1 || !a.in_s2d, "mud_conv2d_mfma: in_s2d is not built for a launch split over K (ask mud_conv2d_mfma_in_s2d_supported first)");
     if (ns > 1) {
       mud_conv_args p = a;
       p.out = (float*)a.splitk_ws;
@@ -1487,6 +1507,21 @@
   return cm_in_up2_built(v, ap->prec) && cm_splits(blocks, (int)mud_cdiv(ap->Cin, 16)) == 1;
 }
 
+static bool cm_in_s2d_built(int variant, int prec) {
+  return (variant == CMV_8X2 || variant == CMV_MT1) && (prec == MUD_PREC_16X3 || prec == MUD_PREC_16X1);
+}
+static bool cm_in_s2d_form(const mud_conv_args& a) {
+  return a.ks == 3 && a.stride == 1 && a.pad == 1 && !a.sub2 && !a.skip_w && !a.res_up2 && !a.in_up2 && a.pro_mode == MUD_PRO_NONE && a.Cin > 0 && a.Cin % 64 == 0;
+}
+extern "C" int mud_conv2d_mfma_in_s2d_supported(const mud_conv_args* ap) {
+  if (!ap || !cm_in_s2d_form(*ap) || ap->B <= 0 || ap->H <= 0 || ap->W <= 0 || ap->Cout <= 0) return 0;
+  static const bool forced_tile = getenv("MUD_CONV_MT") != nullptr;
+  if (forced_tile) return 0;
+  int64_t blocks = 0;
+  const int v = cm_variant3(*ap, &blocks);
+  return cm_in_s2d_built(v, ap->prec) && cm_splits(blocks, (int)mud_cdiv(ap->Cin, 16)) == 1;
+}
+
 static bool cm_fp8x_built(const mud_conv_args& a) {
   if (a.ks != 3 || a.sub2 || (a.pro_mode != MUD_PRO_NONE && a.pro_mode != MUD_PRO_AFFINE_SILU)) return false;
   if (a.skip_w && a.pro_mode != MUD_PRO_AFFINE_SILU) return false;
@@ -1509,8 +1544,21 @@
   MUD_REQUIRE(a.x && a.w && a.out, "mud_conv2d_mfma: null pointer");
   MUD_REQUIRE((a.ks == 1 || a.ks == 3) && a.stride == 1 && a.pad == a.ks / 2, "mud_conv2d_mfma: only ks in {1,3}, stride 1, pad ks/2 (got ks=%d stride=%d pad=%d)", a.ks, a.stride, a.pad);
   MUD_REQUIRE(a.B >= 0 && a.H > 0 && a.W > 0 && a.Cin > 0 && a.Cout > 0, "mud_conv2d_mfma: bad sizes");
-  MUD_REQUIRE(a.Cin % 4 == 0 && a.ldx % 4 == 0 && a.ldx >= a.Cin && mud_aligned16(a.x), "mud_conv2d_mfma: needs Cin%%4==0 (Cin=%d), ldx%%4==0 (ldx=%d), 16-byte aligned x", a.Cin, a.ldx);
-  MUD_REQUIRE((int64_t)a.H * a.W * a.ldx < 0x7fffffffLL, "mud_conv2d_mfma: one image must stay below 2^31 elements");
+  if (a.in_s2d) {
+    MUD_REQUIRE(cm_in_s2d_form(a),
+                "mud_conv2d_mfma: in_s2d needs ks == 3, no prologue, no sub2 / fused skip conv / res_up2 / in_up2 and Cin %% 64 == 0 (ks=%d sub2=%d pro_mode=%d Cin=%d)",
+                a.ks, a.sub2, a.pro_mode, a.Cin);
+    MUD_REQUIRE(a.ldx % 4 == 0 && a.ldx >= a.Cin / 4 && mud_aligned16(a.x), "mud_conv2d_mfma: in_s2d needs ldx%%4==0, ldx >= Cin/4 (Cin=%d ldx=%d), 16-byte aligned x", a.Cin, a.ldx);
+    MUD_REQUIRE(4 * (int64_t)a.H * a.W * a.ldx < 0x7fffffffLL, "mud_conv2d_mfma: in_s2d: one full-resolution image must stay below 2^31 elements");
+    MUD_REQUIRE(a.prec == MUD_PREC_16X3 || a.prec == MUD_PREC_16X1, "mud_conv2d_mfma: in_s2d is built for the two fp16 plans only (prec=%d)", a.prec);
+    MUD_REQUIRE(a.w_exp >= -100 && a.w_exp <= 100, "mud_conv2d_mfma: in_s2d: w_exp (the weights' power-of-two pre-scale) out of range (%d)", a.w_exp);
+    static const bool forced_tile = getenv("MUD_CONV_MT") != nullptr;
+    MUD_REQUIRE(!forced_tile && cm_in_s2d_built(cm_variant3(a, nullptr), a.prec),
+                "mud_conv2d_mfma: in_s2d is not built for the tile of this launch (ask mud_conv2d_mfma_in_s2d_supported first)");
+  } else {
+    MUD_REQUIRE(a.Cin % 4 == 0 && a.ldx % 4 == 0 && a.ldx >= a.Cin && mud_aligned16(a.x), "mud_conv2d_mfma: needs Cin%%4==0 (Cin=%d), ldx%%4==0 (ldx=%d), 16-byte aligned x", a.Cin, a.ldx);
+    MUD_REQUIRE((int64_t)a.H * a.W * a.ldx < 0x7fffffffLL, "mud_conv2d_mfma: one image must stay below 2^31 elements");
+  }
   MUD_REQUIRE(mud_aligned16(a.w) && a.w_bstride % 16 == 0, "mud_conv2d_mfma: packed weights must be 16-byte aligned");
   MUD_REQUIRE(a.ldo >= a.Cout && (!a.res || a.ldr >= a.Cout), "mud_conv2d_mfma: bad output/residual view");
   MUD_REQUIRE(!a.stats || a.stats_ld >= a.Cout, "mud_conv2d_mfma: bad stats view");
@@ -1568,6 +1616,12 @@
                                        : cm_launch_pro<3, 2, 4, 2, PU>(a, s);
     return a.prec == MUD_PREC_16X1 ? cm_launch_pro<3, 1, 4, 1, PU, false, MUD_PREC_16X1>(a, s) : cm_launch_pro<3, 1, 4, 1, PU>(a, s);
   }
+  if (a.in_s2d) {
+    constexpr int PS = MUD_PRO_S2D;
+    if (cm_variant3(a, nullptr) == CMV_8X2)
+      return a.prec == MUD_PREC_16X1 ? cm_launch_pro<3, 2, 4, 2, PS, false, MUD_PREC_16X1>(a, s) : cm_launch_pro<3, 2, 4, 2, PS>(a, s);
+    return a.prec == MUD_PREC_16X1 ? cm_launch_pro<3, 1, 4, 1, PS, false, MUD_PREC_16X1>(a, s) : cm_launch_pro<3, 1, 4, 1, PS>(a, s);
+  }
 #ifdef MUD_EXPERIMENT_WS
   if (cm_ws_wanted(a)) return cm_ws_dispatch(a, s);
 #endif
diff --git a/mu-diff_amd/mudiff_hip/__init__.py b/mu-diff_amd/mudiff_hip/__init__.py
--- a/mu-diff_amd/mudiff_hip/__init__.py
+++ b/mu-diff_amd/mudiff_hip/__init__.py
@@ -42,6 +42,7 @@
         ('prec', C.c_int), ('w_exp', C.c_int),
         ('res_up2', C.c_int), ('res_k', C.c_float * 4),
         ('in_up2', C.c_int), ('in_k', C.c_float * 4),
+        ('in_s2d', C.c_int),
     ]
 
 
@@ -111,6 +112,7 @@
     'mud_conv2d_mfma_splitk_bytes': (_L, [C.POINTER(ConvArgs)]),
     'mud_conv2d_mfma_res_up2_supported': (_I, [C.POINTER(ConvArgs)]),
     'mud_conv2d_mfma_in_up2_supported': (_I, [C.POINTER(ConvArgs)]),
+    'mud_conv2d_mfma_in_s2d_supported': (_I, [C.POINTER(ConvArgs)]),
     'mud_upfirdn2d': (_I, [_P, _L, _I, _I, _P, _I, _I, _I, _I, _I, _I, _I, _I, _I, _I, _P, _P]),
     'mud_fir_nhwc': (_I, [_P, _I, _I, _I, _I, _I, C.POINTER(C.c_float), _I, _I, _I, _I, _I, _I, _P, _P, _I, _I, _P, _I, _P, _I, _P]),
     'mud_minibatch_stddev': (_I, [_P, _I, _L, _I, _I, _I, _P, _P]),
diff --git a/mu-diff_amd/mudiff_hip/ops.py b/mu-diff_amd/mudiff_hip/ops.py
--- a/mu-diff_amd/mudiff_hip/ops.py
+++ b/mu-diff_amd/mudiff_hip/ops.py
@@ -72,6 +72,9 @@
 
     def up2_shape(self):
         return View(self.base, self.B, 2 * self.H, 2 * self.W, self.C, self.ld, self.c0)
+
+    def s2d_shape(self):
+        return View(self.base, self.B, self.H // 2, self.W // 2, 4 * self.C, self.ld, self.c0)
 
     def slice(self, c0, C_):
         assert 0 <= c0 and c0 + C_ <= self.C
@@ -388,6 +391,23 @@
     return bool(load().mud_conv2d_mfma_in_up2_supported(C.byref(a)))
 
 
+PYR_S2D = os.environ.get('MUD_PYR_S2D', '1') != '0'
+
+
+def in_s2d_ok(B, H, W, c, cout, prec=PREC_16X3):
+    if H % 2 or W % 2 or c % 16 or cout % 4:
+        return False
+    a = ConvArgs()
+    a.B, a.H, a.W, a.Cin, a.ldx, a.ks, a.stride, a.pad, a.Cout, a.ldo, a.pro_mode, a.prec = B, H // 2, W // 2, 4 * c, c, 3, 1, 1, cout, cout, PRO_NONE, prec
+    a.in_s2d = 1
+    return bool(load().mud_conv2d_mfma_in_s2d_supported(C.byref(a)))
+
+
+def s2d_fold(t):
+    B, H, W, Cc = t.shape
+    return t.reshape(B, H // 2, 2, W // 2, 2, Cc).permute(0, 1, 3, 2, 4, 5).reshape(B, H // 2, W // 2, 4 * Cc).contiguous()
+
+
 def resolve_pro(pro):
     if pro is not None and isinstance(pro[0], LazyGN):
         sc, sh = pro[0].tensors()
@@ -485,7 +505,7 @@
     return PREC_FP8X if conv_prec_supported(x, cout, pro_mode, PREC_FP8X, skip=skip, sub2=sub2) else PREC_16X3
 
 
-Launch = collections.namedtuple('Launch', 'layer ks mfma prec shape sub2 skip pro')
+Launch = collections.namedtuple('Launch', 'layer ks mfma prec shape sub2 skip pro s2d', defaults=(False,))
 
 
 RECORD = None
@@ -493,7 +513,12 @@
 
 def conv(x: View, w, ks, Cout, *, mfma, stride=1, pad=None, pro=None, bias=None, bias2=None, res: View = None,
          out_scale=1.0, act=ACT_NONE, out: View = None, w_bstride=0, arena=None, sub2=False, emul: View = None, gate=None, emul_cout=0,
-         skip=None, prec=PREC_16X3, w_exp=0, layer=None, res_up2=None, split_k=True, in_up2=None):
+         skip=None, prec=PREC_16X3, w_exp=0, layer=None, res_up2=None, split_k=True, in_up2=None, in_s2d=False, flops=None):
+    if in_s2d:
+        assert mfma and ks == 3 and stride == 1 and not sub2 and skip is None and res_up2 is None and in_up2 is None and pro is None
+        if x.H % 2 or x.W % 2 or x.C % 16:
+            raise MudiffHipError(f'conv: in_s2d needs even H, W and C % 16 == 0 (got {x.H}x{x.W}, C={x.C})')
+        x = x.s2d_shape()
     if in_up2 is not None:
         assert mfma and ks == 3 and stride == 1 and not sub2 and skip is None and res_up2 is None and len(in_up2) == 4
         assert pro is not None and pro[2] == PRO_AFFINE_SILU
@@ -501,8 +526,8 @@
     if RECORD is not None:
         if torch.cuda.is_current_stream_capturing():
             raise RuntimeError('precision.launch_record() is eager only: the launch is being captured into a graph')
-        RECORD.append(Launch(layer, ks, bool(mfma), prec, (x.B, x.H, x.W, x.C, Cout), bool(sub2), skip is not None,
-                             PRO_NONE if pro is None else pro[2]))
+        RECORD.append(Launch(layer, ks, bool(mfma), prec, (x.B, x.H, x.W, x.C, Cout), bool(sub2 or in_s2d), skip is not None,
+                             PRO_NONE if pro is None else pro[2], bool(in_s2d)))
     lib = load()
     pad = ks // 2 if pad is None else pad
     Ho = (x.H + 2 * pad - ks) // stride + 1
@@ -549,6 +574,8 @@
         a.res, a.ldr = res.ptr, res.ld
     if in_up2 is not None:
         a.in_up2, a.in_k = 1, (C.c_float * 4)(*in_up2)
+    if in_s2d:
+        a.in_s2d = 1
     a.out_scale, a.act = out_scale, act
     a.sub2 = 1 if sub2 else 0
     if emul is not None:
@@ -568,7 +595,7 @@
         assert mfma and ks == 3 and res is None and (so.B, so.H, so.W, so.C) == (x.B, Ho, Wo, Cout)
         a.skip_w, a.skip_bias, a.skip_out, a.skip_ldo = ptr(sw), ptr(sb), so.ptr, so.ld
         skip_flops = 2.0 * x.B * Ho * Wo * Cout * x.C
-    if mfma and ks == 3 and split_k and res_up2 is None and in_up2 is None:
+    if mfma and ks == 3 and split_k and res_up2 is None and in_up2 is None and not in_s2d:
         cnt = splitk_counters(x.device)
         a.splitk_counters, a.splitk_ncounters = ptr(cnt), cnt.numel()
         nws = lib.mud_conv2d_mfma_splitk_bytes(C.byref(a))
@@ -577,7 +604,8 @@
             a.splitk_ws, a.splitk_ws_bytes = ptr(keep[1]), nws
     fn = lib.mud_conv2d_mfma if mfma else lib.mud_conv2d_direct
     name = (f'conv_mfma_k{ks}' if mfma else f'conv_direct_k{ks}') + {PREC_FP8X: '_fp8x', PREC_16X1: '_fp16'}.get(prec, '')
-    flops = 2.0 * x.B * Ho * Wo * Cout * x.C * ks * ks + skip_flops
+    if flops is None:
+        flops = 2.0 * x.B * Ho * Wo * Cout * x.C * ks * ks + skip_flops
     nbytes = 4.0 * ((x_lo if in_up2 is not None else x).npix * x.C + out.npix * Cout * ((2 if res is not None else 1) + (1 if skip is not None else 0))) + (w.numel() * w.element_size() if w_bstride == 0 else x.B * w_bstride)
     _launch(name, x.device, fn, C.byref(a), STREAM, flops=flops, nbytes=nbytes)
     return out
```

Result: faster. 112.7 slices/s, median of 6 (+1.1%).
